# leejet/stable-diffusion.cpp

Measured on AMD Instinct MI355X. Metric: denoise it/s (image-iterations/s: cond+uncond UNet forwards per image per step), higher is better.
Workload: dtype f16; 1 GPU; sd15 UNet 512x512, cfg 7 (cond+uncond), f16 weights, batch 8/GPU, Euler-A step; global_batch=8, flash_attn=True, hip_graph=1, cfg_pair_in_one_graph=True, device_resident_sampler=True

## Files before the change

include/ggml-mi355x.h:

```cpp
#ifndef GGML_MI355X_H
#define GGML_MI355X_H

#include "ggml-abi.h"

#ifdef __cplusplus
extern "C" {
#endif

#define GGML_MI355X_API __attribute__((visibility("default")))

GGML_MI355X_API ggml_backend_reg_t ggml_backend_init(void);
GGML_MI355X_API int ggml_backend_score(void);
GGML_MI355X_API ggml_backend_reg_t ggml_backend_mi355x_reg(void);
GGML_MI355X_API int ggml_backend_mi355x_get_device_count(void);

struct ggml_backend_mi355x_stats {
    int64_t graphs_computed;
    int64_t plans_built;
    int64_t nodes_seen;
    int64_t kernels_planned;
    int64_t kernels_launched;
    int64_t fused_conv;
    int64_t fused_conv_bounced;
    int64_t fused_linear;
    int64_t fused_norm;
    int64_t fused_geglu;
    int64_t fused_attention;
    int64_t generic_matmul;
    int64_t swizzled_weight_bytes;
    int64_t graph_replays;
    int64_t fused_linear_geglu;
    int64_t split_k_gemms;
    int64_t head_major_gemms;
    int64_t fused_modulate;
    int64_t fused_gate;
    int64_t fused_gelu;
    int64_t fused_rope;
    int64_t fused_concat_heads;
    int64_t qgemv_linears;
    int64_t fused_chan_add;
    int64_t fused_proj_tokens;
    int64_t gemm_attention;
    int64_t fused_q16;
    int64_t split_k_inlaunch;
    int64_t qgemm16_linears;
    int64_t fgemv_linears;
    int64_t fused_presilu;
    int64_t fused_sibling_linears;
    int64_t hoisted_kv_linears;
    int64_t window_convs;
    int64_t hoisted_emb_linears;
    int64_t fused_rows16;
    int64_t fused_joint_qkv;
    int64_t jit_images;
    int64_t fused_cat_rows16;
    int64_t fused_gn_stats;
    int64_t fused_ln_reduce;
    int64_t redirect_fallbacks;
    int64_t fused_concat_gn;
    int64_t fused_conv_scale;
    int64_t view_graphs;
    int64_t plans_evicted;
    int64_t hoisted_mod_linears;
    int64_t view_external_nodes;
    int64_t qinloop_linears;
    int64_t flash_out_alias;
    int64_t flash_slice_images;
    int64_t flash_short_launches;
    int64_t flash_qb2_launches;
    int64_t flash_mslot_launches;
    int64_t flash_generic_launches;
};
GGML_MI355X_API void ggml_backend_mi355x_get_stats(struct ggml_backend_mi355x_stats* out);
GGML_MI355X_API int ggml_backend_mi355x_resolve_enums(const char* (*op_name)(int), const char* (*unary_op_name)(int), const char* (*type_name)(int));
GGML_MI355X_API const char* ggml_backend_mi355x_enum_status(void);
GGML_MI355X_API void ggml_backend_mi355x_get_enum_maps(uint8_t* ops256, uint8_t* unary256);
struct ggml_backend_mi355x_kernel_timing {
    char kernel[96];
    int64_t launches;
    double total_ms;
    double total_flops;
    double total_bytes;
    int32_t bound;
    int32_t family;
};
GGML_MI355X_API void ggml_backend_mi355x_kernel_timing_enable(int enable);
GGML_MI355X_API void ggml_backend_mi355x_kernel_timing_enable_mask(uint32_t family_mask);
GGML_MI355X_API void ggml_backend_mi355x_get_kernel_timing(struct ggml_backend_mi355x_kernel_timing* out);
GGML_MI355X_API int ggml_backend_mi355x_get_kernel_timings(struct ggml_backend_mi355x_kernel_timing* out, int capacity);
GGML_MI355X_API void ggml_backend_mi355x_set_option(const char* key, int value);
struct ggml_backend_mi355x_calibration {
    float mfma_f16_tflops;
    float mfma_clock_mhz;
    float copy_tbs;
    float read_tbs;
    int compute_units;
};
GGML_MI355X_API int ggml_backend_mi355x_calibrate(struct ggml_backend_mi355x_calibration* out);
GGML_MI355X_API void* ggml_backend_mi355x_get_stream(ggml_backend_t backend);
GGML_MI355X_API const char* ggml_backend_mi355x_hip_library(void);
GGML_MI355X_API int ggml_backend_mi355x_set_device(int hip_device);
GGML_MI355X_API int ggml_backend_mi355x_get_device(void);

#ifdef __cplusplus
}
#endif
#endif
```

stable-diffusion.cpp_amd/__init__.py:

```python
from __future__ import annotations

import ctypes as C
import os
from pathlib import Path

import numpy as np

PKG_DIR = Path(__file__).resolve().parent
ROOT = PKG_DIR.parent
LIB_DIR = PKG_DIR / "lib"
HOST_LIB = Path(os.environ.get("SDCPP_HOST_LIB", str(LIB_DIR / "libsdcpp-host.so")))
BACKEND_LIB = Path(os.environ.get("SDCPP_BACKEND_LIB", str(LIB_DIR / "libggml-mi355x.so")))

F32, F16, Q4_0, Q8_0, I32, BF16 = 0, 1, 2, 8, 26, 30
TYPE_SIZE = {F32: 4, F16: 2, BF16: 2, I32: 4}

SD15, SDXL, SD15_TINY, SDXL_TINY, SD35_LARGE, SD35_TINY, FLUX_DEV, FLUX_TINY, SD35_WIDE2, FLUX_WIDE1, SD3M_TINY, SD35_WIDE8, FLUX_WIDE8 = 0, 1, 2, 3, 4, 5, 6, 7, 8, 9, 10, 11, 12
PAIR_EXCHANGE_FN = C.CFUNCTYPE(C.c_bool, C.c_void_p, C.c_int64, C.c_void_p, C.c_void_p)
EVAL_CALLBACK_FN = C.CFUNCTYPE(C.c_bool, C.c_void_p, C.c_bool, C.c_void_p)
EULER, EULER_A, HEUN, DPM2, DPMPP2S_A, DPMPP2M, DPMPP2Mv2, IPNDM, IPNDM_V, LCM, DDIM_TRAILING = range(11)
TCD, RES_MULTISTEP, RES_2S, ER_SDE, EULER_CFG_PP, EULER_A_CFG_PP, EULER_GE, DPMPP2M_SDE, DPMPP2M_SDE_BT, LMS = range(11, 21)
SAMPLE_METHOD_DEFAULT = 21
SCHED_DISCRETE, SCHED_KARRAS, SCHED_EXPONENTIAL, SCHED_AYS, SCHED_GITS, SCHED_SGM_UNIFORM, SCHED_SIMPLE, SCHED_SMOOTHSTEP, SCHED_KL_OPTIMAL, SCHED_LCM = range(10)
SCHED_BONG_TANGENT, SCHED_FLUX, SCHED_BETA, SCHEDULER_DEFAULT = 10, 14, 15, 16
# ... 202 lines not shown
    L.sd_get_tensor_f32.restype = C.c_bool
    L.sd_set_tensor_f32.argtypes = [C.c_void_p, C.c_char_p, C.c_void_p, C.c_int64]
    L.sd_set_tensor_f32.restype = C.c_bool
    L.sd_unet_forward.argtypes = [C.c_void_p, C.c_void_p, C.c_int, C.c_int, C.c_int, C.c_int, C.c_void_p, C.c_void_p,
                                  C.c_int64, C.c_int64, C.c_int64, C.c_void_p, C.c_int64, C.c_int64, C.c_void_p]
    L.sd_unet_forward.restype = C.c_bool
    L.sd_vae_decode.argtypes = [C.c_void_p, C.c_void_p, C.c_int, C.c_int, C.c_int, C.c_int, C.c_void_p]
    L.sd_vae_decode.restype = C.c_bool
    L.sd_sample_latents.argtypes = [C.c_void_p, C.POINTER(SdImgGenParams), C.c_void_p]
    L.sd_sample_latents.restype = C.c_bool
    L.sdm_generate_image.argtypes = [C.c_void_p, C.POINTER(SdImgGenParams), C.POINTER(C.POINTER(SdImage)), C.POINTER(C.c_int)]
    L.sdm_generate_image.restype = C.c_bool
    L.sdm_free_images.argtypes = [C.POINTER(SdImage), C.c_int]
    L.sd_philox_randn.argtypes = [C.c_uint64, C.c_uint32, C.c_uint32, C.c_void_p]
    L.sd_philox_uint32.argtypes = [C.c_uint64, C.c_uint32, C.c_uint32, C.c_void_p]
    L.sd_get_sigmas.argtypes = [C.c_int, C.c_void_p]
    L.sd_get_flow_sigmas.argtypes = [C.c_int, C.c_float, C.c_void_p]
    L.sd_get_flux_sigmas.argtypes = [C.c_int, C.c_int, C.c_void_p]
    L.sd_set_guidance.argtypes = [C.c_void_p, C.c_float]
    L.sd_set_guidance.restype = None
    L.sd_set_vae_conv2d_scale.argtypes = [C.c_void_p, C.c_float]
    L.sd_set_vae_conv2d_scale.restype = C.c_bool
    L.sd_set_pair_exchange.argtypes = [C.c_void_p, PAIR_EXCHANGE_FN, C.c_void_p, C.c_int]
    L.sd_set_pair_exchange.restype = None
    L.sd_rccl_get_unique_id.argtypes = [C.c_void_p]
    L.sd_rccl_get_unique_id.restype = C.c_bool
    L.sd_rccl_comm_create.argtypes = [C.c_int, C.c_int, C.c_int, C.c_void_p]
    L.sd_rccl_comm_create.restype = C.c_void_p
    L.sd_rccl_comm_destroy.argtypes = [C.c_void_p]
    L.sd_rccl_comm_destroy.restype = None
    L.sd_set_pair_exchange_rccl.argtypes = [C.c_void_p, C.c_void_p, C.c_int]
    L.sd_set_pair_exchange_rccl.restype = C.c_bool
    L.sd_rccl_last_error.restype = C.c_char_p
    L.sd_gen_flux_pe.argtypes = [C.c_int, C.c_int, C.c_int, C.c_int, C.POINTER(C.c_int), C.c_int, C.c_float, C.c_void_p]
    L.sd_sigma_to_t.argtypes = [C.c_float]
    L.sd_sigma_to_t.restype = C.c_float
    L.sd_get_stats.argtypes = [C.c_void_p, C.POINTER(SdStats)]
    L.sd_load_weights_prefixed.argtypes = [C.c_void_p, C.c_char_p, C.c_char_p, C.POINTER(C.c_int64), C.POINTER(C.c_int64)]
    L.sd_load_weights_prefixed.restype = C.c_int64
    L.sd_convert_tensor_name.argtypes = [C.c_void_p, C.c_char_p, C.c_char_p, C.c_size_t]
    L.sd_convert_tensor_name.restype = C.c_bool
    L.sd_text_encoders_init.argtypes = [C.c_void_p]
    L.sd_text_encoders_init.restype = C.c_bool
    L.sd_clip_forward.argtypes = [C.c_void_p, C.c_int, C.c_void_p, C.c_int, C.c_int, C.c_bool, C.c_int, C.c_void_p, C.c_int64]
    L.sd_clip_forward.restype = C.c_int64
    L.sd_t5_forward.argtypes = [C.c_void_p, C.c_void_p, C.c_int, C.c_void_p, C.c_int64]
    L.sd_t5_forward.restype = C.c_int64
    L.sd_t5_relative_position_buckets.argtypes = [C.c_int, C.c_int, C.c_void_p]
    L.sd_get_learned_condition.argtypes = [C.c_void_p, C.POINTER(SdTokenList), C.POINTER(SdTokenList), C.POINTER(SdTokenList), C.c_int, C.c_int, C.c_int,
                                           C.c_bool, C.c_void_p, C.c_int64, C.POINTER(C.c_int64), C.c_void_p, C.c_int64, C.POINTER(C.c_int64)]
    L.sd_get_learned_condition.restype = C.c_bool
    L.sdm_set_backend_eval_callback.argtypes = [EVAL_CALLBACK_FN, C.c_void_p]
    L.sdm_set_backend_eval_callback.restype = None
    L.sdm_backend_graph_compute_with_eval_callback.argtypes = [C.c_void_p, C.c_void_p, EVAL_CALLBACK_FN, C.c_void_p]
    L.sdm_backend_graph_compute_with_eval_callback.restype = C.c_int
    _lib = L
    return L


_loaded_plugins: set[str] = set()


def load_backend(path: os.PathLike | str) -> None:
    p = str(Path(path).resolve())
    if p in _loaded_plugins:
        return
    if not lib().sd_load_backend(p.encode()):
        raise EngineError(f"failed to load backend plug-in {p}")
    _loaded_plugins.add(p)


def load_mi355x_backend() -> None:
    if not BACKEND_LIB.exists():
        raise EngineError(f"{BACKEND_LIB} missing — the HIP backend was not built")
    load_backend(BACKEND_LIB)
    names = devices()
    if not any(n.upper().startswith("MI355X") for n in names):
        raise EngineError(f"libggml-mi355x.so loaded but exposes no MI355X device (devices: {names}); is a gfx950 GPU visible?")


_BACKEND_STAT_FIELDS = ("graphs_computed plans_built nodes_seen kernels_planned kernels_launched fused_conv fused_conv_bounced fused_linear "
                        "fused_norm fused_geglu fused_attention generic_matmul swizzled_weight_bytes graph_replays fused_linear_geglu "
                        "split_k_gemms head_major_gemms fused_modulate fused_gate fused_gelu fused_rope fused_concat_heads qgemv_linears fused_chan_add fused_proj_tokens gemm_attention fused_q16 split_k_inlaunch qgemm16_linears fgemv_linears fused_presilu fused_sibling_linears hoisted_kv_linears window_convs hoisted_emb_linears fused_rows16 fused_joint_qkv jit_images fused_cat_rows16 fused_gn_stats fused_ln_reduce redirect_fallbacks fused_concat_gn fused_conv_scale view_graphs plans_evicted hoisted_mod_linears view_external_nodes qinloop_linears flash_out_alias flash_slice_images "
                        "flash_short_launches flash_qb2_launches flash_mslot_launches flash_generic_launches").split()


class BackendStats(C.Structure):
    _fields_ = [(n, C.c_int64) for n in _BACKEND_STAT_FIELDS]


_backend_cdll = None


def _backend() -> C.CDLL:
    global _backend_cdll
    if _backend_cdll is None:
        load_mi355x_backend()
        _backend_cdll = C.CDLL(str(BACKEND_LIB))
        _backend_cdll.ggml_backend_mi355x_get_stats.argtypes = [C.POINTER(BackendStats)]
        _backend_cdll.ggml_backend_mi355x_set_option.argtypes = [C.c_char_p, C.c_int]
    return _backend_cdll


def backend_stats() -> dict:
    st = BackendStats()
    _backend().ggml_backend_mi355x_get_stats(C.byref(st))
    return {n: int(getattr(st, n)) for n in _BACKEND_STAT_FIELDS}


class KernelTiming(C.Structure):
    _fields_ = [("kernel", C.c_char * 96), ("launches", C.c_int64), ("total_ms", C.c_double), ("total_flops", C.c_double),
                ("total_bytes", C.c_double), ("bound", C.c_int32), ("family", C.c_int32)]


KF_ALL = 0x3FFFF


def kernel_timing_enable(on) -> None:
    b = _backend()
    b.ggml_backend_mi355x_kernel_timing_enable_mask.argtypes = [C.c_uint32]
    mask = 1 if on is True else int(on or 0)
    b.ggml_backend_mi355x_kernel_timing_enable_mask(mask)


def _timing_dict(kt) -> dict:
    return {"kernel": kt.kernel.decode(), "family": int(kt.family), "bound": "hbm" if kt.bound else "mfma", "launches": int(kt.launches),
            "total_ms": float(kt.total_ms), "total_flops": float(kt.total_flops), "total_bytes": float(kt.total_bytes)}


def kernel_timings() -> list:
    arr = (KernelTiming * 32)()
    b = _backend()
    b.ggml_backend_mi355x_get_kernel_timings.argtypes = [C.POINTER(KernelTiming), C.c_int]
    b.ggml_backend_mi355x_get_kernel_timings.restype = C.c_int
    n = b.ggml_backend_mi355x_get_kernel_timings(arr, 32)
    return [_timing_dict(arr[i]) for i in range(n)]


def kernel_timing() -> dict:
    t = kernel_timings()
    return t[0] if t else {"kernel": "(no timed launches)", "family": -1, "bound": "mfma", "launches": 0, "total_ms": 0.0, "total_flops": 0.0, "total_bytes": 0.0}


class Calibration(C.Structure):
    _fields_ = [("mfma_f16_tflops", C.c_float), ("mfma_clock_mhz", C.c_float), ("copy_tbs", C.c_float), ("read_tbs", C.c_float), ("compute_units", C.c_int)]


def calibrate() -> dict | None:
    b = _backend()
    b.ggml_backend_mi355x_calibrate.argtypes = [C.POINTER(Calibration)]
    c = Calibration()
    if b.ggml_backend_mi355x_calibrate(C.byref(c)) != 0:
        return None
    return {"mfma_f16_tflops": round(c.mfma_f16_tflops, 1), "mfma_clock_mhz": round(c.mfma_clock_mhz, 1), "copy_tbs": round(c.copy_tbs, 3), "read_tbs": round(c.read_tbs, 3),
            "compute_units": c.compute_units}


def backend_set_option(key: str, value: int) -> None:
    _backend().ggml_backend_mi355x_set_option(key.encode(), int(value))


def devices() -> list[str]:
    L = lib()
    return [L.sd_device_name(i).decode() for i in range(L.sd_device_count())]


def _fptr(a: np.ndarray | None):
# ... 542 lines not shown
```

stable-diffusion.cpp_amd/csrc/backend/planner.cpp:

```cpp
#include "planner.h"

#include <atomic>
#include <cstddef>
#include <cstdio>
#include <cstdlib>
#include <cstring>
#include <functional>
#include <memory>
#include <mutex>
#include <string>
#include <algorithm>
#include <map>
#include <unordered_map>
#include <unordered_set>
#include <vector>

#include "kernels.h"
#include "ktime.h"

namespace mi355x {

static uint8_t g_opmap[256];
static uint8_t g_unmap[256];
static bool g_opmap_init = [] {
// ... 26 lines not shown
const NameNum kNeededTypes[] = {
    {"f32", GGML_TYPE_F32}, {"f16", GGML_TYPE_F16}, {"q4_0", GGML_TYPE_Q4_0}, {"q8_0", GGML_TYPE_Q8_0}, {"i32", GGML_TYPE_I32}, {"bf16", GGML_TYPE_BF16},
};

bool plausible_op_name(const char* nm) {
    if (!nm) return false;
    int n = 0;
    for (; nm[n] && n <= 32; ++n)
        if (!((nm[n] >= 'A' && nm[n] <= 'Z') || (nm[n] >= '0' && nm[n] <= '9') || nm[n] == '_')) return false;
    return n > 0 && n <= 32;
}
bool build_map(const char* (*name_of)(int), const NameNum* need, int n_need, int cap, int unknown, uint8_t* table, char* err, size_t err_len, const char* what,
               const char* const* optional = nullptr, int n_optional = 0) {
    uint8_t out[256];
    for (int i = 0; i < 256; ++i) out[i] = (uint8_t)unknown;
    std::vector<int> found(n_need, -1);
    int left = n_need;
    for (int h = 0; h < cap && left > 0; ++h) {
        const char* nm = name_of(h);
        if (!plausible_op_name(nm)) break;
        for (int k = 0; k < n_need; ++k)
            if (!strcmp(nm, need[k].name)) {
                if (found[k] >= 0) {
                    snprintf(err, err_len, "host %s numbers %d and %d are both named '%s'", what, found[k], h, nm);
                    return false;
                }
                found[k] = h;
                out[h]   = (uint8_t)need[k].num;
                --left;
            }
    }
    for (int k = 0; k < n_need; ++k)
        if (found[k] < 0) {
            bool opt = false;
            for (int o = 0; o < n_optional; ++o) opt = opt || !strcmp(optional[o], need[k].name);
            if (opt) continue;
            snprintf(err, err_len, "host has no %s named '%s'", what, need[k].name);
            return false;
        }
    memcpy(table, out, 256);
    return true;
}
}

bool planner_build_op_maps(const char* (*op_name)(int), const char* (*unary_name)(int), const char* (*type_name)(int), char* err, size_t err_len) {
    uint8_t ops[256], un[256];
    if (err && err_len) err[0] = 0;
    char local[256];
    if (!err) {
        err     = local;
        err_len = sizeof(local);
    }
    static const char* const kOptionalOps[]   = {"CONV_2D"};
    static const char* const kOptionalUnary[] = {"EXP"};
    if (op_name && !build_map(op_name, kNeededOps, (int)(sizeof(kNeededOps) / sizeof(kNeededOps[0])), 200, GGML_OP_COUNT, ops, err, err_len, "op", kOptionalOps, 1)) return false;
    if (unary_name && !build_map(unary_name, kNeededUnary, (int)(sizeof(kNeededUnary) / sizeof(kNeededUnary[0])), 64, GGML_UNARY_OP_COUNT, un, err, err_len, "unary op", kOptionalUnary, 1))
        return false;
    if (type_name) {
        for (const NameNum& t : kNeededTypes) {
            const char* nm = type_name(t.num);
            if (!nm || strcmp(nm, t.name)) {
                snprintf(err, err_len, "host ggml_type %d is named '%s', this backend was written against '%s'", t.num, nm ? nm : "(null)", t.name);
                return false;
            }
        }
    }
    if (op_name) memcpy(g_opmap, ops, 256);
    if (unary_name) memcpy(g_unmap, un, 256);
    return true;
}
void planner_get_op_maps(uint8_t* ops256, uint8_t* unary256) {
    if (ops256) memcpy(ops256, g_opmap, 256);
    if (unary256) memcpy(unary256, g_unmap, 256);
}

namespace {

constexpr size_t N_STATS = sizeof(ggml_backend_mi355x_stats) / sizeof(int64_t);
static_assert(N_STATS * sizeof(int64_t) == sizeof(ggml_backend_mi355x_stats), "ggml_backend_mi355x_stats: int64_t fields only");
std::atomic<int64_t> g_stat_counters[N_STATS];
#define STAT(field) g_stat_counters[offsetof(ggml_backend_mi355x_stats, field) / sizeof(int64_t)]

struct Options {
    std::atomic<int> fusion{1}, mfma_gemm{1}, hip_graph{1}, flash_pattern{1}, fuse_modulate{1}, fuse_gate{1}, fuse_gelu{1}, fuse_rope{1}, fuse_concat_heads{1}, qgemv{1}, fuse_chan_add{1}, fuse_proj_tokens{1}, fuse_q16{1}, qgemm16{1}, fgemv{1}, fuse_siblings{1}, hoist_kv{1}, hoist_emb{1}, fuse_rows16{0}, fuse_cat_rows16{1}, fuse_joint_qkv{1}, jit_qimages{4096}, fuse_gn_stats{1}, fuse_ln_reduce{1}, relax_res_overlap{1}, fuse_split_gelu{1}, fuse_concat_gn{1}, fuse_gn_tokens{1}, fuse_linear_nchw{1}, fuse_conv_scale{1}, ignore_use_counts{0}, plan_cache_cap{512}, hoist_mod{1}, fuse_flash_slices{1}, fuse_act_pack{1};
} g_opt;

using Step = std::function<void(hipStream_t)>;

struct Plan {
    int n_nodes = 0;
    uint64_t check = 0;
    size_t arena_needed = 0;
    std::vector<Step> steps;
    hipGraphExec_t graph_exec = nullptr;
    bool graph_failed         = false;
    int64_t runs              = 0;
    uint64_t last_use         = 0;
};

struct SwzEntry {
    void* swz;
    size_t bytes;
    const void* src;
    size_t src_bytes;
};

std::mutex g_mu;
std::vector<Planner*> g_planners;

}

struct Planner {
    int device;
    std::mutex mu;
    uint64_t tick = 0;
    std::unordered_map<uint64_t, std::unique_ptr<Plan>> plans;
    std::unordered_map<uint64_t, SwzEntry> swz;
    char* arena       = nullptr;
    size_t arena_cap  = 0;
    std::map<size_t, void*> jit_buf;
    void* jit_buffer(size_t bytes, int parity = 0) {
        const size_t key = bytes * 2 + (size_t)(parity & 1);
        auto it = jit_buf.find(key);
        if (it != jit_buf.end()) return it->second;
        void* d = nullptr;
        if (hipMalloc(&d, bytes) != hipSuccess) return nullptr;
        jit_buf[key] = d;
        return d;
    }
};

namespace {

inline bool overlaps(const void* a, size_t an, const void* b, size_t bn) {
    const char* pa = (const char*)a;
    const char* pb = (const char*)b;
    return pa < pb + bn && pb < pa + an;
}

bool flash_out_aliases_operand(const ggml_tensor* ct, const ggml_tensor* fa, bool q_in_arena, bool k_in_arena, bool v_in_arena) {
    const size_t on = ggml_abi_nbytes(ct);
    const bool skip[3] = {q_in_arena, k_in_arena, v_in_arena};
    for (int j = 0; j < 3; ++j) {
        const ggml_tensor* o = fa->src[j];
        if (!o || skip[j]) continue;
        const ggml_tensor* root = o->view_src ? o->view_src : o;
        if (overlaps(ct->data, on, root->data, ggml_abi_nbytes(root)) || overlaps(ct->data, on, o->data, ggml_abi_nbytes(o))) return true;
    }
    return false;
}

View4 view_of(const ggml_tensor* t) {
    View4 v;
    v.data = t->data;
    for (int i = 0; i < 4; ++i) {
        v.ne[i] = t->ne[i];
        v.nb[i] = (int64_t)t->nb[i];
    }
    v.type = (int)t->type;
    return v;
}
inline bool is_f32(const ggml_tensor* t) { return t->type == GGML_TYPE_F32; }
inline bool contig(const ggml_tensor* t) { return ggml_abi_is_contiguous(t); }
inline const ggml_tensor* root_of(const ggml_tensor* t) { return t->view_src ? t->view_src : t; }
inline bool is_static_weight(const ggml_tensor* t) {
    const ggml_backend_buffer* b = t->view_src ? t->view_src->buffer : t->buffer;
    return b != nullptr && b->usage == GGML_BACKEND_BUFFER_USAGE_WEIGHTS;
// ... 109 lines not shown
        mix2(h, k, &n->data, sizeof(n->data));
        for (int j = 0; j < GGML_MAX_SRC; ++j) {
            const ggml_tensor* s = n->src[j];
            if (!s) break;
            const uint64_t sh[4] = {(uint64_t)(uintptr_t)s->data, ((uint64_t)(uint32_t)s->type << 32) | (uint32_t)j,
                                    ((uint64_t)(uint32_t)s->op << 32) | (is_static_weight(s) ? 1u : 0u), (uint64_t)s->view_offs};
            mix2(h, k, sh, sizeof(sh));
            mix2(h, k, s->ne, sizeof(s->ne));
            mix2(h, k, s->nb, sizeof(s->nb));
        }
    }
    return {h, k};
}

struct GInfo {
    const ggml_cgraph* g;
    std::unordered_map<const ggml_tensor*, int> index;
    std::vector<std::vector<int>> consumers;
    std::vector<char> done;

    ggml_tensor phantom;
    bool is_view = false;
    int n_external = 0;

    explicit GInfo(const ggml_cgraph* gr) : g(gr), consumers(gr->n_nodes + 1), done(gr->n_nodes + 1, 0) {
        memset(&phantom, 0, sizeof(phantom));
        phantom.op = (enum ggml_op)255;
        for (int h = 255; h >= 0; --h)
            if (g_opmap[h] == GGML_OP_COUNT) {
                phantom.op = (enum ggml_op)h;
                break;
            }
        snprintf(phantom.name, sizeof(phantom.name), "(reader outside the view)");
        done[g->n_nodes] = 1;
        for (int i = 0; i < g->n_nodes; ++i) index[g->nodes[i]] = i;
        for (int i = 0; i < g->n_nodes; ++i) {
            const ggml_tensor* n = g->nodes[i];
            for (int j = 0; j < GGML_MAX_SRC; ++j) {
                if (!n->src[j]) continue;
                auto it = index.find(n->src[j]);
                if (it != index.end()) consumers[it->second].push_back(i);
            }
        }
        is_view = graph_is_view(g);
        if (is_view) {
            std::vector<char> ext;
            view_external_nodes(g, ext);
            for (int i = 0; i < g->n_nodes; ++i)
                if (ext[i]) {
                    consumers[i].push_back(g->n_nodes);
                    ++n_external;
                }
        }
    }
    const ggml_tensor* node(int i) const { return i == g->n_nodes ? &phantom : g->nodes[i]; }
    int idx(const ggml_tensor* t) const {
        auto it = index.find(t);
        return it == index.end() ? -1 : it->second;
    }
    int sole(int i) const {
        if (i < 0 || consumers[i].size() != 1) return -1;
        if (node(i)->flags & GGML_TENSOR_FLAG_OUTPUT) return -1;
        if (i == g->n_nodes - 1) return -1;
        return consumers[i][0];
    }
    bool only_noops_between(int a, int b, const std::vector<int>& chain) const {
        for (int k = a + 1; k < b; ++k) {
            if (ggml_abi_op_is_noop(xop(node(k)))) continue;
            bool in_chain = false;
            for (int c : chain) in_chain = in_chain || (c == k);
            if (!in_chain) return false;
        }
        return true;
    }
};

struct Packed {
    size_t off;
    int64_t ld;
    bool nhwc;
    float mul = 1.f;
    int64_t runL = 0, runS = 0;
};

struct Builder {
    Planner* P;
    Plan* plan;
    GInfo gi;
    size_t arena_off = 0;
    std::unordered_map<const ggml_tensor*, Packed> packed;
    std::unordered_map<const ggml_tensor*, size_t> q16;
    std::unordered_map<const ggml_tensor*, const ggml_tensor*> ups;
    std::unordered_map<const ggml_tensor*, const ggml_tensor*> presilu;
    std::map<int, std::vector<Step>> deferred;
    std::map<size_t, int> jit_seq;
    Builder(Planner* p, Plan* pl, const ggml_cgraph* g) : P(p), plan(pl), gi(g) {}
    int emit_redirect = -1;
    bool hm_grouping  = false;
    bool hm_hoisting  = false;
    struct HmLaunch {
        int node, out_node;
        float* dst;
        void* dst16;
        size_t dst16_off;
        bool dst16_arena;
        size_t a_off;
        int64_t lda;
        const void* swz;
        int64_t tokens, K, M;
        Epilogue ep;
        int hd, hH, hL;
    };
    std::vector<HmLaunch> hm_group;
    std::unordered_map<const ggml_tensor*, size_t> moved;
    struct MovedEmb {
        size_t off;
        int64_t ld, M, N;
    };
    std::unordered_map<const ggml_tensor*, MovedEmb> moved_emb;
    struct GnPre {
        size_t off;
        const float *w, *b;
        int groups;
        float eps;
    };
    std::unordered_map<const ggml_tensor*, GnPre> gn_pre;
    struct LnPre {
        size_t off;
        const float *w, *b;
        float eps;
    };
    std::unordered_map<const ggml_tensor*, LnPre> ln_pre;
    struct Cat16 {
        size_t off;
        int64_t ld;
        bool written[2];
    };
    struct Cat16Part {
        size_t off;
        int64_t ld, col;
        int cat, part;
    };
    std::unordered_map<int, Cat16> cat16;
    std::unordered_map<const ggml_tensor*, Cat16Part> cat16_part;
    struct PreScale {
        const ggml_tensor* src;
        float mul;
    };
    std::unordered_map<const ggml_tensor*, PreScale> prescale;
    std::unordered_set<const ggml_tensor*> cat16_by_linear;
    struct JPart {
        size_t off = 0;
        int64_t xs = 0;
        const float* w = nullptr;
        float eps = 0.f;
    };
    struct JCat {
        JPart part[2];
        int d = 0, H = 0, last = -1;
        bool f16 = false;
        std::vector<int> chain;
    };
    std::unordered_map<int, JCat> jqkv;
    std::unordered_map<const ggml_tensor*, size_t> lin_redirect;
    std::unordered_set<const ggml_tensor*> redirect_taken;
    bool no_redirect = false;
    struct RopeSrc {
        JPart part[2];
        int64_t La = 0, Lb = 0;
    };
    std::unordered_map<int, RopeSrc> rope_src, v_src;
    std::unordered_map<int, std::pair<size_t, size_t>> scratch_slots;
    size_t scratch(int key, size_t bytes) {
        auto it = scratch_slots.find(key);
        if (it != scratch_slots.end() && it->second.second >= bytes) return it->second.first;
        const size_t off   = alloc(bytes);
        scratch_slots[key] = {off, bytes};
        return off;
    }
    void emit(Step s) {
        if (emit_redirect >= 0)
            deferred[emit_redirect].push_back(std::move(s));
        else
            plan->steps.push_back(std::move(s));
    }
    void emit_at(int node, int cur, Step s) {
        if (node <= cur)
            emit(std::move(s));
        else
            deferred[node].push_back(std::move(s));
    }
    bool clobbered_between(int a, int b, const void* p, size_t n, const std::vector<int>& chain) const {
        for (int k = a + 1; k <= b; ++k) {
            const ggml_tensor* t = gi.node(k);
            if (ggml_abi_op_is_noop(xop(t))) continue;
            bool in_chain = false;
            for (int c : chain) in_chain = in_chain || (c == k);
            if (in_chain) continue;
            const char *a0 = (const char*)t->data, *b0 = (const char*)p;
            if (a0 < b0 + n && b0 < a0 + ggml_abi_nbytes(t)) return true;
        }
        return false;
    }
    size_t alloc(size_t bytes) {
        const size_t off = (arena_off + 255) & ~(size_t)255;
        arena_off        = off + bytes;
        return off;
    }
    static constexpr size_t CNT_CAP = 1u << 18;
// ... 445 lines not shown
        STAT(qgemv_linears)++;
        STAT(fused_linear)++;
        if (silu) STAT(fused_presilu)++;
        return;
    }
    if (g_opt.fgemv && plain_epi && simple_rows && src_safe && emit_node == i && fgemv_supported((int)w->type, tokens, K) && aligned16(w->data)) {
        float* fdst       = (float*)gi.node(last)->data;
        const float* fx   = (const float*)xsrc->data;
        const int64_t fxs = (int64_t)x->nb[1] / 4;
        const void* wp    = w->data;
        const int wt      = (int)w->type;
        const bool silu   = xsrc != x;
        B.emit([=](hipStream_t st) { launch_fgemv(st, fdst, M, fx, fxs, tokens, wp, wt, K, M, ep, silu); });
        STAT(fgemv_linears)++;
        STAT(fused_linear)++;
        if (silu) STAT(fused_presilu)++;
        return;
    }
    if (xsrc != x) {
        float* ud       = (float*)x->data;
        const float* us = (const float*)xsrc->data;
        const int64_t un = ggml_abi_nelements(x);
        B.emit([=](hipStream_t st) { launch_unary(st, UN_SILU, ud, us, un); });
    }
    const bool useq  = g_opt.qgemm16 && hm_d == 0 && geglu_out < 0 && qgemm16_supported((int)w->type, tokens, K, M);
    const void* wraw = w->data;
    const int wt     = (int)w->type;
    const bool qin = !useq && geglu_out < 0 && hm_d == 0 && !B.hm_hoisting && nchw_add < 0 && (wt == 8 || wt == 2) &&
                     (int64_t)w->nb[1] == (int64_t)ggml_abi_row_size(w->type, K) && aligned16(w->data) && gemm16_qinloop_supported(wt, tokens, M, K, 1, 1);
    if (qin) {
        ep.qtype      = wt;
        ep.qrow_bytes = (int64_t)w->nb[1];
        STAT(qinloop_linears)++;
    }
    const bool jit = !useq && !qin && g_opt.jit_qimages > 0 && tokens >= g_opt.jit_qimages && geglu_out < 0 && hm_d == 0 && !B.hm_hoisting && wswz_q_supported((int)w->type, K) &&
                     (int64_t)w->nb[1] == (int64_t)ggml_abi_row_size(w->type, K) && aligned16(w->data);
    const int geglu_mode = geglu_out >= 0 ? gemm16_geglu_mode(tokens, M, K) : 0;
    const void* swz = useq ? nullptr : qin ? w->data : (jit ? B.P->jit_buffer(wswz_bytes(M, K), B.jit_seq[wswz_bytes(M, K)]++) : get_swz_linear(B.P, w, s, geglu_mode));
    if (jit && swz) {
        void* jb          = const_cast<void*>(swz);
        const void* wsrc  = w->data;
        const int wty     = (int)w->type;
        B.emit_at(emit_node, i, [=](hipStream_t st) { launch_wswz_q(st, jb, wsrc, wty, K, M); });
        STAT(jit_images)++;
    }
    float* dst      = (float*)gi.node(last)->data;
    const float* xp = (const float*)x->data;
    const int64_t xs = (int64_t)x->nb[1] / 4;
    const ggml_tensor* key = strip_reshape(x);
    auto it = B.packed.find(key);
    if (it == B.packed.end() || it->second.nhwc) {
        Packed pk{B.alloc((size_t)tokens * rup64(K) * 2), rup64(K), false};
        Planner* P = B.P;
        const size_t off = pk.off;
        const bool runs  = x->ne[2] > 1 && x->nb[2] != x->nb[1] * (size_t)x->ne[1];
        const int64_t pL = runs ? x->ne[1] : 0, pbs = runs ? (int64_t)x->nb[2] / 4 : 0;
        B.emit([=](hipStream_t st) { launch_pack_rows_f16(st, P->arena + off, xp, tokens, K, xs, pL, pbs); });
        it = B.packed.emplace(key, pk).first;
        if (it->second.nhwc) it->second = pk;
    }
    Planner* P       = B.P;
    size_t off       = it->second.off;
    const int64_t ld = it->second.ld;
    if (it->second.runL > 0) {
        const int64_t rL = it->second.runL, rS = it->second.runS;
        if (geglu_out >= 0 || hm_d > 0 || nchw_add >= 0) {
            const size_t goff = B.alloc((size_t)tokens * ld * 2), soff = off;
            const int64_t nrun = tokens / rL;
            B.emit([=](hipStream_t st) {
                for (int64_t r = 0; r < nrun; ++r)
                    (void)hipMemcpyAsync(P->arena + goff + (size_t)(r * rL * ld * 2), P->arena + soff + (size_t)(r * rS * ld * 2), (size_t)(rL * ld * 2), hipMemcpyDeviceToDevice, st);
            });
            off = goff;
        } else {
            ep.a_run_L = rL;
            ep.a_run_S = rS;
        }
    }
    if (nchw_add >= 0 && !useq && swz && ld == rup64(K) && geglu_out < 0 && gelu_out < 0 && !ep.gate && !redir) {
        float* ndst             = (float*)gi.node(nchw_add)->data;
        const int64_t HWt = nchw_HW, Nimg = nchw_N;
        const float* resp       = nchw_res;
        const Builder::Split sk = B.plan_split(tokens, M, rup64(K), true, true);
        B.emit_at(emit_node, i, [=](hipStream_t st) {
            Epilogue e2 = ep;
            e2.residual = resp;
            launch_gemm16_conv(st, ndst, P->arena + off, swz, HWt, 1, K, Nimg, M, 1, 1, 0, false, e2, sk.ws(P), sk.cnt(P), sk.S);
        });
        STAT(fused_linear)++;
        STAT(fused_proj_tokens)++;
        return;
    }
    if (nchw_add >= 0) {
        while (!chain.empty() && chain.back() != last) chain.pop_back();
    }
    if (geglu_out >= 0) {
        const size_t ooff  = B.alloc((size_t)tokens * (M / 2) * 2);
        const float* biasp = ep.bias;
        const Builder::Split sk = B.plan_split(tokens, M, K, false, false, true);
        B.emit([=](hipStream_t st) { launch_gemm16_linear_geglu(st, P->arena + ooff, P->arena + off, ld, swz, tokens, K, M, biasp, sk.ws(P), sk.cnt(P), sk.S, geglu_mode); });
        B.packed[gi.node(geglu_out)] = Packed{ooff, M / 2, false};
        STAT(fused_geglu)++;
        STAT(fused_linear_geglu)++;
    } else if (gelu_out >= 0) {
        const size_t ooff = B.alloc((size_t)tokens * M * 2);
        if (useq) {
            B.emit([=](hipStream_t st) { launch_qgemm16(st, nullptr, P->arena + ooff, M, P->arena + off, ld, tokens, wraw, wt, K, M, ep); });
            STAT(qgemm16_linears)++;
        } else {
            const Builder::Split sk = B.plan_split(tokens, M, K, false, false);
            B.emit([=](hipStream_t st) { launch_gemm16_linear(st, nullptr, P->arena + ooff, M, P->arena + off, ld, swz, tokens, K, M, M, ep, 0, 0, 0, sk.ws(P), sk.cnt(P), sk.S); });
        }
        B.packed[gi.node(gelu_out)] = Packed{ooff, M, false};
        STAT(fused_gelu)++;
    } else if (hm_d > 0) {
        void* hdst = gi.node(last)->data;
        STAT(head_major_gemms)++;
        const bool f16o = hm_f16;
        const int hd = hm_d, hH = hm_H, hL = hm_L;
        int qflash = -1, qview = -1;
        if (!f16o && g_opt.fuse_q16 && hd % 8 == 0) {
            const int c1 = gi.sole(last);
            const int c2 = (c1 >= 0 && xop(gi.node(c1)) == GGML_OP_RESHAPE) ? gi.sole(c1) : -1;
            if (c2 >= 0 && xop(gi.node(c2)) == GGML_OP_FLASH_ATTN_EXT && gi.node(c2)->src[0] == gi.node(c1) && !gi.node(c2)->src[3] && contig(gi.node(c1)) &&
                gi.node(c1)->ne[0] == hd && flash_attn_supported(hd, gi.node(c2)->src[2]->ne[0])) {
                qflash = c2;
                qview  = c1;
            }
        }
        const bool groupable = B.hm_grouping && !ep.residual && !ep.gate && !ep.gelu && !ep.chan_add;
        if (qflash >= 0) {
            const size_t qoff        = B.alloc((size_t)tokens * M * 2);
            B.q16[gi.node(qview)]    = qoff;
            STAT(fused_q16)++;
            const Builder::Split sk = B.plan_split(tokens, M, K, false, false);
            if (groupable && sk.S <= 1)
                B.hm_group.push_back(Builder::HmLaunch{i, last, nullptr, nullptr, qoff, true, off, ld, swz, tokens, K, M, ep, hd, hH, hL});
            else
                B.emit([=](hipStream_t st) { launch_gemm16_linear(st, nullptr, P->arena + qoff, 0, P->arena + off, ld, swz, tokens, K, M, M, ep, hd, hH, hL, sk.ws(P), sk.cnt(P), sk.S); });
        } else {
            const Builder::Split sk = (hL >= 32 && !B.hm_hoisting) ? B.plan_split(tokens, M, K, false, false) : Builder::Split();
            if (groupable && sk.S <= 1)
                B.hm_group.push_back(Builder::HmLaunch{i, last, f16o ? nullptr : (float*)hdst, f16o ? hdst : nullptr, 0, false, off, ld, swz, tokens, K, M, ep, hd, hH, hL});
            else
                B.emit([=](hipStream_t st) {
                    launch_gemm16_linear(st, f16o ? nullptr : (float*)hdst, f16o ? hdst : nullptr, 0, P->arena + off, ld, swz, tokens, K, M, M, ep, hd, hH, hL, sk.ws(P), sk.cnt(P), sk.S);
                });
        }
    } else if (useq) {
        const int S        = ep.gate ? 1 : qgemm16_split_k(tokens, K, M);
        const size_t wsoff = S > 1 ? B.alloc((size_t)S * tokens * M * 4) : 0;
        B.emit_at(emit_node, i, [=](hipStream_t st) {
            launch_qgemm16(st, redir ? (float*)(P->arena + redir_off) : dst, nullptr, 0, P->arena + off, ld, tokens, wraw, wt, K, M, ep, S > 1 ? (float*)(P->arena + wsoff) : nullptr, S);
        });
        if (redir) B.redirect_taken.insert(gi.node(last));
        STAT(qgemm16_linears)++;
    } else if (g_opt.fuse_rows16 && !ep.gate && emit_node == i && M % 64 == 0 && x->ne[3] == 1 && only_consumer_is_tokens_to_conv(gi, last)) {
        const size_t ooff       = B.alloc((size_t)tokens * M * 2);
        const Builder::Split sk = B.plan_split(tokens, M, K, false, false);
        B.emit([=](hipStream_t st) { launch_gemm16_linear(st, nullptr, P->arena + ooff, M, P->arena + off, ld, swz, tokens, K, M, M, ep, 0, 0, 0, sk.ws(P), sk.cnt(P), sk.S); });
        B.packed[gi.node(last)] = Packed{ooff, M, false};
        STAT(fused_rows16)++;
    } else {
        const Builder::Split sk = B.plan_split(tokens, M, K, false, !ep.gate);
        bool ln_on       = false;
        size_t ln_off    = 0;
        const float *lnw = nullptr, *lnb = nullptr;
        float lneps      = 0.f;
        if (g_opt.fuse_ln_reduce && g_opt.fusion && sk.S > 1 && sk.S <= 4 && !sk.inkernel && !redir && !ep.gate && emit_node == i && hm_d == 0 && splitk_reduce_ln_supported(tokens, M) &&
// ... 539 lines not shown
        const int jp = gi.sole(last);
        const int jc = (jp >= 0 && xop(gi.node(jp)) == GGML_OP_PERMUTE && gi.node(jp)->src[0] == gi.node(last)) ? gi.sole(jp) : -1;
        if (jc >= 0 && xop(gi.node(jc)) == GGML_OP_CONT && gi.node(jc)->src[0] == gi.node(jp) && is_f32(gi.node(jc)) && contig(gi.node(jc))) {
            const int32_t* pa = gi.node(jp)->op_params;
            std::vector<int> c2 = chain;
            c2.push_back(jp);
            c2.push_back(jc);
            if (pa[0] == 1 && pa[1] == 2 && pa[2] == 0 && pa[3] == 3 && gi.node(jc)->ne[0] == OC && gi.only_noops_between(last, jc, c2) &&
                !(gi.node(last)->flags & GGML_TENSOR_FLAG_OUTPUT)) {
                chain           = c2;
                last            = jc;
                token_major_out = jc;
            }
        }
    }
    const size_t ob = ggml_abi_nbytes(out);
    int emit_node = i;
    bool emb_arena = false;
    size_t emb_off = 0;
    if (g_opt.fuse_chan_add && token_major_out < 0) {
        const int r = gi.sole(last);
        if (r >= 0 && xop(gi.node(r)) == GGML_OP_ADD && gi.node(r)->src[0] == gi.node(last)) {
            const ggml_tensor* a = gi.node(r);
            const ggml_tensor* e = a->src[1];
            const ggml_tensor* eroot = strip_reshape(e);
            const bool from_linear   = xop(eroot) == GGML_OP_MUL_MAT || (xop(eroot) == GGML_OP_ADD && eroot->src[0] && xop(strip_reshape(eroot->src[0])) == GGML_OP_MUL_MAT);
            if (!gi.done[r] && from_linear && is_f32(e) && contig(e) && contig(a) && e->ne[0] == 1 && e->ne[1] == 1 && e->ne[2] == OC && e->ne[3] == N && N > 0 &&
                ggml_abi_same_shape(out, a) && gi.idx(eroot) < r && !(gi.node(last)->flags & GGML_TENSOR_FLAG_OUTPUT)) {
                bool ok = true;
                for (int k = last + 1; k < r && ok; ++k) {
                    const ggml_tensor* t = gi.node(k);
                    if (ggml_abi_op_is_noop(xop(t))) continue;
                    for (int q = 0; q < GGML_MAX_SRC && t->src[q]; ++q)
                        for (int c : chain) ok = ok && t->src[q] != gi.node(c);
                }
                if (ok) {
                    ep.chan_add = (const float*)e->data;
                    chain.push_back(r);
                    last      = r;
                    emit_node = r;
                    STAT(fused_chan_add)++;
                    const auto me = B.moved_emb.find(eroot);
                    if (me != B.moved_emb.end()) {
                        emb_arena  = true;
                        emb_off    = me->second.off;
                        ep.chan_ld = me->second.ld;
                        ep.chan_add = nullptr;
                    }
                }
            }
        }
    }
    if (!ep.chan_add && !emb_arena && token_major_out < 0) {
        int r = gi.sole(last);
        if (r >= 0 && !gi.done[r] && xop(gi.node(r)) == GGML_OP_ADD && gi.only_noops_between(last, r, chain)) {
            const ggml_tensor* a     = gi.node(r);
            const ggml_tensor* other = a->src[0] == gi.node(last) ? a->src[1] : (a->src[1] == gi.node(last) ? a->src[0] : nullptr);
            if (other && is_f32(other) && contig(other) && contig(a) && ggml_abi_same_shape(other, a) && ggml_abi_same_shape(out, a) && gi.idx(other) < i &&
                (other->data == a->data || !overlaps(a->data, ob, other->data, ob))) {
                ep.residual = (const float*)other->data;
                chain.push_back(r);
                last = r;
            }
        }
    }
    float* final_dst = (float*)gi.node(last)->data;
    const int ks = KW, st_ = s0, pd = p0;
    Builder::GnPre gnp{0, nullptr, nullptr, 0, 0.f};
    if (g_opt.fuse_gn_stats && token_major_out < 0) {
        const ggml_tensor* res = gi.node(last);
        for (int k : gi.consumers[last]) {
            if (gnp.groups) break;
            const ggml_tensor* g = gi.node(k);
            if (xop(g) != GGML_OP_GROUP_NORM || g->src[0] != res || gi.done[k]) continue;
            const int j1 = gi.sole(k);
            if (j1 < 0 || xop(gi.node(j1)) != GGML_OP_MUL || gi.node(j1)->src[0] != g || !bias_like_chan(gi.node(j1)->src[1], OC)) break;
            const int j2 = gi.sole(j1);
            if (j2 < 0 || xop(gi.node(j2)) != GGML_OP_ADD || gi.node(j2)->src[0] != gi.node(j1) || !bias_like_chan(gi.node(j2)->src[1], OC)) break;
            const int64_t ohw = res->ne[0] * res->ne[1];
            if (!splitk_reduce_gn_supported(ohw, OC, N, g->op_params[0])) break;
            gnp = Builder::GnPre{0, (const float*)gi.node(j1)->src[1]->data, (const float*)gi.node(j2)->src[1]->data, g->op_params[0], ggml_abi_op_param_f32(g, 1)};
        }
    }
    auto gn_register = [&](int S) -> bool {
        if (S <= 1 || !gnp.groups) return false;
        if ((((uintptr_t)final_dst | (uintptr_t)ep.residual) & 15) != 0) return false;
        gnp.off                    = B.alloc((size_t)N * OC * 4 * 2);
        B.gn_pre[gi.node(last)]    = gnp;
        STAT(fused_gn_stats)++;
        return true;
    };
    auto gn_fill = [](Epilogue& e, const Builder::GnPre& g, char* arena, int64_t nc) {
        e.gn_scale  = (float*)(arena + g.off);
        e.gn_shift  = e.gn_scale + nc;
        e.gn_w      = g.w;
        e.gn_b      = g.b;
        e.gn_groups = g.groups;
        e.gn_eps    = g.eps;
    };
    const bool ups_in = B.ups.find(xs) != B.ups.end();
    const int w3S     = (token_major_out < 0) ? conv3w_plan(x->ne[0], x->ne[1], IC, N, OC, ks, st_, ups_in) : 0;
    const void* swz   = get_swz_conv(B.P, ker, s, w3S > 0);
    if (!swz) return false;
    const ggml_tensor* src = xs;
    bool upscale           = false;
    auto ui                = B.ups.find(xs);
    if (ui != B.ups.end()) {
        src     = ui->second;
        upscale = true;
    }
    const int64_t SW = src->ne[0], SH = src->ne[1];
    auto it = B.packed.find(src);
    if (it != B.packed.end() && it->second.nhwc && it->second.mul != pre_mul) {
        fprintf(stderr, "[ggml-mi355x] plan_conv_chain: operand image of node %d was written with factor %g, the conv wants %g\n", i, it->second.mul, pre_mul);
        return false;
    }
    if (it == B.packed.end() || !it->second.nhwc) {
        Packed pk{B.alloc((size_t)N * SW * SH * rup64(IC) * 2), rup64(IC), true, pre_mul};
        Planner* P       = B.P;
        const size_t off = pk.off;
        const float* sp  = (const float*)src->data;
        B.emit([=](hipStream_t st) { launch_nchw_to_nhwc_f16(st, P->arena + off, sp, SW * SH, IC, N, nullptr, nullptr, false, nullptr, 0, nullptr, pre_mul); });
        B.packed[src] = pk;
        it            = B.packed.find(src);
    }
    Planner* P       = B.P;
    const size_t off = it->second.off;
    const int64_t CW_ = upscale ? SW * 2 : SW, CH_ = upscale ? SH * 2 : SH;
    const int64_t opos = ((CW_ + 2 * pd - ks) / st_ + 1) * ((CH_ + 2 * pd - ks) / st_ + 1) * N;
    if (token_major_out >= 0) {
        float* tdst          = (float*)gi.node(token_major_out)->data;
        const int64_t tokens = SW * SH * N;
        const int64_t lda    = it->second.ld;
        B.emit([=](hipStream_t st) { launch_gemm16_linear(st, tdst, nullptr, 0, P->arena + off, lda, swz, tokens, IC, OC, OC, ep); });
        STAT(fused_conv)++;
        STAT(fused_proj_tokens)++;
        return true;
    }
    if (w3S > 0) {
        const size_t wsoff = w3S > 1 ? B.alloc((size_t)w3S * opos * OC * 4) : 0;
        if (w3S > 1) STAT(split_k_gemms)++;
        const bool gn_on = gn_register(w3S);
        B.emit_at(emit_node, i, [=](hipStream_t st) {
            Epilogue e2 = ep;
            if (emb_arena) e2.chan_add = (const float*)(P->arena + emb_off);
            if (gn_on) gn_fill(e2, gnp, P->arena, N * OC);
            launch_conv3w(st, final_dst, P->arena + off, swz, SW, SH, IC, N, OC, e2, w3S > 1 ? (float*)(P->arena + wsoff) : nullptr, w3S);
        });
        STAT(fused_conv)++;
        STAT(window_convs)++;
        return true;
    }
    const Builder::Split sk = B.plan_split(opos, OC, rup64(IC) * ks * ks, true, true);
    const bool gn_on        = sk.inkernel ? false : gn_register(sk.S);
    B.emit_at(emit_node, i, [=](hipStream_t st) {
        Epilogue e2 = ep;
        if (emb_arena) e2.chan_add = (const float*)(P->arena + emb_off);
        if (gn_on) gn_fill(e2, gnp, P->arena, N * OC);
        launch_gemm16_conv(st, final_dst, P->arena + off, swz, SW, SH, IC, N, OC, ks, st_, pd, upscale, e2, sk.ws(P), sk.cnt(P), sk.S);
    });
    STAT(fused_conv)++;
    return true;
}

bool plan_tokens_to_conv(Builder& B, int i, hipStream_t, std::vector<int>& chain) {
    GInfo& gi = B.gi;
    int rs    = -1;
    if (!tokens_to_conv_match(gi, i, &rs)) return false;
    const ggml_tensor* t  = gi.node(i)->src[0]->src[0];
    const ggml_tensor* xr = gi.node(rs);
    const int64_t C = t->ne[0], HW = t->ne[1], N = t->ne[2];
    chain = {i};
    STAT(fused_proj_tokens)++;
    const auto pr = B.packed.find(t);
    if (pr != B.packed.end() && !pr->second.nhwc && pr->second.ld == rup64(C)) {
        B.packed[xr] = Packed{pr->second.off, pr->second.ld, true};
        return true;
    }
    Packed pk{B.alloc((size_t)N * HW * rup64(C) * 2), rup64(C), true};
    Planner* P       = B.P;
    const size_t off = pk.off;
    const float* tp  = (const float*)t->data;
    B.emit([=](hipStream_t st) { launch_pack_rows_f16(st, P->arena + off, tp, N * HW, C, C); });
    B.packed[xr] = pk;
    return true;
}

bool plan_group_norm(Builder& B, int i, hipStream_t, std::vector<int>& chain) {
    GInfo& gi            = B.gi;
    const ggml_tensor* n = gi.node(i);
    const ggml_tensor* x = n->src[0];
    if (!is_f32(x) || !contig(x) || !contig(n)) return false;
    const int groups = n->op_params[0];
    const float eps  = ggml_abi_op_param_f32(n, 1);
    const int64_t hw = x->ne[0] * x->ne[1], C = x->ne[2], N = x->ne[3];
    const float *w = nullptr, *b = nullptr;
    bool silu = false;
    chain.push_back(i);
    int last = i;
    if (g_opt.fusion) {
        int j1 = gi.sole(i);
        if (j1 >= 0 && xop(gi.node(j1)) == GGML_OP_MUL && gi.node(j1)->src[0] == n && bias_like_chan(gi.node(j1)->src[1], C) && gi.node(j1)->data == n->data &&
            gi.only_noops_between(i, j1, chain)) {
            int j2 = gi.sole(j1);
            if (j2 >= 0 && xop(gi.node(j2)) == GGML_OP_ADD && gi.node(j2)->src[0] == gi.node(j1) && bias_like_chan(gi.node(j2)->src[1], C) &&
                gi.node(j2)->data == n->data && gi.only_noops_between(j1, j2, chain)) {
                w = (const float*)gi.node(j1)->src[1]->data;
                b = (const float*)gi.node(j2)->src[1]->data;
                chain.push_back(j1);
                chain.push_back(j2);
                last   = j2;
                int j3 = gi.sole(j2);
                if (j3 >= 0 && xop(gi.node(j3)) == GGML_OP_UNARY && xunary(gi.node(j3)) == GGML_UNARY_OP_SILU && gi.node(j3)->data == n->data &&
                    gi.only_noops_between(j2, j3, chain)) {
                    silu = true;
                    chain.push_back(j3);
                    last = j3;
                }
            }
        }
    }
    float* dst      = (float*)n->data;
    const float* xp = (const float*)x->data;
    int tok_cont = -1;
    if (g_opt.fusion && g_opt.fuse_gn_tokens && w && !silu) {
        const int jp = gi.sole(last);
        const ggml_tensor* pt = jp >= 0 ? gi.node(jp) : nullptr;
        if (pt && xop(pt) == GGML_OP_PERMUTE && pt->src[0] == gi.node(last) && pt->op_params[0] == 1 && pt->op_params[1] == 2 && pt->op_params[2] == 0 && pt->op_params[3] == 3) {
            const int jc = gi.sole(jp);
            const ggml_tensor* ct = jc >= 0 ? gi.node(jc) : nullptr;
            if (ct && xop(ct) == GGML_OP_CONT && ct->src[0] == pt && is_f32(ct) && contig(ct) && ct->ne[0] == C && !(ct->flags & GGML_TENSOR_FLAG_OUTPUT) && all_consumers_gemm16(gi, jc, false)) {
                std::vector<int> c2 = chain;
                c2.push_back(jp);
                c2.push_back(jc);
                if (gi.only_noops_between(last, jc, c2)) tok_cont = jc;
            }
        }
    }
    if (tok_cont >= 0) {
        Planner* P       = B.P;
        const auto pre   = B.gn_pre.find(x);
        const bool have  = pre != B.gn_pre.end() && pre->second.w == w && pre->second.b == b && pre->second.groups == groups && pre->second.eps == eps;
        const size_t so  = have ? pre->second.off : B.alloc((size_t)N * C * 4 * 2);
        const size_t off = B.alloc((size_t)N * hw * rup64(C) * 2);
        const int gsp    = have ? 0 : gn_stats_split(hw, C, N, groups);
        const size_t po  = gsp ? B.alloc((size_t)N * groups * gsp * 2 * 4) : 0;
        B.emit([=](hipStream_t st) {
            float* sc = (float*)(P->arena + so);
            float* sh = sc + N * C;
            if (!have) launch_gn_stats(st, sc, sh, xp, hw, C, N, groups, eps, w, b, nullptr, 0, gsp ? (float*)(P->arena + po) : nullptr);
            launch_nchw_to_nhwc_f16(st, P->arena + off, xp, hw, C, N, sc, sh, false);
        });
        chain.push_back(gi.sole(last));
        chain.push_back(tok_cont);
        B.packed[gi.node(tok_cont)] = Packed{off, rup64(C), false};
        STAT(fused_norm)++;
        STAT(fused_proj_tokens)++;
        return true;
    }
    float conv_mul = 1.f;
    if (w && all_consumers_gemm16(gi, last, true, &conv_mul)) {
        Planner* P          = B.P;
        const auto pre      = B.gn_pre.find(x);
        const bool have     = pre != B.gn_pre.end() && pre->second.w == w && pre->second.b == b && pre->second.groups == groups && pre->second.eps == eps;
        const size_t so     = have ? pre->second.off : B.alloc((size_t)N * C * 4 * 2);
        const size_t off    = B.alloc((size_t)N * hw * rup64(C) * 2);
        const int gsp       = have ? 0 : gn_stats_split(hw, C, N, groups);
        const size_t po     = gsp ? B.alloc((size_t)N * groups * gsp * 2 * 4) : 0;
        B.emit([=](hipStream_t st) {
            float* sc = (float*)(P->arena + so);
            float* sh = sc + N * C;
            if (!have) launch_gn_stats(st, sc, sh, xp, hw, C, N, groups, eps, w, b, nullptr, 0, gsp ? (float*)(P->arena + po) : nullptr);
            launch_nchw_to_nhwc_f16(st, P->arena + off, xp, hw, C, N, sc, sh, silu, nullptr, 0, nullptr, conv_mul);
        });
        STAT(kernels_planned)++;
        B.packed[gi.node(last)] = Packed{off, rup64(C), true, conv_mul};
        STAT(fused_norm)++;
        return true;
    }
    B.emit([=](hipStream_t st) { launch_group_norm(st, dst, xp, hw, C, N, groups, eps, w, b, silu); });
    if (last != i) STAT(fused_norm)++;
    return true;
}

bool plan_concat_gn(Builder& B, int i, hipStream_t, std::vector<int>& chain) {
    GInfo& gi            = B.gi;
    const ggml_tensor* n = gi.node(i);
    if (!g_opt.fusion || !g_opt.fuse_concat_gn || xop(n) != GGML_OP_CONCAT || n->op_params[0] != 2 || !is_f32(n) || !contig(n) || (n->flags & GGML_TENSOR_FLAG_OUTPUT)) return false;
    const ggml_tensor *a = n->src[0], *b = n->src[1];
    if (!is_f32(a) || !is_f32(b) || !contig(a) || !contig(b) || a->ne[0] != n->ne[0] || a->ne[1] != n->ne[1] || a->ne[3] != n->ne[3] || b->ne[0] != n->ne[0] || b->ne[1] != n->ne[1] ||
        b->ne[3] != n->ne[3] || a->ne[2] + b->ne[2] != n->ne[2])
        return false;
    const int64_t hw = n->ne[0] * n->ne[1], C = n->ne[2], C1 = a->ne[2], N = n->ne[3];
    int jg = -1, jc = -1;
    for (int c : gi.consumers[i]) {
        const ggml_tensor* t = gi.node(c);
        if (xop(t) == GGML_OP_GROUP_NORM && t->src[0] == n && jg < 0)
            jg = c;
        else if (xop(t) == GGML_OP_IM2COL && t->src[1] == n && jc < 0 && conv_im2col_fast_ok(gi, c))
            jc = c;
        else
            return false;
    }
    if (jg < 0) return false;
    const ggml_tensor* gn = gi.node(jg);
    const int groups      = gn->op_params[0];
    const float eps       = ggml_abi_op_param_f32(gn, 1);
    if (!contig(gn) || !gn_two_source_supported((const float*)a->data, (const float*)b->data, hw, C, C1, groups)) return false;
    const int j1 = gi.sole(jg);
    if (j1 < 0 || xop(gi.node(j1)) != GGML_OP_MUL || gi.node(j1)->src[0] != gn || !bias_like_chan(gi.node(j1)->src[1], C) || gi.node(j1)->data != gn->data) return false;
    const int j2 = gi.sole(j1);
    if (j2 < 0 || xop(gi.node(j2)) != GGML_OP_ADD || gi.node(j2)->src[0] != gi.node(j1) || !bias_like_chan(gi.node(j2)->src[1], C) || gi.node(j2)->data != gn->data) return false;
    int last  = j2;
    bool silu = false;
    const int j3 = gi.sole(j2);
    if (j3 >= 0 && xop(gi.node(j3)) == GGML_OP_UNARY && xunary(gi.node(j3)) == GGML_UNARY_OP_SILU && gi.node(j3)->data == gn->data) {
        silu = true;
        last = j3;
    }
    if (!all_consumers_gemm16(gi, last, true)) return false;
    for (int k : {jg, j1, j2, j3})
        if (k >= 0 && k <= last && gi.done[k]) return false;
    const float* w  = (const float*)gi.node(j1)->src[1]->data;
    const float* bb = (const float*)gi.node(j2)->src[1]->data;
    Planner* P       = B.P;
    const size_t so  = B.alloc((size_t)N * C * 4 * 2);
    const size_t off = B.alloc((size_t)N * hw * rup64(C) * 2);
    const size_t roff = jc >= 0 ? B.alloc((size_t)N * hw * rup64(C) * 2) : 0;
    const float *ap = (const float*)a->data, *bp = (const float*)b->data;
    const bool raw  = jc >= 0;
    B.emit([=](hipStream_t st) {
        float* sc = (float*)(P->arena + so);
        float* sh = sc + N * C;
        launch_gn_stats(st, sc, sh, ap, hw, C, N, groups, eps, w, bb, bp, C1);
        launch_nchw_to_nhwc_f16(st, P->arena + off, ap, hw, C, N, sc, sh, silu, bp, C1, raw ? (void*)(P->arena + roff) : nullptr);
    });
    B.packed[gi.node(last)] = Packed{off, rup64(C), true};
    if (raw) B.packed[n] = Packed{roff, rup64(C), true};
    chain = {i, jg, j1, j2};
    if (silu) chain.push_back(j3);
    STAT(fused_norm)++;
    STAT(fused_concat_gn)++;
    return true;
}

bool plan_layer_norm(Builder& B, int i, hipStream_t, std::vector<int>& chain) {
    GInfo& gi            = B.gi;
    const ggml_tensor* n = gi.node(i);
    const ggml_tensor* x = n->src[0];
    if (!is_f32(x) || x->nb[0] != 4 || n->nb[0] != 4) return false;
    if ((x->ne[2] > 1 && x->nb[2] != x->nb[1] * (size_t)x->ne[1]) || (x->ne[3] > 1 && x->nb[3] != x->nb[2] * (size_t)x->ne[2]) ||
        (n->ne[2] > 1 && n->nb[2] != n->nb[1] * (size_t)n->ne[1]) || (n->ne[3] > 1 && n->nb[3] != n->nb[2] * (size_t)n->ne[2])) {
        for (int d = 1; d < 4; ++d)
            if (x->nb[d] % 4 != 0 || n->nb[d] % 4 != 0) return false;
        View4 xv = view_of(x), dv = view_of(n);
        const float eps4 = ggml_abi_op_param_f32(n, 0);
        const bool rms4  = xop(n) == GGML_OP_RMS_NORM;
        B.emit([=](hipStream_t st) { launch_layer_norm_4d(st, (float*)dv.data, (const float*)xv.data, xv.ne, xv.nb, dv.nb, eps4, nullptr, nullptr, rms4); });
        chain.push_back(i);
        return true;
    }
    const bool rms   = xop(n) == GGML_OP_RMS_NORM;
    const float eps  = ggml_abi_op_param_f32(n, 0);
    const int64_t C = x->ne[0], rows = x->ne[1] * x->ne[2] * x->ne[3];
    const float *w = nullptr, *b = nullptr;
    chain.push_back(i);
    int last = i;
    if (g_opt.fusion) {
        int j1 = gi.sole(i);
        if (j1 >= 0 && xop(gi.node(j1)) == GGML_OP_MUL && gi.node(j1)->src[0] == n && bias_like_row(gi.node(j1)->src[1], C) && gi.node(j1)->data == n->data &&
            gi.only_noops_between(i, j1, chain)) {
            w = (const float*)gi.node(j1)->src[1]->data;
            chain.push_back(j1);
            last   = j1;
            int j2 = gi.sole(j1);
            if (j2 >= 0 && xop(gi.node(j2)) == GGML_OP_ADD && gi.node(j2)->src[0] == gi.node(j1) && bias_like_row(gi.node(j2)->src[1], C) &&
                gi.node(j2)->data == n->data && gi.only_noops_between(j1, j2, chain)) {
                b = (const float*)gi.node(j2)->src[1]->data;
                chain.push_back(j2);
                last = j2;
            }
        }
    }
    float* dst      = (float*)n->data;
    const float* xp = (const float*)x->data;
    const int64_t xs = (int64_t)x->nb[1] / 4, ds = (int64_t)n->nb[1] / 4;
    if (g_opt.fusion && g_opt.fuse_modulate && !w && !rms && gi.consumers[i].size() == 2 && n->ne[3] == 1 && contig(n) && C % 4 == 0 && xs % 4 == 0 && aligned16(xp)) {
        int jm = -1, ja = -1;
        for (int c : gi.consumers[i]) {
            const ggml_tensor* t = gi.node(c);
            if (xop(t) == GGML_OP_MUL && t->src[0] == n) jm = c;
            if (xop(t) == GGML_OP_ADD && t->src[0] == n) ja = c;
        }
        auto mod_vec = [&](const ggml_tensor* v) {
            return v && is_f32(v) && contig(v) && v->ne[0] == C && v->ne[1] == 1 && v->ne[2] == n->ne[2] && v->ne[3] == 1 && aligned16(v->data);
        };
        const int js = (jm >= 0 && ja >= 0 && gi.node(ja)->src[1] == gi.node(jm) && gi.sole(jm) == ja) ? gi.sole(ja) : -1;
        if (js >= 0 && xop(gi.node(js)) == GGML_OP_ADD && gi.node(js)->src[0] == gi.node(ja) && mod_vec(gi.node(jm)->src[1]) && mod_vec(gi.node(js)->src[1]) &&
            all_consumers_gemm16(gi, js, false)) {
            std::vector<int> c2{i, jm, ja, js};
            const ggml_tensor* sc_t = gi.node(jm)->src[1];
            if (!B.clobbered_between(i, js, x->data, ggml_abi_nbytes(x), c2)) {
                chain               = c2;
                Planner* P          = B.P;
                const size_t off    = B.alloc((size_t)rows * rup64(C) * 2);
                const float* scalep = (const float*)sc_t->data;
                const float* shiftp = (const float*)gi.node(js)->src[1]->data;
                const int64_t L     = n->ne[1];
                const bool sc_clob  = B.clobbered_between(jm, js, sc_t->data, ggml_abi_nbytes(sc_t), c2);
                const size_t sc_n   = ggml_abi_nbytes(sc_t);
                const size_t sc_off = sc_clob ? B.alloc(sc_n) : 0;
                if (sc_clob) B.emit_at(jm, i, [=](hipStream_t st) { (void)hipMemcpyAsync(P->arena + sc_off, scalep, sc_n, hipMemcpyDeviceToDevice, st); });
                B.emit_at(js, i, [=](hipStream_t st) {
                    launch_layer_norm_f16(st, P->arena + off, xp, C, rows, xs, eps, sc_clob ? (const float*)(P->arena + sc_off) : scalep, shiftp, false, L);
                });
                B.packed[gi.node(js)] = Packed{off, rup64(C), false};
                STAT(fused_norm)++;
// ... 1535 lines not shown
            if (!a || !b || n->type != GGML_TYPE_F32) return false;
            const bool at = a->type == GGML_TYPE_F32 || a->type == GGML_TYPE_F16 || a->type == GGML_TYPE_BF16 || a->type == GGML_TYPE_Q8_0 || a->type == GGML_TYPE_Q4_0;
            const bool bt = b->type == GGML_TYPE_F32 || b->type == GGML_TYPE_F16;
            return at && bt && a->nb[0] == ggml_abi_type_size(a->type) && b->nb[0] == ggml_abi_type_size(b->type);
        }
        case GGML_OP_IM2COL:
            return f32c(n->src[1]) && (n->type == GGML_TYPE_F16 || n->type == GGML_TYPE_F32);
        case GGML_OP_CONV_2D: {
            const ggml_tensor *k = n->src[0], *x = n->src[1];
            if (!k || !x || k->type != GGML_TYPE_F16 || !f32c(x) || !ggml_abi_is_contiguous(x) || !ggml_abi_is_contiguous(k)) return false;
            const int32_t* p = n->op_params;
            const int ks     = (int)k->ne[0];
            if (k->ne[1] != ks || p[0] != p[1] || p[2] != p[3] || p[4] != 1 || p[5] != 1) return false;
            return (ks == 3 && p[2] == 1 && (p[0] == 1 || p[0] == 2)) || (ks == 1 && p[2] == 0 && p[0] == 1);
        }
        case GGML_OP_CONCAT:
        case GGML_OP_REPEAT:
        case GGML_OP_UPSCALE:
        case GGML_OP_PAD:
            if (xop(n) == GGML_OP_UPSCALE && n->op_params[0] != GGML_SCALE_MODE_NEAREST) return false;
            return f32c(n) && f32c(n->src[0]);
        case GGML_OP_GET_ROWS: {
            const ggml_tensor *a = n->src[0], *b = n->src[1];
            if (!a || !b || !f32c(n) || b->type != GGML_TYPE_I32 || n->nb[0] != 4) return false;
            const bool at = a->type == GGML_TYPE_F32 || a->type == GGML_TYPE_F16 || a->type == GGML_TYPE_BF16 || a->type == GGML_TYPE_Q8_0 || a->type == GGML_TYPE_Q4_0;
            return at && a->nb[0] == ggml_abi_type_size(a->type);
        }
        case GGML_OP_TIMESTEP_EMBEDDING:
            return f32c(n) && f32c(n->src[0]);
        case GGML_OP_FLASH_ATTN_EXT: {
            const ggml_tensor *q = n->src[0], *k = n->src[1], *v = n->src[2];
            if (!q || !k || !v || n->src[3] != nullptr) return false;
            if (!f32c(q) || !(k->type == GGML_TYPE_F16 || k->type == GGML_TYPE_F32) || v->type != k->type) return false;
            if (ggml_abi_op_param_f32(n, 1) != 0.0f || ggml_abi_op_param_f32(n, 2) != 0.0f) return false;
            if (q->nb[0] != 4 || k->nb[0] != ggml_abi_type_size(k->type) || v->nb[0] != ggml_abi_type_size(v->type)) return false;
            if (q->ne[3] != 1 || k->ne[2] != q->ne[2]) return false;
            return flash_attn_supported(q->ne[0], v->ne[0]);
        }
        default:
            return false;
    }
}

void planner_get_stats(ggml_backend_mi355x_stats* o) {
    int64_t* out = reinterpret_cast<int64_t*>(o);
    for (size_t i = 0; i < N_STATS; ++i) out[i] = g_stat_counters[i].load();
    o->flash_short_launches   = flash_attn_variant_launches(FLASH_VAR_SHORT);
    o->flash_qb2_launches     = flash_attn_variant_launches(FLASH_VAR_QB2);
    o->flash_mslot_launches   = flash_attn_variant_launches(FLASH_VAR_MSLOT);
    o->flash_generic_launches = flash_attn_variant_launches(FLASH_VAR_GENERIC);
}

namespace {
struct OptionRow {
    const char* key;
    std::atomic<int> Options::*member;
    void (*setter)(int);
};
#define OPT(name) {#name, &Options::name, nullptr}
const OptionRow g_option_table[] = {
    OPT(fusion),
    OPT(mfma_gemm),
    OPT(hip_graph),
    OPT(flash_pattern),
    {"gemm16_t320", nullptr, gemm16_set_t320},
    {"t256p_pad", nullptr, gemm16_set_t256p_pad},
    {"tail_split", nullptr, gemm16_set_tail_split},
    {"conv_wmajor", nullptr, gemm16_set_conv_wmajor},
    {"ln16_rows", nullptr, gemm16_set_ln16_rows},
    {"t320_linear_max_split", nullptr, gemm16_set_t320_linear_max_split},
    OPT(qgemv),
    OPT(fuse_q16),
    {"streamk", nullptr, gemm16_set_streamk},
    {"geglu16", nullptr, gemm16_set_geglu16},
    {"bn64_max_tiles", nullptr, gemm16_set_bn64_max},
    {"conv3w_prio", nullptr, conv3w_set_prio},
    {"t256p_min_nt_sk", nullptr, gemm16_set_t256p_min_nt_sk},
    {"t256p_min_tiles_sk", nullptr, gemm16_set_t256p_min_tiles_sk},
    {"conv3w", nullptr, conv3w_set},
    OPT(hoist_emb),
    OPT(fuse_rows16),
    OPT(fuse_cat_rows16),
    OPT(fuse_gn_stats),
    OPT(fuse_joint_qkv),
    OPT(fuse_ln_reduce),
    OPT(jit_qimages),
    {"qinloop_min_rows", nullptr, gemm16_set_qinloop_min_rows},
    OPT(fuse_flash_slices),
    {"gemm16_t192p", nullptr, gemm16_set_t192p},
    {"conv3w_min_blocks", nullptr, conv3w_set_min_blocks},
    {"conv3w_min_blocks_deep", nullptr, conv3w_set_min_blocks_deep},
    {"gemm16_bn64", nullptr, gemm16_set_bn64},
    OPT(qgemm16),
    {"qgemv_max_rows", nullptr, qgemv_set_max_rows},
    OPT(fgemv),
    OPT(fuse_siblings),
    OPT(hoist_kv),
    {"fgemv_max_rows", nullptr, fgemv_set_max_rows},
    {"qgemm16_max_rows", nullptr, qgemm16_set_max_rows},
    {"qgemm16_rb", nullptr, qgemm16_set_rb},
    {"splitk_inkernel", nullptr, gemm16_set_splitk_inkernel},
    {"splitk_in_target", nullptr, gemm16_set_splitk_in_target},
    OPT(fuse_chan_add),
    OPT(fuse_proj_tokens),
    OPT(fuse_modulate),
    OPT(fuse_gate),
    OPT(relax_res_overlap),
    OPT(fuse_split_gelu),
    OPT(fuse_concat_gn),
    OPT(fuse_gn_tokens),
    OPT(fuse_linear_nchw),
    OPT(fuse_conv_scale),
    OPT(fuse_act_pack),
    OPT(hoist_mod),
    OPT(plan_cache_cap),
    OPT(ignore_use_counts),
    OPT(fuse_gelu),
    OPT(fuse_rope),
    OPT(fuse_concat_heads),
    {"gemm16_variant", nullptr, gemm16_set_variant},
    {"conv_tap_major", nullptr, gemm16_set_tap_major},
    {"gemm16_tile", nullptr, gemm16_set_tile},
    {"splitk_mid", nullptr, gemm16_set_splitk_mid},
    {"splitk_target", nullptr, gemm16_set_splitk_target},
    {"gn_split_min", nullptr, gemm16_set_gn_split_min},
#ifdef MI355X_EXPERIMENTS
    {"gemm16_abl", nullptr, gemm16_set_abl},
#endif
};
#undef OPT
}

void planner_set_option(const char* key, int value) {
    const OptionRow* row = nullptr;
    for (const OptionRow& r : g_option_table)
        if (!strcmp(key, r.key)) row = &r;
    if (!row) {
        fprintf(stderr, "ggml-mi355x: unknown backend option \"%s\" (ignored)\n", key);
        return;
    }
    if (row->member)
        (g_opt.*row->member) = value;
    else
        row->setter(value);
    std::lock_guard<std::mutex> lk(g_mu);
    for (Planner* p : g_planners) {
        std::lock_guard<std::mutex> lp(p->mu);
        (void)hipDeviceSynchronize();
        planner_clear_locked(p);
    }
}

}
```

stable-diffusion.cpp_amd/csrc/kernels/conv3w.hip:

```cpp
#include <cstdio>
#include <cstdlib>

#include "device_utils.h"
#include "g16_common.h"
#include "kernels.h"
#include "ktime.h"

namespace mi355x {

template <int TW, int BN>
struct C3Geom {
    static constexpr int TR     = 256 / TW;
    static constexpr int PITCH  = TW + 16;
    static constexpr int WROWS  = TR + 2;
    static constexpr int WBYTES = WROWS * PITCH * 64;
    static constexpr int NWP    = WBYTES / 1024;
    static constexpr int NWPW   = (NWP + 7) / 8;
    static constexpr int WBUF   = NWPW * 8 * 1024;
    static constexpr int CB     = BN / 64;
    static constexpr int NF     = (BN / 32) * 2;
    static constexpr int BSTAGE = NF * 1024;
    static constexpr int NST    = 4;
    static constexpr int LDS    = 2 * WBUF + NST * BSTAGE;
    static constexpr int RB1    = TW >= 64 ? 32 * 64 : (32 / TW) * PITCH * 64;
// ... 150 lines not shown
        C3_TIE(AS_[0]);                                                                                              \
        C3_TIE(AS_[1]);                                                                                              \
        _Pragma("unroll") for (int cb_ = 0; cb_ < CL; ++cb_) C3_TIE(BL[cb_]);                                        \
        C3_TIE(HS_[0]);                                                                                              \
        C3_TIE(HS_[1]);                                                                                              \
        __builtin_amdgcn_sched_barrier(0);                                                                           \
    } while (0)
#define C3_NOHOOK(I_, ...) ((void)0)
#define C3_DMAHOOK(I_, T_, NP_, LAST_, FSLOT_)                                                        \
    do {                                                                                              \
        if constexpr ((!(LAST_) || (T_) <= 4) && (I_) < (NP_)) C3_DMA_B(I_, FSLOT_);                  \
        if constexpr (!(LAST_) && (T_) < NWPW && (I_) == 3) C3_DMA_W(T_, wb ^ 1);                     \
    } while (0)

#define C3_W(T_) ((T_) >= 0 && (T_) < NWPW ? 1 : 0)
#define C3_STAGE(T_, NP_, LAST_)                                                                                                         \
    do {                                                                                                                                 \
        constexpr int kh_ = (T_) / 3, kw_ = (T_) % 3, tn_ = ((T_) + 1) % 9, khn_ = tn_ / 3, kwn_ = tn_ % 3;                             \
        if constexpr ((T_) == 0 && !(LAST_)) abase += 64;         \
        constexpr int vm_ = (LAST_) ? (NP_) * (((T_) <= 6 ? 1 : 0) + ((T_) <= 5 ? 1 : 0))                                                \
                                    : 2 * (NP_) + C3_W((T_) - 3) + C3_W((T_) - 2) + C3_W((T_) - 1);                                      \
        asm volatile("s_waitcnt lgkmcnt(0)" ::: "memory");                                                                               \
        C3_TIE_FRAGS(A0, BH0);                                                                                                           \
        const uint32_t a1_ = aw[kw_] ^ 32u;                                                                                              \
        C3_KSTEP(A0, A1, BH0, BH1, a1_, kh_ * PITCH * 64, bcur, 1, C3_NOHOOK, 0);                                                        \
        asm volatile("s_waitcnt vmcnt(%0) lgkmcnt(0)" ::"n"(vm_) : "memory");                                                            \
        C3_TIE_FRAGS(A1, BH1);                                                                                                           \
        asm volatile("s_barrier" ::: "memory");                                                                                          \
        const int fslot_ = slot;                                                                                                         \
        slot             = (slot + 1) & 3;                                                                                               \
        bcur             = bad0 + (uint32_t)slot * BSTAGE;                                                                               \
        if constexpr ((T_) == 8 && !(LAST_)) {                     \
            wb ^= 1;                                                                                                                     \
            const uint32_t d_ = wb ? (uint32_t)WBUF : (uint32_t)(0 - WBUF);                                                              \
            _Pragma("unroll") for (int a_ = 0; a_ < 3; ++a_) aw[a_] += d_;                                                               \
        }                                                                                                                                \
        __builtin_amdgcn_sched_barrier(0);                                                                                               \
        C3_KSTEP(A1, A0, BH1, BH0, aw[kwn_], khn_ * PITCH * 64, bcur, 0, C3_DMAHOOK, T_, NP_, LAST_, fslot_);                            \
    } while (0)
#define C3_BLOCK(NP_, LAST_)          \
    do {                              \
        C3_STAGE(0, NP_, LAST_);      \
        C3_STAGE(1, NP_, LAST_);      \
        C3_STAGE(2, NP_, LAST_);      \
        C3_STAGE(3, NP_, LAST_);      \
        C3_STAGE(4, NP_, LAST_);      \
        C3_STAGE(5, NP_, LAST_);      \
        C3_STAGE(6, NP_, LAST_);      \
        C3_STAGE(7, NP_, LAST_);      \
        C3_STAGE(8, NP_, LAST_);      \
    } while (0)
#define C3_MAIN(NP_)                                                                                                         \
    do {                                                                                                                     \
         \
        _Pragma("unroll") for (int j_ = 0; j_ < NWPW; ++j_) C3_DMA_W(j_, 0);                                                 \
        _Pragma("unroll") for (int s_ = 0; s_ < 4; ++s_) {                                                                   \
            if constexpr ((NP_) > 0) C3_DMA_B(0, s_);                                                                        \
            if constexpr ((NP_) > 1) C3_DMA_B(1, s_);                                                                        \
            if constexpr ((NP_) > 2) C3_DMA_B(2, s_);                                                                        \
        }                                                                                                                    \
        asm volatile("s_waitcnt vmcnt(%0)" ::"n"(3 * (NP_)) : "memory");                                                     \
        asm volatile("s_barrier" ::: "memory");                                                                              \
        C3_RD(A0[0], aw[0], 0);                                                                                              \
        C3_RD(A0[1], aw[0], RB1);                                                                                            \
        C3_RD(BL[0], bcur, (0 * 2) * 1024);                                                                                  \
        C3_RD(BL[1], bcur, (1 * 2) * 1024);                                                                                  \
        if constexpr (CL > 2) C3_RD(BL[CL - 1], bcur, (2 * 2) * 1024);                                                       \
        C3_RD(BH0[0], bcur, ((CB - 2) * 2) * 1024);                                                                          \
        C3_RD(BH0[1], bcur, ((CB - 1) * 2) * 1024);                                                                          \
        for (int ib_ = 0; ib_ + 1 < nicb; ++ib_) C3_BLOCK(NP_, false);                                                       \
        C3_BLOCK(NP_, true);                                                                                                 \
        asm volatile("s_waitcnt lgkmcnt(0)" ::: "memory");                                                                   \
    } while (0)

    if constexpr (NF % 8 != 0) {
        if (w_short)
            C3_MAIN(NPBMAX - 1);
        else
            C3_MAIN(NPBMAX);
    } else {
        C3_MAIN(NPBMAX);
    }

    if (g.ep.residual)
        epi_conv<1>(acc, g, row0, col0, wr, wc, lane);
    else
        epi_conv<0>(acc, g, row0, col0, wr, wc, lane);
}

static int g_conv3w_prio = 3;
void conv3w_set_prio(int v) { g_conv3w_prio = v; }
static int g_conv3w = 1;
void conv3w_set(int v) { g_conv3w = v; }
static int g_conv3w_min_blocks = 8, g_conv3w_min_blocks_deep = 5;
void conv3w_set_min_blocks(int v) { g_conv3w_min_blocks = v > 0 ? v : 1; }
void conv3w_set_min_blocks_deep(int v) { g_conv3w_min_blocks_deep = v > 0 ? v : 1; }

int conv3w_plan(int64_t W, int64_t H, int64_t IC, int64_t N, int64_t OC, int ksize, int stride, bool upscale2x, int* bn_out) {
    if (!g_conv3w || ksize != 3 || stride != 1 || upscale2x) return 0;
    if (!(W == 16 || W == 32 || W == 64 || W == 128) || (H * W) % 256 != 0 || IC < 64) return 0;
    if (N * H * W * ((IC + 63) / 64 * 64) * 2 >= (1ll << 32)) return 0;
    const int bn = OC % 320 == 0 ? 320 : (OC % 256 == 0 ? 256 : 0);
    if (!bn) return 0;
    const int64_t tiles = (H * W * N / 256) * (OC / bn);
    const int64_t nicb  = (IC + 63) / 64 * 2;
    int S = 1;
    if (tiles < 192) {
        S = (int)(256 / tiles);
        if (S > 8) S = 8;
        const int64_t minb = tiles <= 64 ? g_conv3w_min_blocks_deep : g_conv3w_min_blocks;
        if (tiles <= 64 && S > 4) S = 4;
        while (S > 1 && (nicb / S < minb || (S - 1) * ((nicb + S - 1) / S) >= nicb)) --S;
        if (tiles * S < 128) return 0;
    } else {
        const int64_t rounds = (tiles + 255) / 256;
        if (tiles * 4 < rounds * 256 * 3) return 0;
    }
    if (bn_out) *bn_out = bn;
    return S;
}

template <int TW, int BN>
static void c3_launch(hipStream_t s, const G16Args& g, unsigned tiles, unsigned ny) {
    if constexpr (BN == 320 && TW <= 64) {
        if (g_conv3w_prio == 0) return (void)k_conv3w<TW, BN, 0><<<dim3(tiles, ny), 512, 0, s>>>(g);
    }
    k_conv3w<TW, BN><<<dim3(tiles, ny), 512, 0, s>>>(g);
}

const _Float16* gemm16_zero_page();
void launch_splitk_reduce_conv_gn(hipStream_t s, float* dst, const float* ws, int S, int64_t hw, int64_t C, int64_t N, const Epilogue& e);
void launch_splitk_reduce_conv(hipStream_t s, float* dst, const float* ws, int S, int64_t n, const float* bias, int64_t inner, int64_t C, const float* residual,
                               const float* chan_add, int64_t chan_ld);

void launch_conv3w(hipStream_t s, float* dst, const void* x16_nhwc, const void* wswz32, int64_t W, int64_t H, int64_t IC, int64_t N, int64_t OC, const Epilogue& e,
                   float* splitk_ws, int S) {
    int bn = 0;
    if (conv3w_plan(W, H, IC, N, OC, 3, 1, false, &bn) == 0) {
        fprintf(stderr, "ggml-mi355x: launch_conv3w called for a shape it does not take\n");
        abort();
    }
    if (e.act >= 0) {
        fprintf(stderr, "ggml-mi355x: conv3w has no fused activation\n");
        abort();
    }
    G16Args g{};
    g.A    = (const _Float16*)x16_nhwc;
    g.W    = (const half8_t*)wswz32;
    g.ICp  = (int)((IC + 63) / 64 * 64);
    g.kfr  = (int64_t)g.ICp * 9 / 16;
    g.dst  = dst;
    g.H    = (int)H;
    g.Wd   = (int)W;
    g.OW   = (int)W;
    g.OH   = (int)H;
    g.OHOW = W * H;
    g.S    = 1;
    g.pad  = 1;
    g.KS   = 3;
    g.nt   = g.ICp / 32;
    g.R    = g.OHOW * N;
    g.C    = OC;
    g.zero = gemm16_zero_page();
    g.ep   = G16Epi{e.bias, e.residual, e.scale};
    g.ep.chan_add = e.chan_add;
    g.ep.chan_ld  = (int)e.chan_ld;
    g.ncol_tiles  = (int)(OC / bn);
    if (S > 1 && splitk_ws) {
        g.split_k  = S;
        g.nt_slice = (g.nt + S - 1) / S;
        g.slab     = g.R * OC;
        g.dst      = splitk_ws;
        g.ep       = G16Epi{nullptr, nullptr, e.scale};
    } else {
        S = 1;
    }
    const unsigned tiles = (unsigned)((g.R / 256) * g.ncol_tiles);
    g.worder             = gemm16_worder_rows(g, tiles, (unsigned)S);
    const double bytes   = (double)N * H * W * g.ICp * 2.0 + (double)g.ICp * 9 * ((OC + 127) / 128 * 128) * 2.0 + (double)g.R * OC * 4.0 * (e.residual ? 2.0 : 1.0);
    {
        KScope ks_(s, KF_CONV_T256, 2.0 * g.R * IC * 9 * OC, bytes);
        if (bn == 320) {
            if (W == 16) c3_launch<16, 320>(s, g, tiles, (unsigned)S);
            else if (W == 32) c3_launch<32, 320>(s, g, tiles, (unsigned)S);
            else if (W == 64) c3_launch<64, 320>(s, g, tiles, (unsigned)S);
            else c3_launch<128, 320>(s, g, tiles, (unsigned)S);
        } else {
            if (W == 16) c3_launch<16, 256>(s, g, tiles, (unsigned)S);
            else if (W == 32) c3_launch<32, 256>(s, g, tiles, (unsigned)S);
            else if (W == 64) c3_launch<64, 256>(s, g, tiles, (unsigned)S);
            else c3_launch<128, 256>(s, g, tiles, (unsigned)S);
        }
    }
    if (S > 1) launch_splitk_reduce_conv_gn(s, dst, splitk_ws, S, g.OHOW, OC, N, e);
}

}
```

stable-diffusion.cpp_amd/csrc/kernels/g16_common.h:

```cpp
#pragma once
#include "device_utils.h"
#include "kernels.h"

namespace mi355x {

struct G16Epi {
    const float* bias;
    const float* residual;
    float scale;
    const float* gate = nullptr;
    int gate_L        = 0;
    int gelu          = 0;
    const float* chan_add = nullptr;
    int chan_ld           = 0;
};

struct G16Args {
    const _Float16* A;
    int64_t lda;
    const half8_t* W;
    int64_t kfr;
    float* dst;
    _Float16* dst16;
    int64_t ldd, ldd16;
    int geglu_inner;
    int geglu16;
    int hm_d, hm_H, hm_L;
    int64_t R, C;
    int64_t row_base;
    int worder;
    int a_runL, a_runS;
    int qt;
    int64_t qrow_bytes;
    int wblk_lim;
    int nt;
    int ncol_tiles;
    int split_k;
    int nt_slice;
    int64_t slab;
    float* sk_slab;
    int* sk_cnt;
    int sk_grid, sk_tiles, sk_dp;
    int split_col;
    _Float16* split_dst16;
    int64_t split_ldd16;
    int multi;
    const half8_t* Wm[16];
    float* dstm[16];
    _Float16* dst16m[16];
    const float* biasm[16];
    int H, Wd, ICp, OH, OW, S, pad, UPS, KS, icb_per_tap, tap_major;
    int64_t OHOW;
    const _Float16* zero;
    G16Epi ep;
#ifdef MI355X_EXPERIMENTS
    int abl;
#endif
};

int gemm16_worder_rows(const G16Args& g, unsigned gx, unsigned ny);
void gemm16_set_conv_wmajor(int v);
__device__ __forceinline__ void g16_wg_order(const G16Args& g, int ncol_all, int& bid, int& kslice) {
    if (g.worder > 0) {
        const int L  = (int)blockIdx.y * (int)gridDim.x + (int)blockIdx.x;
        const int k  = L & 7, j = L >> 3;
        const int pl = j / g.worder, r = j - pl * g.worder;
        const int p  = pl * 8 + k;
        kslice       = p / ncol_all;
        bid          = r * ncol_all + (p - kslice * ncol_all);
        return;
    }
    const int nb = gridDim.x;
    bid          = blockIdx.x;
    if ((nb & 7) == 0) bid = (bid & 7) * (nb >> 3) + (bid >> 3);
    kslice = blockIdx.y;
}

#define GLDS16(gptr, ldsptr) \
    __builtin_amdgcn_global_load_lds((const __attribute__((address_space(1))) void*)(gptr), (__attribute__((address_space(3))) void*)(ldsptr), 16, 0, 0)


template <typename T>
__device__ __forceinline__ void st_u(T* ubase, uint32_t lane_bytes, T v) { *(T*)((char*)ubase + lane_bytes) = v; }
template <typename T>
__device__ __forceinline__ T ld_u(const T* ubase, uint32_t lane_bytes) { return *(const T*)((const char*)ubase + lane_bytes); }

enum { EPI_F32 = 0, EPI_F32_RES = 1, EPI_F16 = 2, EPI_HM_F32 = 3, EPI_HM_F16 = 4, EPI_GENERIC = 5, EPI_F16_GELU = 6, EPI_F32_GATE = 7, EPI_F16_RES = 8 };

template <int RB, int CB>
__device__ __forceinline__ void epi_geglu(const float16_t (&acc)[RB][CB], const G16Args& g, int64_t row0, int col0, int wr, int wc, int lane) {
    static_assert(CB % 2 == 0, "GEGLU pairing needs an even number of column blocks per wave");
    const int hi = lane >> 5, lc = lane & 31;
#pragma unroll
    for (int p = 0; p < CB / 2; ++p) {
        const int gb  = col0 / 32 + wc * CB + 2 * p;
        const int oc0 = ((gb >> 2) * 2 + ((gb & 3) >> 1)) * 32;
        if (oc0 >= g.geglu_inner) continue;
        const float bx = g.ep.bias ? g.ep.bias[oc0 + lc] : 0.f, bg = g.ep.bias ? g.ep.bias[g.geglu_inner + oc0 + lc] : 0.f;
// ... 173 lines not shown
            }
        }
    }
}

template <int BM, int RB, int CB>
__device__ __forceinline__ void epi_dispatch_linear(const float16_t (&acc)[RB][CB], const G16Args& g, int64_t row0, int col0, int wr, int wc, int lane) {
    const bool full = row0 + BM <= g.R;
    if (g.geglu_inner > 0 && g.geglu16) {
        epi_geglu16(acc, g, row0, col0, wr, wc, lane);
    } else if (CB % 2 == 0 && g.geglu_inner > 0) {
        if constexpr (CB % 2 == 0) epi_geglu(acc, g, row0, col0, wr, wc, lane);
    } else if (g.hm_d > 0 && g.hm_L >= 32 && !g.ep.residual && (g.dst != nullptr) != (g.dst16 != nullptr)) {
        if (g.dst16)
            epi_linear<EPI_HM_F16>(acc, g, row0, col0, wr, wc, lane);
        else
            epi_linear<EPI_HM_F32>(acc, g, row0, col0, wr, wc, lane);
    } else if (g.ep.gate) {
        epi_linear<EPI_F32_GATE>(acc, g, row0, col0, wr, wc, lane);
    } else if (full && g.hm_d == 0 && g.dst && !g.dst16) {
        if (g.ep.residual)
            epi_linear<EPI_F32_RES>(acc, g, row0, col0, wr, wc, lane);
        else
            epi_linear<EPI_F32>(acc, g, row0, col0, wr, wc, lane);
    } else if (g.hm_d == 0 && g.dst16 && !g.dst && g.ep.residual && !g.ep.gelu) {
        epi_linear<EPI_F16_RES>(acc, g, row0, col0, wr, wc, lane);
    } else if (g.hm_d == 0 && g.dst16 && !g.dst && !g.ep.residual) {
        if (g.ep.gelu)
            epi_linear<EPI_F16_GELU>(acc, g, row0, col0, wr, wc, lane);
        else
            epi_linear<EPI_F16>(acc, g, row0, col0, wr, wc, lane);
    } else {
        epi_linear<EPI_GENERIC>(acc, g, row0, col0, wr, wc, lane);
    }
}


template <int MODE, int RB, int CB>
__device__ __forceinline__ void epi_conv(const float16_t (&acc)[RB][CB], const G16Args& g, int64_t row0, int col0, int wr, int wc, int lane) {
    const int hi = lane >> 5, lc = lane & 31;
    const uint32_t ohow = (uint32_t)g.OHOW;
#pragma unroll
    for (int rb = 0; rb < RB; ++rb) {
        const int64_t pos_base = row0 + wr * (RB * 32) + rb * 32;
        if (pos_base >= g.R) continue;
        const uint32_t img0 = (uint32_t)pos_base / ohow, p0 = (uint32_t)pos_base - img0 * ohow;
        uint32_t pl = p0 + lc, dimg = 0;
        while (pl >= ohow) {
            pl -= ohow;
            ++dimg;
        }
        if (pos_base + lc >= g.R) continue;
        const uint32_t le = dimg * (uint32_t)g.C * ohow + pl + 4u * hi * ohow;
#pragma unroll
        for (int cb = 0; cb < CB; ++cb) {
            const int cblk = col0 + (wc * CB + cb) * 32;
            if (cblk >= g.C) continue;
            const int64_t ub = ((int64_t)img0 * g.C + cblk) * g.OHOW;
            const float* pb  = g.ep.bias ? g.ep.bias + cblk : nullptr;
            const uint32_t cld = g.ep.chan_ld ? (uint32_t)g.ep.chan_ld : (uint32_t)g.C;
            const float* pc  = g.ep.chan_add ? g.ep.chan_add + (int64_t)img0 * cld + cblk : nullptr;
#pragma unroll
            for (int r0 = 0; r0 < 16; r0 += 8) {
                float bv[8], rv[8];
#pragma unroll
                for (int r = r0; r < r0 + 8; ++r) {
                    const int ro  = (r & 3) + 8 * (r >> 2);
                    const bool ok = MODE != 2 || cblk + ro + 4 * hi < g.C;
                    bv[r - r0]    = (pb && ok) ? ld_u(pb + ro, 16u * hi) : 0.f;
                    if (pc && ok) bv[r - r0] += ld_u(pc + ro, (4u * hi + dimg * cld) * 4u);
                    rv[r - r0]    = ((MODE == 1 || (MODE == 2 && g.ep.residual)) && ok) ? ld_u(g.ep.residual + ub + (int64_t)ro * g.OHOW, le * 4u) : 0.f;
                }
#pragma unroll
                for (int r = r0; r < r0 + 8; ++r) {
                    const int ro = (r & 3) + 8 * (r >> 2);
                    if (MODE == 2 && cblk + ro + 4 * hi >= g.C) continue;
                    st_u(g.dst + ub + (int64_t)ro * g.OHOW, le * 4u, acc[rb][cb][r] * g.ep.scale + bv[r - r0] + rv[r - r0]);
                }
            }
        }
    }
}

}
```

stable-diffusion.cpp_amd/csrc/kernels/gemm16.hip:

```cpp
#include <atomic>
#include <cstdio>
#include <cstdlib>
#include <mutex>
#include <type_traits>
#include <utility>
#include <vector>
#include "device_utils.h"
#include "kernels.h"
#include "ktime.h"
#include "g16_common.h"

namespace mi355x {

template <int BM, int BN, bool CONV, int BK, int NST, int WR, int WC, int PIPE = 0, bool SK = false, int QT = 0>
__global__ __launch_bounds__(WR * WC * 64, PIPE ? 2 : 2) void k_gemm16(G16Args g) {
    static_assert(!SK || (PIPE == 1 && !CONV), "stream-K is written for the pipelined Linear tiles");
    static_assert(QT == 0 || ((QT == 8 || QT == 4) && PIPE == 1 && !CONV && !SK && BM == 256 && (BN == 256 || BN == 192) && WR * WC == 8), "in-loop dequantisation: pipelined 256 x 256 / 256 x 192 Linear tiles");
    constexpr int NW  = WR * WC;
    constexpr int RB  = BM / WR / 32;
    constexpr int CB  = BN / WC / 32;
    static_assert(RB * WR * 32 == BM && CB * WC * 32 == BN, "tile must split into 32x32 blocks per wave");
    constexpr int ROWB   = BK * 2;
    constexpr int SLOTS  = ROWB / 16;
    constexpr int RPP    = 1024 / ROWB;
    constexpr int ABYTES = BM * ROWB;
    constexpr int KSTEPS = BK / 16;
    constexpr int NF     = (BN / 32) * KSTEPS;
    constexpr int APW    = (ABYTES / 1024) / NW;
    constexpr int WPW    = (NF + NW - 1) / NW;
    constexpr int WEXTRA = NF % NW;
    constexpr int BBYTES = NF * 1024;
    constexpr int NPT    = APW + WPW;
    static_assert(APW * NW * 1024 == ABYTES && APW >= 1, "A stage must split evenly over the waves");
    constexpr int QBLK  = QT == 8 ? 34 : 18;
    constexpr int QPB   = QT == 8 ? 64 : 32;
    constexpr int QNP   = QPB / 16;
    constexpr int QTOFF = 2 * QBLK - 16;
    constexpr int QVC   = 256;
    constexpr int QRAWB = QVC * (QPB + 16);
    constexpr int QNRAW = 3;
    constexpr int QPI   = QT ? QVC * QNP / (NW * 64) : 0;
    constexpr int QRQ   = QPI + 1;
    constexpr int QB0   = NST * ABYTES;
    constexpr int QR0   = QB0 + 2 * BBYTES;
    constexpr int SMEMB = QT ? QR0 + QNRAW * QRAWB : NST * (ABYTES + BBYTES);
    static_assert(SMEMB <= 160 * 1024, "LDS budget");
    __shared__ __attribute__((aligned(1024))) char smem[SMEMB];

    const int lane0 = threadIdx.x & 63;
    const int wave = __builtin_amdgcn_readfirstlane(threadIdx.x >> 6);
    const int wr = wave % WR, wc = wave / WR;

    int64_t sk_u = 0, sk_end = 0;
    int sk_w = 0;
    int dp_t = 0, dp_end = 0;
    if constexpr (SK) {
        const int64_t U = (int64_t)(g.sk_tiles - g.sk_dp) * g.nt;
        sk_w            = (g.sk_grid & 7) == 0 ? (int)(blockIdx.x & 7) * (g.sk_grid >> 3) + (int)(blockIdx.x >> 3) : (int)blockIdx.x;
        sk_u            = (int64_t)sk_w * U / g.sk_grid;
        sk_end          = (int64_t)(sk_w + 1) * U / g.sk_grid;
        const int per   = g.sk_dp / g.sk_grid;
        dp_t            = sk_w * per;
        dp_end          = dp_t + per;
    }
  for (bool sk_more = true; sk_more;) {
    int lane = lane0;
    if constexpr (SK) asm volatile("" : "+v"(lane));
    int bid = blockIdx.x, kslice = blockIdx.y;
    int kt0 = 0, nt = g.nt;
    if constexpr (SK) {
        if (sk_u < sk_end) {
            const int rt = (int)(sk_u / g.nt);
            bid          = g.sk_dp + rt;
            kt0          = (int)(sk_u - (int64_t)rt * g.nt);
            nt           = (int)min((int64_t)(g.nt - kt0), sk_end - sk_u);
            sk_u += nt;
        } else if (dp_t < dp_end) {
            bid = dp_t++;
        } else {
            break;
        }
        sk_more = sk_u < sk_end || dp_t < dp_end;
    } else {
        sk_more = false;
        g16_wg_order(g, g.multi > 1 ? g.ncol_tiles * g.multi : g.ncol_tiles, bid, kslice);
#ifdef MI355X_EXPERIMENTS
        if (g.abl == 7) nt = PIPE ? 4 : 1;
#endif
        if (g.split_k > 1) {
            kt0 = kslice * g.nt_slice;
            nt  = min(g.nt_slice, g.nt - kt0);
            if (!g.sk_cnt) g.dst += (int64_t)kslice * g.slab;
        }
    }
    const int nct_all  = g.multi > 1 ? g.ncol_tiles * g.multi : g.ncol_tiles;
    const int row_tile = bid / nct_all;
    int col_tile       = bid - row_tile * nct_all;
    if (!CONV && g.multi > 1) {
        const int wi = col_tile / g.ncol_tiles;
        col_tile -= wi * g.ncol_tiles;
#define G16_PICK(F, A)                                                                                                                                    \
    g.F = wi < 8 ? (wi < 4 ? (wi < 2 ? (wi == 0 ? g.A[0] : g.A[1]) : (wi == 2 ? g.A[2] : g.A[3])) : (wi < 6 ? (wi == 4 ? g.A[4] : g.A[5]) : (wi == 6 ? g.A[6] : g.A[7]))) \
                 : (wi < 12 ? (wi < 10 ? (wi == 8 ? g.A[8] : g.A[9]) : (wi == 10 ? g.A[10] : g.A[11]))                                                       \
                            : (wi < 14 ? (wi == 12 ? g.A[12] : g.A[13]) : (wi == 14 ? g.A[14] : g.A[15])))
        G16_PICK(W, Wm);
        G16_PICK(dst, dstm);
        G16_PICK(dst16, dst16m);
        G16_PICK(ep.bias, biasm);
#undef G16_PICK
    }
    const int64_t row0 = (CONV ? 0 : g.row_base) + (int64_t)row_tile * BM;
    const int col0     = col_tile * BN;

    auto rowswz = [](int r) { return SLOTS == 8 ? ((r >> 1) & 7) : ((r >> 2) & 3); };

    const _Float16* asrc[APW];
    unsigned a_mask[APW];
    int a_slot[APW];
#pragma unroll
    for (int q = 0; q < APW; ++q) {
        const int r  = (wave * APW + q) * RPP + lane / SLOTS;
        const int ls = (lane % SLOTS) ^ rowswz(r);
        a_slot[q]    = ls * 8;
        int64_t row  = row0 + r;
        if (!CONV) {
            if (row >= g.R) row = g.R - 1;
            if (g.a_runL > 0) row = (int64_t)((uint32_t)row / (uint32_t)g.a_runL) * g.a_runS + (uint32_t)row % (uint32_t)g.a_runL;
            asrc[q] = g.A + row * g.lda + ls * 8;
        } else {
            const bool ok = row < g.R;
// ... 656 lines not shown
#pragma unroll
            for (int rb = 0; rb < RB; ++rb)
#pragma unroll
                for (int cb = 0; cb < CB; ++cb)
#pragma unroll
                    for (int i4 = 0; i4 < 4; ++i4) {
                        const u32x4_t v = __builtin_amdgcn_raw_buffer_load_b128(rs, sl * TILE_B + ((((wave * RB + rb) * CB + cb) * 4 + i4) * 64 + lane) * 16, 0, 16);
                        acc[rb][cb][4 * i4] += __uint_as_float(v[0]);
                        acc[rb][cb][4 * i4 + 1] += __uint_as_float(v[1]);
                        acc[rb][cb][4 * i4 + 2] += __uint_as_float(v[2]);
                        acc[rb][cb][4 * i4 + 3] += __uint_as_float(v[3]);
                    }
        }
    }

    if constexpr (SK) {
        __syncthreads();
        if (!(kt0 == 0 && nt == g.nt)) {
            typedef unsigned int u32x4_t __attribute__((ext_vector_type(4)));
            constexpr int TILE_B = BM * BN * 4;
            const int64_t U  = (int64_t)(g.sk_tiles - g.sk_dp) * g.nt, G = g.sk_grid;
            const int64_t uf = (int64_t)(bid - g.sk_dp) * g.nt;
            const int wf     = (int)(((uf + 1) * G - 1) / U), wl = (int)(((uf + g.nt) * G - 1) / U);
            const int nparts = wl - wf + 1;
            char* mine       = (char*)g.sk_slab + (int64_t)(2 * sk_w + (kt0 == 0 ? 1 : 0)) * TILE_B;
            {
                const auto rs = __builtin_amdgcn_make_buffer_rsrc((void*)mine, 0, TILE_B, 0x00020000);
#pragma unroll
                for (int rb = 0; rb < RB; ++rb)
#pragma unroll
                    for (int cb = 0; cb < CB; ++cb)
#pragma unroll
                        for (int i4 = 0; i4 < 4; ++i4) {
                            u32x4_t v;
                            v[0] = __float_as_uint(acc[rb][cb][4 * i4]);
                            v[1] = __float_as_uint(acc[rb][cb][4 * i4 + 1]);
                            v[2] = __float_as_uint(acc[rb][cb][4 * i4 + 2]);
                            v[3] = __float_as_uint(acc[rb][cb][4 * i4 + 3]);
                            __builtin_amdgcn_raw_buffer_store_b128(v, rs, ((((wave * RB + rb) * CB + cb) * 4 + i4) * 64 + lane) * 16, 0, 16);
                        }
            }
            asm volatile("s_waitcnt vmcnt(0)" ::: "memory");
            __syncthreads();
            int* flag = (int*)smem;
            if (threadIdx.x == 0) *flag = __hip_atomic_fetch_add(&g.sk_cnt[bid - g.sk_dp], 1, __ATOMIC_RELAXED, __HIP_MEMORY_SCOPE_AGENT) == nparts - 1;
            __syncthreads();
            const int last = *flag;
            __syncthreads();
            if (!last) continue;
#pragma unroll
            for (int rb = 0; rb < RB; ++rb)
#pragma unroll
                for (int cb = 0; cb < CB; ++cb) acc[rb][cb] = (float16_t){0};
            for (int p = 0; p < nparts; ++p) {
                const char* part = (const char*)g.sk_slab + (int64_t)(p == 0 ? 2 * wf + 1 : 2 * (wf + p)) * TILE_B;
                const auto rp    = __builtin_amdgcn_make_buffer_rsrc((void*)part, 0, TILE_B, 0x00020000);
#pragma unroll
                for (int rb = 0; rb < RB; ++rb)
#pragma unroll
                    for (int cb = 0; cb < CB; ++cb)
#pragma unroll
                        for (int i4 = 0; i4 < 4; ++i4) {
                            const u32x4_t v = __builtin_amdgcn_raw_buffer_load_b128(rp, ((((wave * RB + rb) * CB + cb) * 4 + i4) * 64 + lane) * 16, 0, 16);
                            acc[rb][cb][4 * i4] += __uint_as_float(v[0]);
                            acc[rb][cb][4 * i4 + 1] += __uint_as_float(v[1]);
                            acc[rb][cb][4 * i4 + 2] += __uint_as_float(v[2]);
                            acc[rb][cb][4 * i4 + 3] += __uint_as_float(v[3]);
                        }
            }
        }
    }

    if (!CONV) {
        if (PIPE == 1 && BN == 256 && g.split_col > 0) {
            const bool hi_part = col0 >= g.split_col;
            G16Args gs   = g;
            gs.dst       = hi_part ? nullptr : g.dst;
            gs.dst16     = hi_part ? g.split_dst16 : nullptr;
            gs.ldd16     = hi_part ? g.split_ldd16 : 0;
            gs.ep.gelu   = hi_part ? 1 : 0;
            epi_dispatch_linear<BM>(acc, gs, row0, col0, wr, wc, lane);
        } else
        epi_dispatch_linear<BM>(acc, g, row0, col0, wr, wc, lane);
    } else {
        const bool fullc = col0 + BN <= g.C;
        if (fullc) {
            if (g.ep.residual)
                epi_conv<1>(acc, g, row0, col0, wr, wc, lane);
            else
                epi_conv<0>(acc, g, row0, col0, wr, wc, lane);
        } else {
            epi_conv<2>(acc, g, row0, col0, wr, wc, lane);
        }
    }
  }
}

static inline int64_t rup64(int64_t a, int64_t b) { return (a + b - 1) / b * b; }

static int g_g16_variant = 3;
static int g_g16_tap_major = 0;
void gemm16_set_tap_major(int v) { g_g16_tap_major = v; }
int gemm16_tap_major() { return g_g16_tap_major; }
void gemm16_set_variant(int v) { g_g16_variant = v; }
static inline bool g16_bk32() { return g_g16_variant == 1 || g_g16_variant == 3; }

enum { G16_T128 = 0, G16_T256 = 1, G16_T256W = 2, G16_T160 = 3, G16_T160N = 4, G16_T320 = 5, G16_T256P = 6, G16_T128N64 = 7, G16_T192P = 8 };
static int g_g16_force_tile = -1;
void gemm16_set_tile(int t) { g_g16_force_tile = t; }
#ifdef MI355X_EXPERIMENTS
static int g_g16_abl = 0;
void gemm16_set_abl(int v) { g_g16_abl = v; }
#endif
static int g_g16_bn64 = 1;
void gemm16_set_bn64(int v) { g_g16_bn64 = v; }
static int g_g16_streamk = 0;
static int g_g16_t256p_min_nt_sk = 64, g_g16_t256p_min_tiles_sk = 192;
void gemm16_set_t256p_min_nt_sk(int v) { g_g16_t256p_min_nt_sk = v; }
void gemm16_set_t256p_min_tiles_sk(int v) { g_g16_t256p_min_tiles_sk = v; }
static int g_g16_t320 = 1;
void gemm16_set_t320(int v) { g_g16_t320 = v; }
int gemm16_split_k(int64_t rows, int64_t M, int64_t K, bool conv);
static int g16_t320_split(int64_t rows, int64_t M, int64_t nt, bool conv);
static int g_g16_t192p = 1;
void gemm16_set_t192p(int v) { g_g16_t192p = v; }
static int g_g16_t256p_pad = 1;
void gemm16_set_t256p_pad(int v) { g_g16_t256p_pad = v; }
static int g_g16_tail_split = 0;
void gemm16_set_tail_split(int v) { g_g16_tail_split = v; }
static bool g16_pad256_ok(int64_t M, int geglu, bool conv, int mul) {
    return g_g16_t256p_pad && !conv && mul == 1 && geglu == 0 && M % 128 == 0 && M % 256 != 0 && M >= 2048;
}
static int g16_num_cus();
static int g16_tail_rows(int64_t rows, int64_t M) {
    if (!g_g16_tail_split) return 0;
    const int64_t ncol = (M + 255) / 256, rt = (rows + 255) / 256, T = rt * ncol, full = T / g16_num_cus(), rem = T % g16_num_cus();
    if (full < 1 || rem == 0) return 0;
    const int64_t rtm = full * g16_num_cus() / ncol;
    if (rtm <= 0 || rtm >= rt) return 0;
    const int64_t tail_rows = rows - rtm * 256, tail_wgs = ((tail_rows + 127) / 128) * ((M + 127) / 128);
    const double tail_cost = tail_wgs <= 256 ? 0.5 : (tail_wgs <= 512 ? 0.75 : 1.25 * (double)((tail_wgs + 767) / 768));
    const double main_cost = (double)((rtm * ncol + g16_num_cus() - 1) / g16_num_cus());
    return (main_cost + tail_cost < (double)(full + 1) * 0.95) ? (int)rtm : 0;
}
static int g16_pick_tile(int64_t rows, int64_t M, int geglu, bool conv, int split, int64_t nt, int mul = 1) {
    if (g_g16_variant != 3) return G16_T128;
    const bool can160 = M % 160 == 0 && geglu != 1;
    const bool can320 = M % 320 == 0 && geglu != 1;
    if (g_g16_force_tile >= 0) {
        if (g_g16_force_tile == G16_T320) return can320 ? G16_T320 : G16_T256;
        if (g_g16_force_tile == G16_T256P) return M % 256 == 0 ? G16_T256P : G16_T256;
        if (g_g16_force_tile == G16_T192P) return ((M % 192 == 0 || (M % 64 == 0 && M >= 2048)) && !conv && geglu == 0 && !split) ? G16_T192P : G16_T256;
        if ((g_g16_force_tile == G16_T160 || g_g16_force_tile == G16_T160N) && !can160) return G16_T256;
        return g_g16_force_tile > G16_T256P ? G16_T128 : g_g16_force_tile;
    }
    const int64_t rt256 = (rows + 255) / 256, c128 = ((rows + 127) / 128) * ((M + 127) / 128) * mul, c256 = rt256 * ((M + 127) / 128) * mul;
    if (g_g16_force_tile < 0 && !split && g_g16_t320 && !can320 && (M % 256 == 0 || g16_pad256_ok(M, geglu, conv, mul))) {
        const int64_t c256p = rt256 * ((M + 255) / 256) * mul;
        int64_t rounds      = (c256p + 255) / 256;
        if (!conv && mul == 1 && geglu == 0 && g16_tail_rows(rows, M) > 0) rounds = c256p / 256;
        const bool sk_ok = g_g16_streamk == 2 && !conv && mul == 1 && c256p * nt >= 256 * 16;
        const bool ok256 = nt >= (sk_ok ? g_g16_t256p_min_nt_sk : 64) && c256p >= (sk_ok ? g_g16_t256p_min_tiles_sk : 192) && (sk_ok || c256p * 4 >= rounds * 256 * 3);
        if (g_g16_t192p && !conv && mul == 1 && geglu == 0 && (M % 192 == 0 || (g_g16_t256p_pad && M % 64 == 0 && M >= 2048)) && !sk_ok && nt >= 64) {
            const int64_t c192 = rt256 * ((M + 191) / 192), r192 = (c192 + 255) / 256;
            const bool ok192   = c192 >= 192 && c192 * 4 >= r192 * 256 * 3;
            if (ok192 && (!ok256 || (double)r192 * 0.80 < (double)rounds * 0.97)) return G16_T192P;
// ... 13 lines not shown
    if (c256 >= 256 && cost256 < best) {
        best = cost256;
        tile = G16_T256;
    }
    if (c160 >= 512 && (double)((c160 + 511) / 512) * 1.52 < best) tile = conv ? G16_T160 : G16_T160N;
    else if (tile == G16_T128 && c160 >= 256 && c160 < 512 && c128 <= 768) tile = G16_T160N;
    return tile;
}

bool gemm16_split_col_supported(int64_t rows, int64_t M, int64_t K);
int gemm16_geglu_mode(int64_t rows, int64_t M, int64_t K);
static bool g16_use_bn64(int64_t rows, int64_t M, int mul);
void gemm16_set_streamk(int v) { g_g16_streamk = v; }
static int g16_num_cus() {
    static const int n = [] {
        int dev = 0, cus = 0;
        if (hipGetDevice(&dev) != hipSuccess || hipDeviceGetAttribute(&cus, hipDeviceAttributeMultiprocessorCount, dev) != hipSuccess || cus <= 0) cus = 256;
        return cus;
    }();
    return n;
}
static int g16_streamk_grid(int64_t rows, int64_t M, int64_t K, bool geglu, int* tiles_out = nullptr, int* bn_out = nullptr, int* dp_out = nullptr) {
    if (!g_g16_streamk || g_g16_variant != 3 || !g16_bk32() || g_g16_force_tile >= 0) return 0;
    const int64_t nt = rup64(K, 64) / 32;
    if (!geglu && gemm16_split_k(rows, M, K, false) > 1) return 0;
    const int tile = g16_pick_tile(rows, M, geglu ? gemm16_geglu_mode(rows, M, K) : 0, false, 0, nt, 1);
    if (tile != G16_T256P) return 0;
    const int bn        = 256;
    const int64_t tiles = ((rows + 255) / 256) * ((M + bn - 1) / bn);
    const int cus       = g16_num_cus();
    const int64_t rounds = (tiles + cus - 1) / cus;
    if (tiles * nt < (int64_t)cus * 16 || tiles >= (1 << 20)) return 0;
    if (g_g16_streamk == 1 && (rounds < 2 || tiles * 100 >= rounds * cus * 85)) return 0;
    if (g_g16_streamk == 2 && tiles * 100 >= rounds * cus * 92) return 0;
    int64_t dp = 0;
    if (g_g16_streamk == 3) {
        dp = (tiles / cus) * cus;
        const int64_t rem = tiles - dp;
        if (dp == 0 || rem == 0 || rem * 4 > (int64_t)cus * 3 || rem * nt < (int64_t)cus * 12) return 0;
    }
    if (dp_out) *dp_out = (int)dp;
    if (tiles_out) *tiles_out = (int)tiles;
    if (bn_out) *bn_out = bn;
    return cus;
}

static int g_g16_geglu16 = 1;
void gemm16_set_geglu16(int v) { g_g16_geglu16 = v; }
int gemm16_geglu_mode(int64_t rows, int64_t M, int64_t K) {
    if (!g_g16_geglu16 || g_g16_variant != 3 || !g16_bk32() || g_g16_force_tile >= 0 || (M / 2) % 16 != 0) return 1;
    const int tile = g16_pick_tile(rows, M, 2, false, 0, rup64(K, 64) / 32, 1);
    return (tile == G16_T160 || tile == G16_T160N || tile == G16_T320) ? 2 : 1;
}
static int g_g16_qinloop_min_rows = 513;
void gemm16_set_qinloop_min_rows(int v) { g_g16_qinloop_min_rows = v; }
bool gemm16_qinloop_supported(int wtype, int64_t rows, int64_t M, int64_t K, int mul, int split) {
    if (g_g16_qinloop_min_rows <= 0 || rows < g_g16_qinloop_min_rows || (wtype != 8 && wtype != 2)) return false;
    if (g_g16_variant != 3 || !g16_bk32() || g_g16_force_tile >= 0 || g_g16_streamk) return false;
    if (K % 64 != 0 || K < 192 || g16_use_bn64(rows, M, mul)) return false;
    const int64_t nt = K / 32;
    if (split > 1 || gemm16_split_k(rows, M, K, false) > 1) return false;
    const int tile = g16_pick_tile(rows, M, 0, false, 0, nt, mul);
    return (tile == G16_T256P || tile == G16_T192P) && M % 64 == 0;
}
bool gemm16_split_col_supported(int64_t rows, int64_t M, int64_t K) {
    if (g_g16_variant != 3 || !g16_bk32() || M % 256 != 0 || M % 160 == 0 || g16_use_bn64(rows, M, 1)) return false;
    const int64_t nt = rup64(K, 64) / 32;
    return gemm16_split_k(rows, M, K, false) == 1 && g16_pick_tile(rows, M, false, false, 0, nt, 1) == G16_T256P;
}

static int g_g16_conv_wmajor = 1;
void gemm16_set_conv_wmajor(int v) { g_g16_conv_wmajor = v; }
int gemm16_worder_rows(const G16Args& g, unsigned gx, unsigned ny) {
    if (!g_g16_conv_wmajor || g.KS == 0 || g.ncol_tiles <= 0 || g.multi > 1 || g.sk_grid > 0) return 0;
    if (gx % 8 != 0 || gx % (unsigned)g.ncol_tiles != 0 || ((unsigned)g.ncol_tiles * ny) % 8 != 0) return 0;
    const int nrow = (int)(gx / (unsigned)g.ncol_tiles);
    if (nrow < 2) return 0;
    const int64_t imgs = g.OHOW > 0 ? g.R / g.OHOW : 1;
    const double act   = (double)imgs * g.H * g.Wd * g.ICp * 2.0;
    const double wts   = (double)g.ICp * g.KS * g.KS * (double)rup64(g.C, 128) * 2.0;
    return wts >= 2.0 * act ? nrow : 0;
}
static bool g16_trace();
template <int BN_, bool CONV_>
static void g16_launch(hipStream_t s, G16Args& g, int64_t rows, double flops, double bytes) {
    const unsigned ny = g.split_k > 1 ? (unsigned)g.split_k : 1u;
    const int mul     = (!CONV_ && g.multi > 1) ? g.multi : 1;
    if (BN_ == 128 && g_g16_variant == 3 && (!g.sk_cnt || g.sk_grid > 0)) {
        const int tile = g16_pick_tile(rows, g.C, g.geglu_inner > 0 ? (g.geglu16 ? 2 : 1) : 0, CONV_, g.split_k > 1 ? g.split_k : 0, g.nt, mul);
        if (g16_trace()) fprintf(stderr, "G16 tile %d rows=%lld C=%lld nt=%d split=%d mul=%d qt=%d\n", tile, (long long)rows, (long long)g.C, g.nt, g.split_k, mul, g.qt);
        if (g.qt && ((tile != G16_T256P && tile != G16_T192P) || g.sk_grid > 0 || g.C % 64 != 0 || g.nt < 6 || (g.nt & 1) || (g.split_k > 1 && ((g.nt_slice & 1) || g.nt_slice < 6 || g.nt - (g.split_k - 1) * g.nt_slice < 6)))) {
            fprintf(stderr, "ggml-mi355x: in-loop dequantisation planned for a launch that does not take the pipelined 256 x 256 tile (tile %d, rows %lld, M %lld, K stages %d)\n", tile, (long long)rows, (long long)g.C, g.nt);
            abort();
        }
        if (g.geglu_inner > 0 && g.geglu16 && tile != G16_T160 && tile != G16_T160N && tile != G16_T320) {
            fprintf(stderr, "ggml-mi355x: GEGLU launch planned on the 16-column interleave, but its tile takes the paired image\n");
            abort();
        }
        if constexpr (!CONV_) {
            if (g.sk_grid > 0) {
                KScope ks_(s, KF_LINEAR, flops, bytes);
                if (tile == G16_T256P) {
                    g.ncol_tiles = (int)((g.C + 255) / 256);
                    k_gemm16<256, 256, false, 32, 4, 4, 2, 1, true><<<dim3((unsigned)g.sk_grid, 1), 512, 0, s>>>(g);
                } else {
                    fprintf(stderr, "ggml-mi355x: stream-K launch planned for a shape that does not take a pipelined tile\n");
                    abort();
                }
                return;
            }
        }
        if constexpr (!CONV_) {
            const int rtm = (tile == G16_T256P && ny == 1 && mul == 1 && g.geglu_inner == 0 && !g.sk_cnt && g.split_col == 0 && !g.qt) ? g16_tail_rows(rows, g.C) : 0;
            if (rtm > 0) {
                const double fm = (double)((int64_t)rtm * 256) / (double)rows;
                G16Args t       = g;
                t.row_base      = g.row_base + (int64_t)rtm * 256;
                {
                    KScope ks_(s, KF_LINEAR, flops * fm, bytes * fm);
                    g.ncol_tiles = (int)((g.C + 255) / 256);
                    if (g.C % 256 != 0) g.wblk_lim = (int)(rup64(g.C, 128) / 32);
                    k_gemm16<256, 256, false, 32, 4, 4, 2, 1><<<dim3((unsigned)(rtm * g.ncol_tiles), 1), 512, 0, s>>>(g);
                }
                g16_launch<BN_, CONV_>(s, t, rows - (int64_t)rtm * 256, flops * (1.0 - fm), bytes * (1.0 - fm));
                return;
            }
        }
        if (tile != G16_T128) {
            const int64_t rt256 = (rows + 255) / 256;
            KScope ks_(s, CONV_ ? KF_CONV_T256 : KF_LINEAR, flops, bytes);
            if constexpr (CONV_) {
                G16Args t    = g;
                t.ncol_tiles = tile == G16_T320 ? (int)((g.C + 319) / 320) : (tile == G16_T256P ? (int)((g.C + 255) / 256) : ((tile == G16_T160 || tile == G16_T160N) ? (int)(g.C / 160) : g.ncol_tiles));
                g.worder     = gemm16_worder_rows(t, (unsigned)(rt256 * t.ncol_tiles * mul), ny);
            }
            if (tile == G16_T320) {
                g.ncol_tiles = (int)((g.C + 319) / 320);
#ifdef MI355X_EXPERIMENTS
                if (g_g16_abl == 1) {
                    k_gemm16<256, 320, CONV_, 32, 4, 4, 2, 2><<<dim3((unsigned)(rt256 * g.ncol_tiles * mul), ny), 512, 0, s>>>(g);
                    return;
                }
                if (g_g16_abl == 2) {
                    k_gemm16<256, 320, CONV_, 32, 4, 4, 2, 3><<<dim3((unsigned)(rt256 * g.ncol_tiles * mul), ny), 512, 0, s>>>(g);
                    return;
                }
                if (g_g16_abl == 3) {
                    k_gemm16<256, 320, CONV_, 32, 4, 4, 2, 4><<<dim3((unsigned)(rt256 * g.ncol_tiles * mul), ny), 512, 0, s>>>(g);
                    return;
                }
#endif
                k_gemm16<256, 320, CONV_, 32, 4, 4, 2, 1><<<dim3((unsigned)(rt256 * g.ncol_tiles * mul), ny), 512, 0, s>>>(g);
            } else if (tile == G16_T256P) {
                g.ncol_tiles = (int)((g.C + 255) / 256);
                if constexpr (!CONV_) {
                    if (g.qt) {
                        const dim3 grid((unsigned)(rt256 * g.ncol_tiles * mul), ny);
                        if (g.qt == 8)
                            k_gemm16<256, 256, false, 32, 4, 4, 2, 1, false, 8><<<grid, 512, 0, s>>>(g);
                        else
                            k_gemm16<256, 256, false, 32, 4, 4, 2, 1, false, 4><<<grid, 512, 0, s>>>(g);
                        return;
                    }
                    if (g.C % 256 != 0) g.wblk_lim = (int)(rup64(g.C, 128) / 32);
#ifdef MI355X_EXPERIMENTS
                    if (g_g16_abl == 1) {
                        k_gemm16<256, 256, false, 32, 4, 4, 2, 2><<<dim3((unsigned)(rt256 * g.ncol_tiles * mul), ny), 512, 0, s>>>(g);
                        return;
                    }
                    if (g_g16_abl == 2) {
                        k_gemm16<256, 256, false, 32, 4, 4, 2, 3><<<dim3((unsigned)(rt256 * g.ncol_tiles * mul), ny), 512, 0, s>>>(g);
                        return;
                    }
                    if (g_g16_abl == 5) {
                        k_gemm16<256, 256, false, 32, 4, 4, 2, 5><<<dim3((unsigned)(rt256 * g.ncol_tiles * mul), ny), 512, 0, s>>>(g);
                        return;
                    }
                    if (g_g16_abl == 6) {
                        k_gemm16<256, 256, false, 32, 4, 4, 2, 6><<<dim3((unsigned)(rt256 * g.ncol_tiles * mul), ny), 512, 0, s>>>(g);
                        return;
                    }
#endif
                }
                k_gemm16<256, 256, CONV_, 32, 4, 4, 2, 1><<<dim3((unsigned)(rt256 * g.ncol_tiles * mul), ny), 512, 0, s>>>(g);
            } else if (tile == G16_T192P) {
                g.ncol_tiles = (int)((g.C + 191) / 192);
                if (g.C % 192 != 0) g.wblk_lim = (int)(rup64(g.C, 128) / 32);
                if constexpr (!CONV_) {
                    const dim3 grid((unsigned)(rt256 * g.ncol_tiles * mul), ny);
                    if (g.qt == 8)
                        k_gemm16<256, 192, false, 32, 4, 4, 2, 1, false, 8><<<grid, 512, 0, s>>>(g);
                    else if (g.qt)
                        k_gemm16<256, 192, false, 32, 4, 4, 2, 1, false, 4><<<grid, 512, 0, s>>>(g);
                    else
                        k_gemm16<256, 192, false, 32, 4, 4, 2, 1><<<grid, 512, 0, s>>>(g);
                }
            } else if (tile == G16_T160) {
                g.ncol_tiles = (int)(g.C / 160);
                k_gemm16<256, 160, CONV_, 32, 3, 4, 1><<<dim3((unsigned)(rt256 * g.ncol_tiles * mul), ny), 256, 0, s>>>(g);
            } else if (tile == G16_T160N) {
                g.ncol_tiles = (int)(g.C / 160);
                k_gemm16<256, 160, CONV_, 32, 3, 8, 1><<<dim3((unsigned)(rt256 * g.ncol_tiles * mul), ny), 512, 0, s>>>(g);
            } else if (tile == G16_T256W) {
                k_gemm16<256, 128, CONV_, 32, 3, 2, 2><<<dim3((unsigned)(rt256 * g.ncol_tiles * mul), ny), 256, 0, s>>>(g);
            } else {
                k_gemm16<256, 128, CONV_, 32, 3, 4, 2><<<dim3((unsigned)(rt256 * g.ncol_tiles * mul), ny), 512, 0, s>>>(g);
            }
            return;
        }
    }
    const dim3 grid((unsigned)(((rows + 127) / 128) * g.ncol_tiles * mul), ny);
    KScope ks_(s, CONV_ ? KF_CONV_T128 : KF_LINEAR, flops, bytes);
    if (g_g16_variant == 0)
        k_gemm16<128, BN_, CONV_, 64, 2, 2, 2><<<grid, 256, 0, s>>>(g);
    else if (g_g16_variant == 2)
        k_gemm16<128, BN_, CONV_, 64, 3, 2, 2><<<grid, 256, 0, s>>>(g);
    else
        k_gemm16<128, BN_, CONV_, 32, 3, 2, 2><<<grid, 256, 0, s>>>(g);
}

static int g_g16_splitk_target = 384;
void gemm16_set_splitk_target(int v) { g_g16_splitk_target = v; }
static int g_g16_splitk_mid = 0;
void gemm16_set_splitk_mid(int v) { g_g16_splitk_mid = v; }
static int g_g16_t320_linear_max_split = 4;
void gemm16_set_t320_linear_max_split(int v) { g_g16_t320_linear_max_split = v; }
static int g16_t320_split(int64_t rows, int64_t M, int64_t nt, bool conv) {
    if (!g_g16_t320 || g_g16_variant != 3 || M % 320 != 0 || (g_g16_force_tile >= 0 && g_g16_force_tile != G16_T320)) return 0;
    const int64_t c320 = ((rows + 255) / 256) * (M / 320);
    if (c320 >= 192 || c320 < 8) return 0;
    int64_t S = 256 / c320;
    if (S > 16) S = 16;
    if (!conv && S > g_g16_t320_linear_max_split) return 0;
    const int64_t min_stages = rows <= 2048 ? 20 : 48;
    while (S > 1 && nt / S < min_stages) --S;
    return (S >= 2 && c320 * S >= 128) ? (int)S : 0;
}
int gemm16_split_k(int64_t rows, int64_t M, int64_t K, bool conv) {
    if (!g16_bk32()) return 1;
    const int64_t wgs = ((rows + 127) / 128) * ((M + 127) / 128);
    const int64_t nt  = rup64(K, 64) / 32;
    if (const int s320 = g16_t320_split(rows, M, nt, conv)) return s320;
    if (wgs > g_g16_splitk_target / 2) {
        if (g_g16_splitk_mid && wgs <= g_g16_splitk_target && nt >= 128) return 2;
        return 1;
    }
    int64_t S = g_g16_splitk_target / wgs;
    if (S > 8) S = 8;
    if (S > nt / 8) S = nt / 8;
    return S < 2 ? 1 : (int)S;
}

static int g_g16_sk_inkernel = 0;
void gemm16_set_splitk_inkernel(int v) { g_g16_sk_inkernel = v; }
static int g_g16_sk_in_target = 320;
void gemm16_set_splitk_in_target(int v) { g_g16_sk_in_target = v; }
static int g_g16_bn64_max = 128;
void gemm16_set_bn64_max(int v) { g_g16_bn64_max = v; }
static bool g16_use_bn64(int64_t rows, int64_t M, int mul) {
    const int64_t c128 = ((rows + 127) / 128) * ((M + 127) / 128) * mul;
    return M <= 64 || (M % 64 == 0 && g16_bk32() && (g_g16_force_tile == G16_T128N64 || (g_g16_force_tile < 0 && g_g16_bn64 && c128 <= g_g16_bn64_max)));
}
G16SplitPlan gemm16_split_plan(int64_t rows, int64_t M, int64_t K, bool conv, bool plain_out, bool geglu) {
    G16SplitPlan r{1, false, 0, 0};
    const int64_t nt = rup64(K, 64) / (g16_bk32() ? 32 : 64);
    if (!g16_bk32()) return r;
    if (!conv) {
        int tiles = 0, bn = 0;
        if (const int grid = g16_streamk_grid(rows, M, K, geglu, &tiles, &bn)) {
            r.S        = -grid;
            r.inkernel = true;
            r.tiles    = tiles;
            r.ws_bytes = (size_t)grid * 2 * 256 * bn * 4;
            return r;
        }
    }
    if (geglu) return r;
    if (g16_t320_split(rows, M, nt, conv) == 0 && (g_g16_sk_inkernel == 1 || (g_g16_sk_inkernel == 2 && !plain_out)) && g_g16_variant == 3 && g_g16_force_tile < 0) {
        const int bn        = (conv ? M <= 64 : g16_use_bn64(rows, M, 1)) ? 64 : 128;
        const int64_t tiles = ((rows + 127) / 128) * ((M + bn - 1) / bn);
        const int64_t c256 = ((rows + 255) / 256) * ((M + 127) / 128);
        if (tiles <= 384 && c256 < 256 && nt >= 16 && tiles < (1 << 20)) {
            int64_t S = (g_g16_sk_in_target + tiles / 2) / tiles;
            if (S > 4) S = 4;
            while (S > 1 && nt / S < 8) --S;
            if (S >= 2) {
                r.S        = (int)S;
                r.inkernel = true;
                r.tiles    = (int)tiles;
                r.ws_bytes = (size_t)tiles * S * 128 * bn * 4;
                return r;
            }
        }
// ... 395 lines not shown
            launch_splitk_reduce(s, dst, splitk_ws, S, rows * M, e.bias, 1, M, e.residual);
    }
}

void launch_gemm16_linear_multi(hipStream_t s, int n, float* const* dst, void* const* dst16, const void* a16, int64_t lda, const void* const* wswz, int64_t rows,
                               int64_t K, int64_t M, const float* const* bias, float scale, int hm_d, int hm_H, int hm_L) {
    if (n < 2 || n > 16) {
        fprintf(stderr, "ggml-mi355x: launch_gemm16_linear_multi takes 2..16 weights\n");
        abort();
    }
    G16Args g{};
    g.A     = (const _Float16*)a16;
    g.lda   = lda;
    const int64_t Kp = rup64(K, 64);
    g.kfr   = Kp / 16;
    g.ldd   = M;
    g.ldd16 = 0;
    g.hm_d  = hm_d;
    g.hm_H  = hm_H;
    g.hm_L  = hm_L;
    g.R     = rows;
    g.C     = M;
    g.nt    = (int)(Kp / (g16_bk32() ? 32 : 64));
    g.ep    = G16Epi{bias[0], nullptr, scale};
    g.multi = n;
    for (int i = 0; i < n; ++i) {
        g.Wm[i]     = (const half8_t*)wswz[i];
        g.dstm[i]   = dst[i];
        g.dst16m[i] = (_Float16*)dst16[i];
        g.biasm[i]  = bias[i];
    }
    g.W     = g.Wm[0];
    g.dst   = g.dstm[0];
    g.dst16 = g.dst16m[0];
    double out_b = 0.0;
    for (int i = 0; i < n; ++i) out_b += (double)rows * M * (dst16[i] ? 2.0 : 4.0);
    const double bytes = (double)rows * Kp * 2.0 + (double)n * Kp * rup64(M, 128) * 2.0 + out_b;
    if (g16_trace()) fprintf(stderr, "G16 linear x%d rows=%lld K=%lld M=%lld hm=%d\n", n, (long long)rows, (long long)K, (long long)M, hm_d);
    if (g16_use_bn64(rows, M, n)) {
        g.ncol_tiles = (int)((M + 63) / 64);
        g16_launch<64, false>(s, g, rows, 2.0 * n * rows * K * M, bytes);
    } else {
        g.ncol_tiles = (int)((M + 127) / 128);
        g16_launch<128, false>(s, g, rows, 2.0 * n * rows * K * M, bytes);
    }
}

void launch_gemm16_linear_geglu(hipStream_t s, void* dst16, const void* a16, int64_t lda, const void* wswz_geglu, int64_t rows, int64_t K, int64_t M,
                                const float* bias, float* splitk_ws, int* splitk_cnt, int splitk_S, int geglu_mode) {
    G16Args g{};
    g.A           = (const _Float16*)a16;
    g.lda         = lda;
    g.W           = (const half8_t*)wswz_geglu;
    const int64_t Kp = rup64(K, 64);
    g.kfr         = Kp / 16;
    g.dst16       = (_Float16*)dst16;
    g.geglu_inner = (int)(M / 2);
    g.geglu16     = geglu_mode == 2 ? 1 : 0;
    g.ldd16       = M / 2;
    g.R           = rows;
    g.C           = M;
    g.nt          = (int)(Kp / (g16_bk32() ? 32 : 64));
    g.ep          = G16Epi{bias, nullptr, 1.f};
    g.ncol_tiles  = (int)((M + 127) / 128);
#ifdef MI355X_EXPERIMENTS
    g.abl = g_g16_abl;
#endif
    if (splitk_ws && splitk_cnt && splitk_S < 0) {
        int tiles = 0, dp = 0;
        if (g16_streamk_grid(rows, M, K, true, &tiles, nullptr, &dp) != -splitk_S) {
            fprintf(stderr, "ggml-mi355x: stream-K plan and launch disagree (options changed between plan and launch?)\n");
            abort();
        }
        g.sk_grid  = -splitk_S;
        g.sk_tiles = tiles;
        g.sk_dp    = dp;
        g.sk_slab  = splitk_ws;
        g.sk_cnt   = splitk_cnt;
    }
    if (g16_trace()) fprintf(stderr, "G16 linear rows=%lld K=%lld M=%lld res=0 hm=0 f16out=1 geglu=1\n", (long long)rows, (long long)K, (long long)M);
    g16_launch<128, false>(s, g, rows, 2.0 * rows * K * M, (double)rows * rup64(K, 64) * 2.0 + (double)rup64(K, 64) * rup64(M, 128) * 2.0 + (double)rows * (M / 2) * 2.0);
}

void launch_gemm16_conv(hipStream_t s, float* dst, const void* x16_nhwc, const void* wswz, int64_t W, int64_t H, int64_t IC, int64_t N, int64_t OC, int ksize,
                        int stride, int pad, bool upscale2x, const Epilogue& e, float* splitk_ws, int* splitk_cnt, int splitk_S) {
    G16Args g{};
    g.A   = (const _Float16*)x16_nhwc;
    g.W   = (const half8_t*)wswz;
    g.ICp = (int)rup64(IC, 64);
    g.kfr = (int64_t)g.ICp * ksize * ksize / 16;
    g.dst = dst;
    g.H   = (int)H;
    g.Wd  = (int)W;
    const int CW = upscale2x ? (int)W * 2 : (int)W, CH = upscale2x ? (int)H * 2 : (int)H;
    g.OW   = (CW + 2 * pad - ksize) / stride + 1;
    g.OH   = (CH + 2 * pad - ksize) / stride + 1;
    g.OHOW = (int64_t)g.OW * g.OH;
    g.S    = stride;
    g.pad  = pad;
    g.UPS  = upscale2x ? 1 : 0;
    g.KS   = ksize;
    g.icb_per_tap = g.ICp / 64;
    g.tap_major   = g_g16_tap_major;
    g.nt   = ksize * ksize * g.icb_per_tap * (g16_bk32() ? 2 : 1);
    g.R    = g.OHOW * N;
    g.C    = OC;
    g.zero = zero_page();
    g16_check_epi(e);
    g.ep   = G16Epi{e.bias, e.residual, e.scale};
    g.ep.chan_add = e.chan_add;
    g.ep.chan_ld  = (int)e.chan_ld;
    const bool inker = splitk_ws && splitk_cnt != nullptr && splitk_S > 1;
    const int S      = inker ? splitk_S : (splitk_ws ? gemm16_split_k(g.R, OC, (int64_t)g.ICp * ksize * ksize, true) : 1);
    if (S > 1) {
        g.split_k  = S;
        g.nt_slice = (g.nt + S - 1) / S;
        if (inker) {
            g.sk_slab = splitk_ws;
            g.sk_cnt  = splitk_cnt;
        } else {
            g.slab = g.R * OC;
            g.dst  = splitk_ws;
            g.ep   = G16Epi{nullptr, nullptr, e.scale};
        }
    }
    const bool bn64 = OC <= 64;
    const double conv_bytes = (double)N * H * W * g.ICp * 2.0 + (double)g.ICp * ksize * ksize * rup64(OC, 128) * 2.0 + (double)g.R * OC * 4.0 * (e.residual ? 2.0 : 1.0);
    if (g16_trace())
        fprintf(stderr, "G16 conv rows=%lld K=%lld M=%lld res=%d ks=%d s=%d ups=%d hw=%lldx%lld ic=%lld\n", (long long)g.R, (long long)g.ICp * ksize * ksize, (long long)OC,
                e.residual ? 1 : 0, ksize, stride, g.UPS, (long long)W, (long long)H, (long long)IC);
    if (bn64) {
        g.ncol_tiles = (int)((OC + 63) / 64);
        g16_launch<64, true>(s, g, g.R, 2.0 * g.R * IC * ksize * ksize * OC, conv_bytes);
    } else {
        g.ncol_tiles = (int)((OC + 127) / 128);
        g16_launch<128, true>(s, g, g.R, 2.0 * g.R * IC * ksize * ksize * OC, conv_bytes);
    }
    if (S > 1 && !inker) {
        const bool gn_ok = (((uintptr_t)dst | (uintptr_t)splitk_ws | (uintptr_t)e.residual) & 15) == 0 && splitk_reduce_gn_supported(g.OHOW, OC, N, e.gn_groups);
        if (e.gn_scale && !gn_ok) g16_gn_contract_violation();
        if (e.gn_scale)
            launch_splitk_reduce_gn(s, dst, splitk_ws, S, g.OHOW, OC, N, e);
        else
            launch_splitk_reduce(s, dst, splitk_ws, S, g.R * OC, e.bias, g.OHOW, OC, e.residual, e.chan_add, e.chan_ld);
    }
}

__global__ void k_pack_rows_f16(_Float16* __restrict__ dst, const float* __restrict__ xin, int64_t R, int K, int Kp, int64_t xs, int64_t L, int64_t bs) {
    const int64_t n8 = R * (Kp / 8);
    for (int64_t i = blockIdx.x * (int64_t)blockDim.x + threadIdx.x; i < n8; i += (int64_t)gridDim.x * blockDim.x) {
        const int64_t r = i / (Kp / 8);
        const int k0    = (int)(i - r * (Kp / 8)) * 8;
        const float* x  = xin + (r / L) * bs + (r % L) * xs - r * xs;
        half8_t h;
        if (k0 + 8 <= K) {
            const float4 a = *(const float4*)(x + r * xs + k0), b = *(const float4*)(x + r * xs + k0 + 4);
            h[0] = (_Float16)a.x; h[1] = (_Float16)a.y; h[2] = (_Float16)a.z; h[3] = (_Float16)a.w;
            h[4] = (_Float16)b.x; h[5] = (_Float16)b.y; h[6] = (_Float16)b.z; h[7] = (_Float16)b.w;
        } else {
#pragma unroll
            for (int j = 0; j < 8; ++j) h[j] = (_Float16)(k0 + j < K ? x[r * xs + k0 + j] : 0.f);
        }
        *(half8_t*)(dst + r * Kp + k0) = h;
    }
}
void launch_pack_rows_f16(hipStream_t s, void* dst, const float* x, int64_t R, int64_t K, int64_t xs, int64_t L, int64_t bs) {
    KScope ks_(s, KF_PACK_F16, 0.0, (double)R * K * 4.0 + (double)R * rup64(K, 64) * 2.0);
    const int Kp = (int)rup64(K, 64);
    const int64_t n8 = R * (Kp / 8);
    int64_t blocks   = (n8 + 255) / 256;
    if (blocks > 8192) blocks = 8192;
    if (L <= 0) {
        L  = R;
        bs = 0;
    }
    k_pack_rows_f16<<<(unsigned)blocks, 256, 0, s>>>((_Float16*)dst, x, R, (int)K, Kp, xs, L, bs);
}

template <int GELU>
__global__ void k_pack_cols_f16(_Float16* __restrict__ dst, int64_t ld, const float* __restrict__ x, int64_t R, int K, int64_t xs) {
    const int K8     = K / 8;
    const int64_t n8 = R * K8;
    for (int64_t i = blockIdx.x * (int64_t)blockDim.x + threadIdx.x; i < n8; i += (int64_t)gridDim.x * blockDim.x) {
        const int64_t r = i / K8;
        const int k0    = (int)(i - r * K8) * 8;
        float4 a = *(const float4*)(x + r * xs + k0), b = *(const float4*)(x + r * xs + k0 + 4);
        if (GELU) {
            a.x = act_apply<UN_GELU>(a.x); a.y = act_apply<UN_GELU>(a.y); a.z = act_apply<UN_GELU>(a.z); a.w = act_apply<UN_GELU>(a.w);
            b.x = act_apply<UN_GELU>(b.x); b.y = act_apply<UN_GELU>(b.y); b.z = act_apply<UN_GELU>(b.z); b.w = act_apply<UN_GELU>(b.w);
        }
        half8_t h;
        h[0] = (_Float16)a.x; h[1] = (_Float16)a.y; h[2] = (_Float16)a.z; h[3] = (_Float16)a.w;
        h[4] = (_Float16)b.x; h[5] = (_Float16)b.y; h[6] = (_Float16)b.z; h[7] = (_Float16)b.w;
        *(half8_t*)(dst + r * ld + k0) = h;
    }
}
// ... 298 lines not shown
    }
    dummy = 0.f;
    block_sum2<NT / 64>(q, dummy, scratch);
    const float rstd = rsqrtf(q / (float)cnt + eps);
    for (int c = c0 + threadIdx.x; c < c1; c += NT) {
        const float sc            = (w ? w[c] : 1.f) * rstd;
        scale[(int64_t)n * C + c] = sc;
        shift[(int64_t)n * C + c] = (b ? b[c] : 0.f) - mean * sc;
    }
}
template <int NT>
__global__ __launch_bounds__(NT) void k_gn_stats_1pass(float* __restrict__ scale, float* __restrict__ shift, const float* __restrict__ x, int64_t hw, int C, int groups,
                                                       int cpg, float eps, const float* __restrict__ w, const float* __restrict__ b, const float* __restrict__ x2 = nullptr, int C1 = 0) {
    __shared__ float scratch[2 * (NT / 64)];
    const int gidx = blockIdx.x % groups, n = blockIdx.x / groups;
    const int c0 = gidx * cpg, c1 = min(c0 + cpg, C);
    if (c0 >= c1) return;
    const int64_t cnt = (int64_t)(c1 - c0) * hw;
    const float K     = gn_ld4(x, x2, C1, C, n, c0, hw, 0).x;
    float s1 = 0.f, s2 = 0.f;
    for (int64_t i = threadIdx.x; i < cnt / 4; i += NT) {
        const float4 v = gn_ld4(x, x2, C1, C, n, c0, hw, i);
        const float a = v.x - K, bb = v.y - K, c = v.z - K, d = v.w - K;
        s1 += (a + bb) + (c + d);
        s2 += (a * a + bb * bb) + (c * c + d * d);
    }
    block_sum2<NT / 64>(s1, s2, scratch);
    const float m1   = s1 / (float)cnt;
    const float mean = K + m1;
    const float var  = fmaxf(s2 / (float)cnt - m1 * m1, 0.f);
    const float rstd = rsqrtf(var + eps);
    for (int c = c0 + threadIdx.x; c < c1; c += NT) {
        const float sc            = (w ? w[c] : 1.f) * rstd;
        scale[(int64_t)n * C + c] = sc;
        shift[(int64_t)n * C + c] = (b ? b[c] : 0.f) - mean * sc;
    }
}
template <int NT>
__global__ __launch_bounds__(NT) void k_gn_stats_part(float* __restrict__ part, const float* __restrict__ x, int64_t hw, int C, int groups, int cpg, int P) {
    __shared__ float scratch[2 * (NT / 64)];
    const int p = blockIdx.x % P, slab = blockIdx.x / P;
    const int gidx = slab % groups, n = slab / groups;
    const int c0 = gidx * cpg, c1 = min(c0 + cpg, C);
    if (c0 >= c1) return;
    const int64_t n4 = (int64_t)(c1 - c0) * hw / 4;
    const float4* xs = (const float4*)(x + ((int64_t)n * C + c0) * hw);
    const float K    = ((const float*)xs)[0];
    const int64_t i0 = n4 * p / P, i1 = n4 * (p + 1) / P;
    float s1 = 0.f, s2 = 0.f;
    for (int64_t i = i0 + threadIdx.x; i < i1; i += NT) {
        const float4 v = xs[i];
        const float a = v.x - K, bb = v.y - K, c = v.z - K, d = v.w - K;
        s1 += (a + bb) + (c + d);
        s2 += (a * a + bb * bb) + (c * c + d * d);
    }
    block_sum2<NT / 64>(s1, s2, scratch);
    if (threadIdx.x == 0) {
        part[(int64_t)blockIdx.x * 2]     = s1;
        part[(int64_t)blockIdx.x * 2 + 1] = s2;
    }
}
__global__ __launch_bounds__(64) void k_gn_stats_final(float* __restrict__ scale, float* __restrict__ shift, const float* __restrict__ part, const float* __restrict__ x,
                                                       int64_t hw, int C, int groups, int cpg, int P, float eps, const float* __restrict__ w, const float* __restrict__ b) {
    const int slab = blockIdx.x, gidx = slab % groups, n = slab / groups;
    const int c0 = gidx * cpg, c1 = min(c0 + cpg, C);
    if (c0 >= c1) return;
    const int64_t cnt = (int64_t)(c1 - c0) * hw;
    float s1 = 0.f, s2 = 0.f;
    for (int p = 0; p < P; ++p) {
        s1 += part[((int64_t)slab * P + p) * 2];
        s2 += part[((int64_t)slab * P + p) * 2 + 1];
    }
    const float K    = x[((int64_t)n * C + c0) * hw];
    const float m1   = s1 / (float)cnt;
    const float mean = K + m1;
    const float var  = fmaxf(s2 / (float)cnt - m1 * m1, 0.f);
    const float rstd = rsqrtf(var + eps);
    for (int c = c0 + threadIdx.x; c < c1; c += 64) {
        const float sc            = (w ? w[c] : 1.f) * rstd;
        scale[(int64_t)n * C + c] = sc;
        shift[(int64_t)n * C + c] = (b ? b[c] : 0.f) - mean * sc;
    }
}
static int64_t g_gn_split_min = 1 << 16;
void gemm16_set_gn_split_min(int v) { g_gn_split_min = v <= 0 ? (1ll << 62) : (int64_t)v; }
int gn_stats_split(int64_t hw, int64_t C, int64_t N, int groups) {
    const int64_t cpg = (C + groups - 1) / groups, cnt = cpg * hw, slabs = N * groups;
    if (hw % 4 != 0 || C % groups != 0 || cnt < g_gn_split_min || slabs >= 128) return 0;
    int64_t P = 512 / slabs;
    if (P > 32) P = 32;
    while (P > 1 && cnt / 4 / P < 2048) P /= 2;
    return P >= 2 ? (int)P : 0;
}

bool gn_two_source_supported(const float* x, const float* x2, int64_t hw, int64_t C, int64_t C1, int groups) {
    const int64_t cnt = ((C + groups - 1) / groups) * hw;
    return hw % 4 == 0 && ((((uintptr_t)x) | ((uintptr_t)x2)) & 15) == 0 && C1 > 0 && C1 < C && (cnt <= 4 * 1024 * 16 || cnt >= 16384) && C * hw < (1ll << 31);
}
void launch_gn_stats(hipStream_t s, float* scale, float* shift, const float* x, int64_t hw, int64_t C, int64_t N, int groups, float eps, const float* w,
                     const float* b, const float* x2, int64_t C1, float* part) {
    KScope ks_(s, KF_GN_STATS, 0.0, (double)hw * C * N * 4.0);
    const int cpg       = (int)((C + groups - 1) / groups);
    const int64_t cnt   = (int64_t)cpg * hw;
    const bool v4       = hw % 4 == 0 && ((((uintptr_t)x) | ((uintptr_t)x2)) & 15) == 0;
    const unsigned grid = (unsigned)(N * groups);
    if (part && !x2 && v4) {
        if (const int P = gn_stats_split(hw, C, N, groups)) {
            k_gn_stats_part<1024><<<grid * (unsigned)P, 1024, 0, s>>>(part, x, hw, (int)C, groups, cpg, P);
            k_gn_stats_final<<<grid, 64, 0, s>>>(scale, shift, part, x, hw, (int)C, groups, cpg, P, eps, w, b);
            return;
        }
    }
    if (x2 && !gn_two_source_supported(x, x2, hw, C, C1, groups)) {
        fprintf(stderr, "ggml-mi355x: two-source GroupNorm statistics asked for a shape they do not take\n");
        abort();
    }
    if (v4 && cnt <= 4 * 256 * 4)
        k_gn_stats_reg<256, 4><<<grid, 256, 0, s>>>(scale, shift, x, hw, (int)C, groups, cpg, eps, w, b, x2, (int)C1);
    else if (v4 && cnt <= 4 * 1024 * 4)
        k_gn_stats_reg<1024, 4><<<grid, 1024, 0, s>>>(scale, shift, x, hw, (int)C, groups, cpg, eps, w, b, x2, (int)C1);
    else if (v4 && cnt <= 4 * 1024 * 16)
        k_gn_stats_reg<1024, 16><<<grid, 1024, 0, s>>>(scale, shift, x, hw, (int)C, groups, cpg, eps, w, b, x2, (int)C1);
    else if (v4 && cnt >= 16384)
        k_gn_stats_1pass<1024><<<grid, 1024, 0, s>>>(scale, shift, x, hw, (int)C, groups, cpg, eps, w, b, x2, (int)C1);
    else if (cnt >= 16384)
        k_gn_stats<1024><<<grid, 1024, 0, s>>>(scale, shift, x, hw, (int)C, groups, cpg, eps, w, b);
    else
        k_gn_stats<256><<<grid, 256, 0, s>>>(scale, shift, x, hw, (int)C, groups, cpg, eps, w, b);
}

__global__ __launch_bounds__(256) void k_nchw_to_nhwc_f16(_Float16* __restrict__ dst, const float* __restrict__ x, int64_t hw, int C, int Cp,
                                                          const float* __restrict__ scale, const float* __restrict__ shift, int silu, float post_mul, float* dst_f32) {
    __shared__ float tile[64][65];
    const int n  = blockIdx.z;
    const int p0 = blockIdx.x * 64, c0 = blockIdx.y * 64;
    const int tx = threadIdx.x & 63, ty = threadIdx.x >> 6;
    const float* xn = x + (int64_t)n * C * hw;
    for (int j = ty; j < 64; j += 4) {
        const int c = c0 + j, p = p0 + tx;
        float v = 0.f;
        if (c < C && p < hw) {
            v = xn[(int64_t)c * hw + p];
            if (scale) v = v * scale[(int64_t)n * C + c] + shift[(int64_t)n * C + c];
            if (silu == 1) v = act_apply<UN_SILU>(v);
            else if (silu == 2) v = act_apply<UN_RELU>(v);
            if (dst_f32) dst_f32[((int64_t)n * C + c) * hw + p] = v;
            v *= post_mul;
        }
        tile[j][tx] = v;
    }
    __syncthreads();
    _Float16* dn = dst + (int64_t)n * hw * Cp;
    for (int j = ty; j < 64; j += 4) {
        const int p = p0 + j, c = c0 + tx;
        if (p < hw && c < Cp) dn[(int64_t)p * Cp + c] = (_Float16)tile[tx][j];
    }
}
__global__ __launch_bounds__(256) void k_nchw_to_nhwc_f16_v4(_Float16* __restrict__ dst, const float* __restrict__ x, int64_t hw, int C, int Cp,
                                                             const float* __restrict__ scale, const float* __restrict__ shift, int silu,
                                                             const float* __restrict__ x2 = nullptr, int C1 = 0, _Float16* __restrict__ dst_raw = nullptr,
                                                             float post_mul = 1.f, float* dst_f32 = nullptr) {
    __shared__ uint32_t tile[64][33];
    __shared__ uint32_t tile_raw[64][33];
    const int n  = blockIdx.z;
    const int p0 = blockIdx.x * 64, c0 = blockIdx.y * 64;
    auto rowp = [&](int c) -> const float* {
        if (!x2) return x + ((int64_t)n * C + c) * hw;
        return c < C1 ? x + ((int64_t)n * C1 + c) * hw : x2 + ((int64_t)n * (C - C1) + (c - C1)) * hw;
    };
#pragma unroll
    for (int k = 0; k < 2; ++k) {
        const int item = threadIdx.x + 256 * k;
        const int cp = item >> 4, pq = (item & 15) * 4;
        const int c = c0 + 2 * cp, p = p0 + pq;
        float4 va = make_float4(0.f, 0.f, 0.f, 0.f), vb = va;
        if (p < hw) {
            if (c < C) va = *(const float4*)(rowp(c) + p);
            if (c + 1 < C) vb = *(const float4*)(rowp(c + 1) + p);
        }
        float a[4] = {va.x, va.y, va.z, va.w}, bq[4] = {vb.x, vb.y, vb.z, vb.w};
        if (dst_raw) {
#pragma unroll
            for (int i = 0; i < 4; ++i) {
                const _Float16 hu = (_Float16)(c < C ? a[i] : 0.f), hv = (_Float16)(c + 1 < C ? bq[i] : 0.f);
// ... 82 lines not shown
```

stable-diffusion.cpp_amd/csrc/kernels/kernels.h:

```cpp
#pragma once
#include <hip/hip_runtime.h>
#include <stddef.h>
#include <stdint.h>

namespace mi355x {

struct View4 {
    const void* data;
    int64_t ne[4];
    int64_t nb[4];
    int type;
};

enum BinOp { BIN_ADD = 0, BIN_SUB = 1, BIN_MUL = 2, BIN_DIV = 3 };
enum UnOp { UN_SILU = 0, UN_GELU = 1, UN_GELU_QUICK = 2, UN_SIGMOID = 3, UN_TANH = 4, UN_RELU = 5, UN_NEG = 6, UN_EXP = 7 };

void launch_binary(hipStream_t s, BinOp op, void* dst, const int64_t dnb[4], const View4& a, const View4& b);
void launch_unary(hipStream_t s, UnOp op, float* dst, const float* src, int64_t n);
void launch_scale(hipStream_t s, float* dst, const float* src, int64_t n, float scale, float bias);
void launch_copy(hipStream_t s, const View4& dst, const View4& src);
void launch_concat(hipStream_t s, const View4& dst, const View4& a, const View4& b, int dim);
void launch_repeat(hipStream_t s, const View4& dst, const View4& src);
void launch_concat_heads(hipStream_t s, void* out, bool out_f16, const float* a, const float* b, int64_t d, int64_t H, int64_t La, int64_t Lb, int64_t N);
bool joint_heads_supported(int64_t d);
void launch_joint_heads(hipStream_t s, void* out, bool out_f16, const float* a, int64_t xsa, const float* wa, const float* b, int64_t xsb, const float* wb, float eps,
                        int64_t d, int64_t H, int64_t La, int64_t Lb, int64_t N, const float* pe = nullptr);
void launch_rope_pairs(hipStream_t s, float* out, const View4& x, const float* pe);
void launch_upscale_nearest(hipStream_t s, const View4& dst, const View4& src);
void launch_pad(hipStream_t s, const View4& dst, const View4& src, const int32_t pads[8]);
void launch_get_rows(hipStream_t s, float* dst, const int64_t dnb[4], const View4& table, const View4& ids);
void launch_timestep_embedding(hipStream_t s, float* dst, const float* t, int n, int dim, int max_period, int64_t dst_row_stride);
void launch_geglu(hipStream_t s, float* dst, const float* x, int64_t tokens, int64_t inner, int64_t x_stride);

void launch_group_norm(hipStream_t s, float* dst, const float* x, int64_t hw, int64_t C, int64_t N, int groups, float eps,
                       const float* w, const float* b, bool silu);
void launch_layer_norm(hipStream_t s, float* dst, const float* x, int64_t ne0, int64_t nrows, int64_t x_stride, int64_t d_stride,
                       float eps, const float* w, const float* b, bool rms);
void launch_layer_norm_4d(hipStream_t s, float* dst, const float* x, const int64_t ne[4], const int64_t xnb[4], const int64_t dnb[4], float eps, const float* w,
                          const float* b, bool rms);
void launch_soft_max(hipStream_t s, float* dst, const float* x, int64_t ncols, int64_t nrows, float scale, const View4* mask,
                     int64_t rows_per_mat);
void launch_soft_max_rows_f16(hipStream_t s, void* dst16, const float* x, int64_t ncols, int64_t nrows);

void launch_mul_mat_generic(hipStream_t s, float* dst, const int64_t dne[4], const int64_t dnb[4], const View4& a, const View4& b);
void launch_im2col_f16(hipStream_t s, void* dst, int dst_type, const View4& x, int64_t KW, int64_t KH, int64_t OW, int64_t OH,
                       int s0, int s1, int p0, int p1, int d0, int d1);

size_t wswz_bytes(int64_t R, int64_t K);
void launch_wswz_linear(hipStream_t s, void* dst, const void* src, int src_type, int64_t K, int64_t R, int64_t src_row_bytes, int64_t geglu_inner = 0);
void launch_wswz_conv(hipStream_t s, void* dst, const void* src, int64_t KW, int64_t KH, int64_t IC, int64_t OC, int kblk = 0);

struct Epilogue {
    const float* bias     = nullptr;
    const float* residual = nullptr;
    const float* chan_add = nullptr;
    int64_t chan_ld       = 0;
    float scale           = 1.0f;
    int act               = -1;
    float* gn_scale       = nullptr;
    float* gn_shift       = nullptr;
    const float* gn_w     = nullptr;
    const float* gn_b     = nullptr;
    int gn_groups         = 0;
    float gn_eps          = 0.f;
    void* ln_dst16        = nullptr;
    const float* ln_w     = nullptr;
    const float* ln_b     = nullptr;
    float ln_eps          = 0.f;
    const float* gate     = nullptr;
    int gate_L            = 0;
    int gelu              = 0;
    int64_t split_col     = 0;
    void* split_dst16     = nullptr;
    int64_t split_ldd16   = 0;
    int qtype             = 0;
    int64_t qrow_bytes    = 0;
    int64_t a_run_L       = 0;
    int64_t a_run_S       = 0;
};
void gemm16_init();
bool gemm16_qinloop_supported(int wtype, int64_t rows, int64_t M, int64_t K, int mul, int split);
void gemm16_set_qinloop_min_rows(int v);
void gemm16_set_t192p(int v);
void gemm16_set_tap_major(int v);
int gemm16_tap_major();
void gemm16_set_splitk_target(int v);
void gemm16_set_splitk_mid(int v);
void gemm16_set_tile(int t);
#ifdef MI355X_EXPERIMENTS
void gemm16_set_abl(int v);
#endif
void gemm16_set_t320(int v);
void gemm16_set_t256p_pad(int v);
void gemm16_set_conv_wmajor(int v);
void gemm16_set_ln16_rows(int v);
void gemm16_set_tail_split(int v);
void gemm16_set_bn64(int v);
void gemm16_set_variant(int v);
void launch_gemm16_linear(hipStream_t s, float* dst, void* dst16, int64_t ldd16, const void* a16, int64_t lda, const void* wswz, int64_t rows,
                          int64_t K, int64_t M, int64_t ldd, const Epilogue& ep, int hm_d = 0, int hm_H = 0, int hm_L = 0, float* splitk_ws = nullptr, int* splitk_cnt = nullptr, int splitk_S = 0);
void launch_gemm16_linear_multi(hipStream_t s, int n, float* const* dst, void* const* dst16, const void* a16, int64_t lda, const void* const* wswz, int64_t rows,
                               int64_t K, int64_t M, const float* const* bias, float scale, int hm_d, int hm_H, int hm_L);
void launch_gemm16_linear_geglu(hipStream_t s, void* dst16, const void* a16, int64_t lda, const void* wswz_geglu, int64_t rows, int64_t K, int64_t M,
                                const float* bias, float* splitk_ws = nullptr, int* splitk_cnt = nullptr, int splitk_S = 0, int geglu_mode = 1);
int gemm16_geglu_mode(int64_t rows, int64_t M, int64_t K);
void gemm16_set_bn64_max(int v);
void gemm16_set_geglu16(int v);
int gemm16_split_k(int64_t rows, int64_t M, int64_t K, bool conv);
bool splitk_reduce_gn_supported(int64_t hw, int64_t C, int64_t N, int groups);
bool splitk_reduce_ln_supported(int64_t rows, int64_t M);
void gemm16_set_t320_linear_max_split(int v);
struct G16SplitPlan {
    int S;
    bool inkernel;
    size_t ws_bytes;
    int tiles;
};
G16SplitPlan gemm16_split_plan(int64_t rows, int64_t M, int64_t K, bool conv, bool plain_out, bool geglu = false);
void gemm16_set_splitk_inkernel(int v);
void gemm16_set_splitk_in_target(int v);
void launch_gemm16_conv(hipStream_t s, float* dst, const void* x16_nhwc, const void* wswz, int64_t W, int64_t H, int64_t IC, int64_t N, int64_t OC,
                        int ksize, int stride, int pad, bool upscale2x, const Epilogue& ep, float* splitk_ws = nullptr, int* splitk_cnt = nullptr, int splitk_S = 0);
int conv3w_plan(int64_t W, int64_t H, int64_t IC, int64_t N, int64_t OC, int ksize, int stride, bool upscale2x, int* bn_out = nullptr);
void launch_conv3w(hipStream_t s, float* dst, const void* x16_nhwc, const void* wswz32, int64_t W, int64_t H, int64_t IC, int64_t N, int64_t OC, const Epilogue& ep,
                   float* splitk_ws, int S);
void qgemm16_set_rb(int v);
void conv3w_set_prio(int v);
void conv3w_set(int v);
void conv3w_set_min_blocks(int v);
void conv3w_set_min_blocks_deep(int v);
void launch_pack_rows_f16(hipStream_t s, void* dst, const float* x, int64_t R, int64_t K, int64_t xs, int64_t L = 0, int64_t bs = 0);
void launch_pack_cols_f16(hipStream_t s, void* dst, int64_t ld, const float* x, int64_t R, int64_t K, int64_t xs, bool gelu);
void launch_layer_norm_f16(hipStream_t s, void* dst, const float* x, int64_t ne0, int64_t nrows, int64_t x_stride, float eps, const float* w,
                           const float* b, bool rms, int64_t mod_L = 0);
void launch_geglu_f16(hipStream_t s, void* dst, const float* x, int64_t tokens, int64_t inner, int64_t x_stride);
bool gn_two_source_supported(const float* x, const float* x2, int64_t hw, int64_t C, int64_t C1, int groups);
void launch_gn_stats(hipStream_t s, float* scale, float* shift, const float* x, int64_t hw, int64_t C, int64_t N, int groups, float eps,
                     const float* w, const float* b, const float* x2 = nullptr, int64_t C1 = 0, float* part = nullptr);
int gn_stats_split(int64_t hw, int64_t C, int64_t N, int groups);
void gemm16_set_gn_split_min(int v);
void launch_nchw_to_nhwc_f16(hipStream_t s, void* dst, const float* x, int64_t hw, int64_t C, int64_t N, const float* scale, const float* shift,
                             int act, const float* x2 = nullptr, int64_t C1 = 0, void* dst_raw = nullptr, float post_mul = 1.f, float* dst_f32 = nullptr);

bool qgemv_supported(int wtype, int64_t rows, int64_t K);
void qgemv_set_max_rows(int v);
size_t qgemv_workspace_bytes(int64_t rows, int64_t K);
void launch_qgemv_group(hipStream_t s, float* dst, int64_t Mtot, const float* x, int64_t xs, int64_t rows, const void* members_dev, int n_members, int wtype, int64_t K,
                        float pre_scale, bool pre_silu);
size_t qgemv_member_bytes();
void qgemv_fill_member(void* host_entry, const void* W, const float* bias, int start);
void launch_qgemv(hipStream_t s, float* dst, int64_t ldd, const float* x, int64_t xs, int64_t rows, const void* wraw, int wtype, int64_t K, int64_t M, void* ws,
                  const Epilogue& ep, float pre_scale, bool pre_silu = false);

bool fgemv_supported(int wtype, int64_t rows, int64_t K);
void fgemv_set_max_rows(int v);
void launch_fgemv(hipStream_t s, float* dst, int64_t ldd, const float* x, int64_t xs, int64_t rows, const void* w, int wtype, int64_t K, int64_t M, const Epilogue& ep,
                  bool pre_silu);
bool qgemm16_supported(int wtype, int64_t rows, int64_t K, int64_t M);
int qgemm16_split_k(int64_t rows, int64_t K, int64_t M);
bool wswz_q_supported(int wtype, int64_t K);
void launch_wswz_q(hipStream_t s, void* dst, const void* wraw, int wtype, int64_t K, int64_t R);
void qgemm16_set_max_rows(int v);
void launch_qgemm16(hipStream_t s, float* dst, void* dst16, int64_t ldd16, const void* a16, int64_t lda, int64_t rows, const void* wraw, int wtype, int64_t K,
                    int64_t M, const Epilogue& ep, float* splitk_ws = nullptr, int splitk_S = 1);
void splitk_reduce_rows(hipStream_t s, float* dst, const float* ws, int S, int64_t n, const float* bias, int64_t C, const float* residual);

bool flash_attn_supported(int64_t D, int64_t DV);
struct FlashOut {
    float* dst       = nullptr;
    int64_t nb_q = 0, nb_h = 0, nb_n = 0;
    int H            = 0;
    void* dst16      = nullptr;
    int64_t ld16     = 0;
};
void gemm16_set_t256p_min_nt_sk(int v);
void gemm16_set_t256p_min_tiles_sk(int v);
bool gemm16_split_col_supported(int64_t rows, int64_t M, int64_t K);
void gemm16_set_streamk(int v);
void launch_flash_attn(hipStream_t s, const FlashOut& out, const View4& q, const View4& k, const View4& v, float scale);
enum FlashVariant { FLASH_VAR_SHORT = 0, FLASH_VAR_QB2, FLASH_VAR_MSLOT, FLASH_VAR_GENERIC, FLASH_VAR_COUNT };
int64_t flash_attn_variant_launches(int variant);


struct CalibrationResult {
    float mfma_f16_tflops = 0.f, mfma_clock_mhz = 0.f, copy_tbs = 0.f, read_tbs = 0.f;
    int compute_units = 0;
};
bool calibrate_device(hipStream_t s, CalibrationResult* out);

}
```

Before: 376.2 it/s.

## Emit GroupNorm partial statistics from conv/linear epilogues and finalize without re-reading activations

Conv and NCHW-output linear GEMM epilogues now write per-256-position chunk mean/M2 records for each channel when their output feeds a GroupNorm. The later GroupNorm (and concat+GroupNorm) path then runs a small finalize kernel that merges these records in double precision instead of a stats kernel that re-reads the full fp32 activation. This removes one full activation read per GroupNorm, at the cost of extra epilogue work with cross-lane reductions, an LDS buffer, and a small record workspace. It only applies to non-split-K tiles of supported shapes, with aborts on contract violations.

```diff
diff --git a/include/ggml-mi355x.h b/include/ggml-mi355x.h
--- a/include/ggml-mi355x.h
+++ b/include/ggml-mi355x.h
@@ -70,6 +70,7 @@
     int64_t flash_qb2_launches;
     int64_t flash_mslot_launches;
     int64_t flash_generic_launches;
+    int64_t fused_gn_epilogue;
 };
 GGML_MI355X_API void ggml_backend_mi355x_get_stats(struct ggml_backend_mi355x_stats* out);
 GGML_MI355X_API int ggml_backend_mi355x_resolve_enums(const char* (*op_name)(int), const char* (*unary_op_name)(int), const char* (*type_name)(int));
diff --git a/stable-diffusion.cpp_amd/__init__.py b/stable-diffusion.cpp_amd/__init__.py
--- a/stable-diffusion.cpp_amd/__init__.py
+++ b/stable-diffusion.cpp_amd/__init__.py
@@ -308,7 +308,7 @@
 _BACKEND_STAT_FIELDS = ("graphs_computed plans_built nodes_seen kernels_planned kernels_launched fused_conv fused_conv_bounced fused_linear "
                         "fused_norm fused_geglu fused_attention generic_matmul swizzled_weight_bytes graph_replays fused_linear_geglu "
                         "split_k_gemms head_major_gemms fused_modulate fused_gate fused_gelu fused_rope fused_concat_heads qgemv_linears fused_chan_add fused_proj_tokens gemm_attention fused_q16 split_k_inlaunch qgemm16_linears fgemv_linears fused_presilu fused_sibling_linears hoisted_kv_linears window_convs hoisted_emb_linears fused_rows16 fused_joint_qkv jit_images fused_cat_rows16 fused_gn_stats fused_ln_reduce redirect_fallbacks fused_concat_gn fused_conv_scale view_graphs plans_evicted hoisted_mod_linears view_external_nodes qinloop_linears flash_out_alias flash_slice_images "
-                        "flash_short_launches flash_qb2_launches flash_mslot_launches flash_generic_launches").split()
+                        "flash_short_launches flash_qb2_launches flash_mslot_launches flash_generic_launches fused_gn_epilogue").split()
 
 
 class BackendStats(C.Structure):
diff --git a/stable-diffusion.cpp_amd/csrc/backend/planner.cpp b/stable-diffusion.cpp_amd/csrc/backend/planner.cpp
--- a/stable-diffusion.cpp_amd/csrc/backend/planner.cpp
+++ b/stable-diffusion.cpp_amd/csrc/backend/planner.cpp
@@ -132,7 +132,7 @@
 #define STAT(field) g_stat_counters[offsetof(ggml_backend_mi355x_stats, field) / sizeof(int64_t)]
 
 struct Options {
-    std::atomic<int> fusion{1}, mfma_gemm{1}, hip_graph{1}, flash_pattern{1}, fuse_modulate{1}, fuse_gate{1}, fuse_gelu{1}, fuse_rope{1}, fuse_concat_heads{1}, qgemv{1}, fuse_chan_add{1}, fuse_proj_tokens{1}, fuse_q16{1}, qgemm16{1}, fgemv{1}, fuse_siblings{1}, hoist_kv{1}, hoist_emb{1}, fuse_rows16{0}, fuse_cat_rows16{1}, fuse_joint_qkv{1}, jit_qimages{4096}, fuse_gn_stats{1}, fuse_ln_reduce{1}, relax_res_overlap{1}, fuse_split_gelu{1}, fuse_concat_gn{1}, fuse_gn_tokens{1}, fuse_linear_nchw{1}, fuse_conv_scale{1}, ignore_use_counts{0}, plan_cache_cap{512}, hoist_mod{1}, fuse_flash_slices{1}, fuse_act_pack{1};
+    std::atomic<int> fusion{1}, mfma_gemm{1}, hip_graph{1}, flash_pattern{1}, fuse_modulate{1}, fuse_gate{1}, fuse_gelu{1}, fuse_rope{1}, fuse_concat_heads{1}, qgemv{1}, fuse_chan_add{1}, fuse_proj_tokens{1}, fuse_q16{1}, qgemm16{1}, fgemv{1}, fuse_siblings{1}, hoist_kv{1}, hoist_emb{1}, fuse_rows16{0}, fuse_cat_rows16{1}, fuse_joint_qkv{1}, jit_qimages{4096}, fuse_gn_stats{1}, fuse_ln_reduce{1}, relax_res_overlap{1}, fuse_split_gelu{1}, fuse_concat_gn{1}, fuse_gn_tokens{1}, fuse_linear_nchw{1}, fuse_conv_scale{1}, ignore_use_counts{0}, plan_cache_cap{512}, hoist_mod{1}, fuse_flash_slices{1}, fuse_act_pack{1}, fuse_gn_epilogue{1};
 } g_opt;
 
 using Step = std::function<void(hipStream_t)>;
@@ -408,6 +408,19 @@
     float mul = 1.f;
     int64_t runL = 0, runS = 0;
 };
+
+static bool feeds_group_norm(const GInfo& gi, int j) {
+    const ggml_tensor* res = gi.node(j);
+    for (int k : gi.consumers[j]) {
+        const ggml_tensor* c = gi.node(k);
+        if (gi.done[k]) continue;
+        if (xop(c) == GGML_OP_GROUP_NORM && c->src[0] == res) return true;
+        if (xop(c) == GGML_OP_CONCAT && c->op_params[0] == 2 && (c->src[0] == res || c->src[1] == res))
+            for (int k2 : gi.consumers[k])
+                if (xop(gi.node(k2)) == GGML_OP_GROUP_NORM && gi.node(k2)->src[0] == c) return true;
+    }
+    return false;
+}
 
 struct Builder {
     Planner* P;
@@ -451,6 +464,7 @@
         float eps;
     };
     std::unordered_map<const ggml_tensor*, GnPre> gn_pre;
+    std::unordered_map<const ggml_tensor*, size_t> gn_rec;
     struct LnPre {
         size_t off;
         const float *w, *b;
@@ -1062,9 +1076,14 @@
         const int64_t HWt = nchw_HW, Nimg = nchw_N;
         const float* resp       = nchw_res;
         const Builder::Split sk = B.plan_split(tokens, M, rup64(K), true, true);
+        const bool rec_want = g_opt.fuse_gn_epilogue && feeds_group_norm(gi, nchw_add);
+        const bool rec_on  = sk.S <= 1 && rec_want && gemm16_conv_gn_rec_supported(HWt, Nimg, M, rup64(K), 1);
+        const size_t rec_o = rec_on ? B.alloc((size_t)Nimg * (HWt / GN_REC_CHUNK) * M * sizeof(GnRec)) : 0;
+        if (rec_on) B.gn_rec[gi.node(nchw_add)] = rec_o;
         B.emit_at(emit_node, i, [=](hipStream_t st) {
             Epilogue e2 = ep;
             e2.residual = resp;
+            if (rec_on) e2.gn_rec = (GnRec*)(P->arena + rec_o);
             launch_gemm16_conv(st, ndst, P->arena + off, swz, HWt, 1, K, Nimg, M, 1, 1, 0, false, e2, sk.ws(P), sk.cnt(P), sk.S);
         });
         STAT(fused_linear)++;
@@ -1770,6 +1789,7 @@
             gnp = Builder::GnPre{0, (const float*)gi.node(j1)->src[1]->data, (const float*)gi.node(j2)->src[1]->data, g->op_params[0], ggml_abi_op_param_f32(g, 1)};
         }
     }
+    const bool rec_want = g_opt.fuse_gn_epilogue && g_opt.fusion && token_major_out < 0 && feeds_group_norm(gi, last);
     auto gn_register = [&](int S) -> bool {
         if (S <= 1 || !gnp.groups) return false;
         if ((((uintptr_t)final_dst | (uintptr_t)ep.residual) & 15) != 0) return false;
@@ -1829,10 +1849,15 @@
         const size_t wsoff = w3S > 1 ? B.alloc((size_t)w3S * opos * OC * 4) : 0;
         if (w3S > 1) STAT(split_k_gemms)++;
         const bool gn_on = gn_register(w3S);
+        const int64_t ohw  = opos / N;
+        const bool rec_on  = w3S == 1 && rec_want && conv3w_gn_rec_supported(ohw, OC, N);
+        const size_t rec_o = rec_on ? B.alloc((size_t)N * (ohw / GN_REC_CHUNK) * OC * sizeof(GnRec)) : 0;
+        if (rec_on) B.gn_rec[gi.node(last)] = rec_o;
         B.emit_at(emit_node, i, [=](hipStream_t st) {
             Epilogue e2 = ep;
             if (emb_arena) e2.chan_add = (const float*)(P->arena + emb_off);
             if (gn_on) gn_fill(e2, gnp, P->arena, N * OC);
+            if (rec_on) e2.gn_rec = (GnRec*)(P->arena + rec_o);
             launch_conv3w(st, final_dst, P->arena + off, swz, SW, SH, IC, N, OC, e2, w3S > 1 ? (float*)(P->arena + wsoff) : nullptr, w3S);
         });
         STAT(fused_conv)++;
@@ -1841,10 +1866,15 @@
     }
     const Builder::Split sk = B.plan_split(opos, OC, rup64(IC) * ks * ks, true, true);
     const bool gn_on        = sk.inkernel ? false : gn_register(sk.S);
+    const int64_t ohw  = opos / N;
+    const bool rec_on  = sk.S <= 1 && rec_want && gemm16_conv_gn_rec_supported(ohw, N, OC, rup64(IC), ks);
+    const size_t rec_o = rec_on ? B.alloc((size_t)N * (ohw / GN_REC_CHUNK) * OC * sizeof(GnRec)) : 0;
+    if (rec_on) B.gn_rec[gi.node(last)] = rec_o;
     B.emit_at(emit_node, i, [=](hipStream_t st) {
         Epilogue e2 = ep;
         if (emb_arena) e2.chan_add = (const float*)(P->arena + emb_off);
         if (gn_on) gn_fill(e2, gnp, P->arena, N * OC);
+        if (rec_on) e2.gn_rec = (GnRec*)(P->arena + rec_o);
         launch_gemm16_conv(st, final_dst, P->arena + off, swz, SW, SH, IC, N, OC, ks, st_, pd, upscale, e2, sk.ws(P), sk.cnt(P), sk.S);
     });
     STAT(fused_conv)++;
@@ -1931,12 +1961,17 @@
         const bool have  = pre != B.gn_pre.end() && pre->second.w == w && pre->second.b == b && pre->second.groups == groups && pre->second.eps == eps;
         const size_t so  = have ? pre->second.off : B.alloc((size_t)N * C * 4 * 2);
         const size_t off = B.alloc((size_t)N * hw * rup64(C) * 2);
-        const int gsp    = have ? 0 : gn_stats_split(hw, C, N, groups);
+        const auto rec   = B.gn_rec.find(x);
+        const bool byrec = !have && g_opt.fuse_gn_epilogue && rec != B.gn_rec.end();
+        const size_t ro  = byrec ? rec->second : 0;
+        const int gsp    = (have || byrec) ? 0 : gn_stats_split(hw, C, N, groups);
         const size_t po  = gsp ? B.alloc((size_t)N * groups * gsp * 2 * 4) : 0;
+        if (byrec) STAT(fused_gn_epilogue)++;
         B.emit([=](hipStream_t st) {
             float* sc = (float*)(P->arena + so);
             float* sh = sc + N * C;
-            if (!have) launch_gn_stats(st, sc, sh, xp, hw, C, N, groups, eps, w, b, nullptr, 0, gsp ? (float*)(P->arena + po) : nullptr);
+            if (byrec) launch_gn_finalize(st, sc, sh, (const GnRec*)(P->arena + ro), nullptr, hw, C, C, N, groups, eps, w, b);
+            else if (!have) launch_gn_stats(st, sc, sh, xp, hw, C, N, groups, eps, w, b, nullptr, 0, gsp ? (float*)(P->arena + po) : nullptr);
             launch_nchw_to_nhwc_f16(st, P->arena + off, xp, hw, C, N, sc, sh, false);
         });
         chain.push_back(gi.sole(last));
@@ -1953,12 +1988,17 @@
         const bool have     = pre != B.gn_pre.end() && pre->second.w == w && pre->second.b == b && pre->second.groups == groups && pre->second.eps == eps;
         const size_t so     = have ? pre->second.off : B.alloc((size_t)N * C * 4 * 2);
         const size_t off    = B.alloc((size_t)N * hw * rup64(C) * 2);
-        const int gsp       = have ? 0 : gn_stats_split(hw, C, N, groups);
+        const auto rec      = B.gn_rec.find(x);
+        const bool byrec    = !have && g_opt.fuse_gn_epilogue && rec != B.gn_rec.end();
+        const size_t ro     = byrec ? rec->second : 0;
+        const int gsp       = (have || byrec) ? 0 : gn_stats_split(hw, C, N, groups);
         const size_t po     = gsp ? B.alloc((size_t)N * groups * gsp * 2 * 4) : 0;
+        if (byrec) STAT(fused_gn_epilogue)++;
         B.emit([=](hipStream_t st) {
             float* sc = (float*)(P->arena + so);
             float* sh = sc + N * C;
-            if (!have) launch_gn_stats(st, sc, sh, xp, hw, C, N, groups, eps, w, b, nullptr, 0, gsp ? (float*)(P->arena + po) : nullptr);
+            if (byrec) launch_gn_finalize(st, sc, sh, (const GnRec*)(P->arena + ro), nullptr, hw, C, C, N, groups, eps, w, b);
+            else if (!have) launch_gn_stats(st, sc, sh, xp, hw, C, N, groups, eps, w, b, nullptr, 0, gsp ? (float*)(P->arena + po) : nullptr);
             launch_nchw_to_nhwc_f16(st, P->arena + off, xp, hw, C, N, sc, sh, silu, nullptr, 0, nullptr, conv_mul);
         });
         STAT(kernels_planned)++;
@@ -2017,10 +2057,15 @@
     const size_t roff = jc >= 0 ? B.alloc((size_t)N * hw * rup64(C) * 2) : 0;
     const float *ap = (const float*)a->data, *bp = (const float*)b->data;
     const bool raw  = jc >= 0;
+    const auto ra = B.gn_rec.find(a), rb = B.gn_rec.find(b);
+    const bool byrec = g_opt.fuse_gn_epilogue && ra != B.gn_rec.end() && rb != B.gn_rec.end();
+    const size_t roa = byrec ? ra->second : 0, rob = byrec ? rb->second : 0;
+    if (byrec) STAT(fused_gn_epilogue)++;
     B.emit([=](hipStream_t st) {
         float* sc = (float*)(P->arena + so);
         float* sh = sc + N * C;
-        launch_gn_stats(st, sc, sh, ap, hw, C, N, groups, eps, w, bb, bp, C1);
+        if (byrec) launch_gn_finalize(st, sc, sh, (const GnRec*)(P->arena + roa), (const GnRec*)(P->arena + rob), hw, C, C1, N, groups, eps, w, bb);
+        else launch_gn_stats(st, sc, sh, ap, hw, C, N, groups, eps, w, bb, bp, C1);
         launch_nchw_to_nhwc_f16(st, P->arena + off, ap, hw, C, N, sc, sh, silu, bp, C1, raw ? (void*)(P->arena + roff) : nullptr);
     });
     B.packed[gi.node(last)] = Packed{off, rup64(C), true};
@@ -3722,6 +3767,7 @@
     OPT(fuse_rows16),
     OPT(fuse_cat_rows16),
     OPT(fuse_gn_stats),
+    OPT(fuse_gn_epilogue),
     OPT(fuse_joint_qkv),
     OPT(fuse_ln_reduce),
     OPT(jit_qimages),
diff --git a/stable-diffusion.cpp_amd/csrc/kernels/conv3w.hip b/stable-diffusion.cpp_amd/csrc/kernels/conv3w.hip
--- a/stable-diffusion.cpp_amd/csrc/kernels/conv3w.hip
+++ b/stable-diffusion.cpp_amd/csrc/kernels/conv3w.hip
@@ -256,6 +256,15 @@
         C3_MAIN(NPBMAX);
     }
 
+    if (g.ep.gn_rec) {
+        static_assert(4 * BN * (int)sizeof(GnRec) <= WBUF, "the tile's records fit one window buffer");
+        GnRec* lds = (GnRec*)(smem + (wb ^ 1) * WBUF);
+        if (g.ep.residual)
+            epi_conv_gn<true, BN, 4, 2, CB>(acc, g, row0, col0, wr, wc, lane, lds);
+        else
+            epi_conv_gn<false, BN, 4, 2, CB>(acc, g, row0, col0, wr, wc, lane, lds);
+        return;
+    }
     if (g.ep.residual)
         epi_conv<1>(acc, g, row0, col0, wr, wc, lane);
     else
@@ -293,6 +302,8 @@
     if (bn_out) *bn_out = bn;
     return S;
 }
+
+bool conv3w_gn_rec_supported(int64_t OHOW, int64_t OC, int64_t N) { return OHOW % GN_REC_CHUNK == 0 && OC % 32 == 0 && N > 0; }
 
 template <int TW, int BN>
 static void c3_launch(hipStream_t s, const G16Args& g, unsigned tiles, unsigned ny) {
@@ -340,6 +351,13 @@
     g.ep.chan_add = e.chan_add;
     g.ep.chan_ld  = (int)e.chan_ld;
     g.ncol_tiles  = (int)(OC / bn);
+    if (e.gn_rec) {
+        if ((S > 1 && splitk_ws) || !conv3w_gn_rec_supported(g.OHOW, OC, N)) {
+            fprintf(stderr, "ggml-mi355x: conv3w asked for a GroupNorm side band on a launch it does not serve (split %d, %lld positions per image)\n", S, (long long)g.OHOW);
+            abort();
+        }
+        g.ep.gn_rec = e.gn_rec;
+    }
     if (S > 1 && splitk_ws) {
         g.split_k  = S;
         g.nt_slice = (g.nt + S - 1) / S;
diff --git a/stable-diffusion.cpp_amd/csrc/kernels/g16_common.h b/stable-diffusion.cpp_amd/csrc/kernels/g16_common.h
--- a/stable-diffusion.cpp_amd/csrc/kernels/g16_common.h
+++ b/stable-diffusion.cpp_amd/csrc/kernels/g16_common.h
@@ -13,7 +13,56 @@
     int gelu          = 0;
     const float* chan_add = nullptr;
     int chan_ld           = 0;
+    GnRec* gn_rec         = nullptr;
 };
+
+__device__ __forceinline__ void gn_merge(float& m, float& q, float m2, float q2, float hn) {
+    const float d = m2 - m;
+    q             = (q + q2) + (d * d) * hn;
+    m             = 0.5f * (m + m2);
+}
+template <int CTRL>
+__device__ __forceinline__ float gn_dpp(float v) { return __int_as_float(__builtin_amdgcn_update_dpp(0, __float_as_int(v), CTRL, 0xf, 0xf, true)); }
+template <int NP, int CTRL>
+__device__ __forceinline__ void gn_bfly(float (&m)[8], float (&q)[8], bool sel, float hn) {
+#pragma unroll
+    for (int j = 0; j < NP; ++j) {
+        const float km = sel ? m[j + NP] : m[j], kq = sel ? q[j + NP] : q[j];
+        const float sm = sel ? m[j] : m[j + NP], sq = sel ? q[j] : q[j + NP];
+        m[j] = km;
+        q[j] = kq;
+        gn_merge(m[j], q[j], gn_dpp<CTRL>(sm), gn_dpp<CTRL>(sq), hn);
+    }
+}
+__device__ __forceinline__ int gn_lane_chan(int lane) {
+    const int j = (lane >> 1) & 7, r = (lane & 16) ? j : j + 8;
+    return (r & 3) + 8 * (r >> 2) + 4 * (lane >> 5);
+}
+template <int RB>
+__device__ __forceinline__ void gn_wave_stats(const float (&v)[RB][16], int lane, float& mo, float& qo) {
+    static_assert(RB == 1 || RB == 2, "one or two row blocks per wave");
+    constexpr float n0 = (float)RB;
+    float m[8], q[8];
+#pragma unroll
+    for (int j = 0; j < 8; ++j) {
+        float ma = v[0][j + 8], qa = 0.f, mb = v[0][j], qb = 0.f;
+        if constexpr (RB == 2) {
+            gn_merge(ma, qa, v[1][j + 8], 0.f, 0.5f);
+            gn_merge(mb, qb, v[1][j], 0.f, 0.5f);
+        }
+        const auto sm = __builtin_amdgcn_permlane16_swap(__float_as_uint(ma), __float_as_uint(mb), false, false);
+        const auto sq = __builtin_amdgcn_permlane16_swap(__float_as_uint(qa), __float_as_uint(qb), false, false);
+        m[j] = __uint_as_float(sm[0]);
+        q[j] = __uint_as_float(sq[0]);
+        gn_merge(m[j], q[j], __uint_as_float(sm[1]), __uint_as_float(sq[1]), 0.5f * n0);
+    }
+    gn_bfly<4, 0x140>(m, q, (lane & 8) != 0, n0);
+    gn_bfly<2, 0x141>(m, q, (lane & 4) != 0, 2.f * n0);
+    gn_bfly<1, 0x1B>(m, q, (lane & 2) != 0, 4.f * n0);
+    gn_merge(m[0], q[0], gn_dpp<0xB1>(m[0]), gn_dpp<0xB1>(q[0]), 8.f * n0);
+    mo = m[0];
+    qo = q[0];
+}
 
 struct G16Args {
     const _Float16* A;
@@ -353,4 +402,61 @@
     }
 }
 
-}
+template <bool RES, int BN, int WR, int RB, int CB>
+__device__ __forceinline__ void epi_conv_gn(const float16_t (&acc)[RB][CB], const G16Args& g, int64_t row0, int col0, int wr, int wc, int lane, GnRec* lds) {
+    static_assert(WR * RB == 8 && (RB == 1 || RB == 2), "a 256-position tile");
+    const int hi = lane >> 5, lc = lane & 31;
+    const uint32_t ohow = (uint32_t)g.OHOW;
+    const uint32_t img0 = (uint32_t)(row0 / g.OHOW), p0 = (uint32_t)(row0 - (int64_t)img0 * g.OHOW);
+    const uint32_t le   = (uint32_t)(wr * (RB * 32) + lc) + 4u * hi * ohow;
+    const uint32_t cld  = g.ep.chan_ld ? (uint32_t)g.ep.chan_ld : (uint32_t)g.C;
+    const int chl = gn_lane_chan(lane);
+#pragma unroll
+    for (int cb = 0; cb < CB; ++cb) {
+        const int cblk   = col0 + (wc * CB + cb) * 32;
+        const int64_t ub = ((int64_t)img0 * g.C + cblk) * g.OHOW + p0;
+        const float* pb  = g.ep.bias ? g.ep.bias + cblk : nullptr;
+        const float* pc  = g.ep.chan_add ? g.ep.chan_add + (int64_t)img0 * cld + cblk : nullptr;
+        float v[RB][16];
+#pragma unroll
+        for (int r0 = 0; r0 < 16; r0 += 8) {
+            float bv[8], rv[RB][8];
+#pragma unroll
+            for (int r = r0; r < r0 + 8; ++r) {
+                const int ro = (r & 3) + 8 * (r >> 2);
+                bv[r - r0]   = pb ? ld_u(pb + ro, 16u * hi) : 0.f;
+                if (pc) bv[r - r0] += ld_u(pc + ro, 16u * hi);
+#pragma unroll
+                for (int rb = 0; rb < RB; ++rb) rv[rb][r - r0] = RES ? ld_u(g.ep.residual + ub + (int64_t)ro * g.OHOW + rb * 32, le * 4u) : 0.f;
+            }
+#pragma unroll
+            for (int r = r0; r < r0 + 8; ++r) {
+                const int ro = (r & 3) + 8 * (r >> 2);
+#pragma unroll
+                for (int rb = 0; rb < RB; ++rb) {
+                    v[rb][r] = acc[rb][cb][r] * g.ep.scale + bv[r - r0] + rv[rb][r - r0];
+                    st_u(g.dst + ub + (int64_t)ro * g.OHOW + rb * 32, le * 4u, v[rb][r]);
+                }
+            }
+        }
+        float m, q;
+        gn_wave_stats<RB>(v, lane, m, q);
+        if (!(lane & 1)) lds[wr * BN + (wc * CB + cb) * 32 + chl] = GnRec{m, q};
+    }
+    __syncthreads();
+    const int c = (wc * WR + wr) * 64 + lane;
+    if (c < BN) {
+        GnRec a[WR];
+#pragma unroll
+        for (int i = 0; i < WR; ++i) a[i] = lds[i * BN + c];
+        float hn = 16.f * RB;
+#pragma unroll
+        for (int st = 1; st < WR; st *= 2, hn *= 2.f)
+#pragma unroll
+            for (int i = 0; i < WR; i += 2 * st) gn_merge(a[i].mean, a[i].m2, a[i + st].mean, a[i + st].m2, hn);
+        const uint32_t chunks = ohow / (uint32_t)GN_REC_CHUNK, t = p0 / (uint32_t)GN_REC_CHUNK;
+        g.ep.gn_rec[((int64_t)img0 * chunks + t) * g.C + col0 + c] = a[0];
+    }
+}
+
+}
diff --git a/stable-diffusion.cpp_amd/csrc/kernels/gemm16.hip b/stable-diffusion.cpp_amd/csrc/kernels/gemm16.hip
--- a/stable-diffusion.cpp_amd/csrc/kernels/gemm16.hip
+++ b/stable-diffusion.cpp_amd/csrc/kernels/gemm16.hip
@@ -46,6 +46,8 @@
     constexpr int SMEMB = QT ? QR0 + QNRAW * QRAWB : NST * (ABYTES + BBYTES);
     static_assert(SMEMB <= 160 * 1024, "LDS budget");
     __shared__ __attribute__((aligned(1024))) char smem[SMEMB];
+    constexpr bool G16_GN_REC_TILE = CONV && BM == 256 && BN != 128 && ((WR == 4 && RB == 2) || (WR == 8 && RB == 1));
+    static_assert(!G16_GN_REC_TILE || WR * BN * (int)sizeof(GnRec) <= SMEMB, "the tile's records fit the staging ring");
 
     const int lane0 = threadIdx.x & 63;
     const int wave = __builtin_amdgcn_readfirstlane(threadIdx.x >> 6);
@@ -868,6 +870,14 @@
             epi_dispatch_linear<BM>(acc, gs, row0, col0, wr, wc, lane);
         } else
         epi_dispatch_linear<BM>(acc, g, row0, col0, wr, wc, lane);
+    } else if (G16_GN_REC_TILE && g.ep.gn_rec) {
+        if constexpr (G16_GN_REC_TILE) {
+            __syncthreads();
+            if (g.ep.residual)
+                epi_conv_gn<true, BN, WR, RB, CB>(acc, g, row0, col0, wr, wc, lane, (GnRec*)smem);
+            else
+                epi_conv_gn<false, BN, WR, RB, CB>(acc, g, row0, col0, wr, wc, lane, (GnRec*)smem);
+        }
     } else {
         const bool fullc = col0 + BN <= g.C;
         if (fullc) {
@@ -1047,6 +1057,14 @@
     return wts >= 2.0 * act ? nrow : 0;
 }
 static bool g16_trace();
+static bool g16_gn_rec_tile_ok(int tile, int64_t C, int64_t ohow, int ny) {
+    const int bn = (tile == G16_T160 || tile == G16_T160N) ? 160 : (tile == G16_T320 ? 320 : (tile == G16_T256P ? 256 : 0));
+    return bn > 0 && ny == 1 && C % bn == 0 && ohow % GN_REC_CHUNK == 0;
+}
+[[noreturn]] static void g16_gn_rec_contract_violation() {
+    fprintf(stderr, "ggml-mi355x: conv launch asked for a GroupNorm side band on a shape / tile it does not serve\n");
+    abort();
+}
 template <int BN_, bool CONV_>
 static void g16_launch(hipStream_t s, G16Args& g, int64_t rows, double flops, double bytes) {
     const unsigned ny = g.split_k > 1 ? (unsigned)g.split_k : 1u;
@@ -1090,6 +1108,9 @@
                 g16_launch<BN_, CONV_>(s, t, rows - (int64_t)rtm * 256, flops * (1.0 - fm), bytes * (1.0 - fm));
                 return;
             }
+        }
+        if constexpr (CONV_) {
+            if (g.ep.gn_rec && !g16_gn_rec_tile_ok(tile, g.C, g.OHOW, (int)ny)) g16_gn_rec_contract_violation();
         }
         if (tile != G16_T128) {
             const int64_t rt256 = (rows + 255) / 256;
@@ -1174,6 +1195,7 @@
             return;
         }
     }
+    if (CONV_ && g.ep.gn_rec) g16_gn_rec_contract_violation();
     const dim3 grid((unsigned)(((rows + 127) / 128) * g.ncol_tiles * mul), ny);
     KScope ks_(s, CONV_ ? KF_CONV_T128 : KF_LINEAR, flops, bytes);
     if (g_g16_variant == 0)
@@ -1735,6 +1757,11 @@
     g16_launch<128, false>(s, g, rows, 2.0 * rows * K * M, (double)rows * rup64(K, 64) * 2.0 + (double)rup64(K, 64) * rup64(M, 128) * 2.0 + (double)rows * (M / 2) * 2.0);
 }
 
+bool gemm16_conv_gn_rec_supported(int64_t OHOW, int64_t N, int64_t OC, int64_t ICp, int ksize) {
+    if (OC <= 64 || g_g16_variant != 3) return false;
+    const int64_t nt = (int64_t)ksize * ksize * (ICp / 64) * (g16_bk32() ? 2 : 1);
+    return g16_gn_rec_tile_ok(g16_pick_tile(OHOW * N, OC, 0, true, 0, nt, 1), OC, OHOW, 1);
+}
 void launch_gemm16_conv(hipStream_t s, float* dst, const void* x16_nhwc, const void* wswz, int64_t W, int64_t H, int64_t IC, int64_t N, int64_t OC, int ksize,
                         int stride, int pad, bool upscale2x, const Epilogue& e, float* splitk_ws, int* splitk_cnt, int splitk_S) {
     G16Args g{};
@@ -1765,6 +1792,8 @@
     g.ep.chan_ld  = (int)e.chan_ld;
     const bool inker = splitk_ws && splitk_cnt != nullptr && splitk_S > 1;
     const int S      = inker ? splitk_S : (splitk_ws ? gemm16_split_k(g.R, OC, (int64_t)g.ICp * ksize * ksize, true) : 1);
+    if (e.gn_rec && (S > 1 || OC <= 64)) g16_gn_rec_contract_violation();
+    g.ep.gn_rec = e.gn_rec;
     if (S > 1) {
         g.split_k  = S;
         g.nt_slice = (g.nt + S - 1) / S;
@@ -2229,6 +2258,50 @@
         shift[(int64_t)n * C + c] = (b ? b[c] : 0.f) - mean * sc;
     }
 }
+__device__ __forceinline__ double gn_wave_sum_f64(double v) {
+#pragma unroll
+    for (int o = 32; o > 0; o >>= 1) v += __shfl_xor(v, o, 64);
+    return v;
+}
+__global__ __launch_bounds__(64) void k_gn_finalize(float* __restrict__ scale, float* __restrict__ shift, const GnRec* __restrict__ r1, const GnRec* __restrict__ r2, int chunks,
+                                                    int C, int C1, int groups, int cpg, float eps, const float* __restrict__ w, const float* __restrict__ b) {
+    const int gidx = blockIdx.x % groups, n = blockIdx.x / groups;
+    const int c0 = gidx * cpg, c1 = min(c0 + cpg, C);
+    if (c0 >= c1) return;
+    const int nc = c1 - c0, nrec = nc * chunks;
+    auto rec = [&](int i) -> GnRec {
+        const int t = i / nc, c = c0 + (i - t * nc);
+        return c < C1 ? r1[((int64_t)n * chunks + t) * C1 + c] : r2[((int64_t)n * chunks + t) * (C - C1) + (c - C1)];
+    };
+    double s = 0.0;
+    for (int i = threadIdx.x; i < nrec; i += 64) s += (double)rec(i).mean;
+    const double mean = gn_wave_sum_f64(s) / (double)nrec;
+    double q = 0.0;
+    for (int i = threadIdx.x; i < nrec; i += 64) {
+        const GnRec r  = rec(i);
+        const double d = (double)r.mean - mean;
+        q += (double)r.m2 + (double)GN_REC_CHUNK * d * d;
+    }
+    const double var = gn_wave_sum_f64(q) / ((double)nrec * (double)GN_REC_CHUNK);
+    const float rstd = (float)(1.0 / sqrt(var + (double)eps));
+    for (int c = c0 + threadIdx.x; c < c1; c += 64) {
+        const float sc            = (w ? w[c] : 1.f) * rstd;
+        scale[(int64_t)n * C + c] = sc;
+        shift[(int64_t)n * C + c] = (b ? b[c] : 0.f) - (float)mean * sc;
+    }
+}
+void launch_gn_finalize(hipStream_t s, float* scale, float* shift, const GnRec* r1, const GnRec* r2, int64_t hw, int64_t C, int64_t C1, int64_t N, int groups, float eps,
+                        const float* w, const float* b) {
+    if (hw % GN_REC_CHUNK != 0 || !r1 || (r2 != nullptr) != (C1 < C) || C1 <= 0 || C1 > C) {
+        fprintf(stderr, "ggml-mi355x: GroupNorm finalize asked for a shape the side band does not describe\n");
+        abort();
+    }
+    const int chunks = (int)(hw / GN_REC_CHUNK), cpg = (int)((C + groups - 1) / groups);
+    KScope ks_(s, KF_GN_STATS, 0.0, (double)N * chunks * C * 8.0 + (double)N * C * 8.0);
+    if (g16_trace()) fprintf(stderr, "GN finalize hw=%lld C=%lld N=%lld groups=%d C1=%lld\n", (long long)hw, (long long)C, (long long)N, groups, (long long)C1);
+    k_gn_finalize<<<(unsigned)(N * groups), 64, 0, s>>>(scale, shift, r1, r2, chunks, (int)C, (int)C1, groups, cpg, eps, w, b);
+}
+
 static int64_t g_gn_split_min = 1 << 16;
 void gemm16_set_gn_split_min(int v) { g_gn_split_min = v <= 0 ? (1ll << 62) : (int64_t)v; }
 int gn_stats_split(int64_t hw, int64_t C, int64_t N, int groups) {
@@ -2247,6 +2320,7 @@
 void launch_gn_stats(hipStream_t s, float* scale, float* shift, const float* x, int64_t hw, int64_t C, int64_t N, int groups, float eps, const float* w,
                      const float* b, const float* x2, int64_t C1, float* part) {
     KScope ks_(s, KF_GN_STATS, 0.0, (double)hw * C * N * 4.0);
+    if (g16_trace()) fprintf(stderr, "GN stats hw=%lld C=%lld N=%lld groups=%d C1=%lld\n", (long long)hw, (long long)C, (long long)N, groups, (long long)(x2 ? C1 : C));
     const int cpg       = (int)((C + groups - 1) / groups);
     const int64_t cnt   = (int64_t)cpg * hw;
     const bool v4       = hw % 4 == 0 && ((((uintptr_t)x) | ((uintptr_t)x2)) & 15) == 0;
diff --git a/stable-diffusion.cpp_amd/csrc/kernels/kernels.h b/stable-diffusion.cpp_amd/csrc/kernels/kernels.h
--- a/stable-diffusion.cpp_amd/csrc/kernels/kernels.h
+++ b/stable-diffusion.cpp_amd/csrc/kernels/kernels.h
@@ -50,6 +50,11 @@
 void launch_wswz_linear(hipStream_t s, void* dst, const void* src, int src_type, int64_t K, int64_t R, int64_t src_row_bytes, int64_t geglu_inner = 0);
 void launch_wswz_conv(hipStream_t s, void* dst, const void* src, int64_t KW, int64_t KH, int64_t IC, int64_t OC, int kblk = 0);
 
+struct GnRec {
+    float mean, m2;
+};
+constexpr int GN_REC_CHUNK = 256;
+
 struct Epilogue {
     const float* bias     = nullptr;
     const float* residual = nullptr;
@@ -63,6 +68,7 @@
     const float* gn_b     = nullptr;
     int gn_groups         = 0;
     float gn_eps          = 0.f;
+    GnRec* gn_rec         = nullptr;
     void* ln_dst16        = nullptr;
     const float* ln_w     = nullptr;
     const float* ln_b     = nullptr;
@@ -121,9 +127,11 @@
 void gemm16_set_splitk_in_target(int v);
 void launch_gemm16_conv(hipStream_t s, float* dst, const void* x16_nhwc, const void* wswz, int64_t W, int64_t H, int64_t IC, int64_t N, int64_t OC,
                         int ksize, int stride, int pad, bool upscale2x, const Epilogue& ep, float* splitk_ws = nullptr, int* splitk_cnt = nullptr, int splitk_S = 0);
+bool gemm16_conv_gn_rec_supported(int64_t OHOW, int64_t N, int64_t OC, int64_t ICp, int ksize);
 int conv3w_plan(int64_t W, int64_t H, int64_t IC, int64_t N, int64_t OC, int ksize, int stride, bool upscale2x, int* bn_out = nullptr);
 void launch_conv3w(hipStream_t s, float* dst, const void* x16_nhwc, const void* wswz32, int64_t W, int64_t H, int64_t IC, int64_t N, int64_t OC, const Epilogue& ep,
                    float* splitk_ws, int S);
+bool conv3w_gn_rec_supported(int64_t OHOW, int64_t OC, int64_t N);
 void qgemm16_set_rb(int v);
 void conv3w_set_prio(int v);
 void conv3w_set(int v);
@@ -138,6 +146,8 @@
 void launch_gn_stats(hipStream_t s, float* scale, float* shift, const float* x, int64_t hw, int64_t C, int64_t N, int groups, float eps,
                      const float* w, const float* b, const float* x2 = nullptr, int64_t C1 = 0, float* part = nullptr);
 int gn_stats_split(int64_t hw, int64_t C, int64_t N, int groups);
+void launch_gn_finalize(hipStream_t s, float* scale, float* shift, const GnRec* r1, const GnRec* r2, int64_t hw, int64_t C, int64_t C1, int64_t N, int groups, float eps,
+                        const float* w, const float* b);
 void gemm16_set_gn_split_min(int v);
 void launch_nchw_to_nhwc_f16(hipStream_t s, void* dst, const float* x, int64_t hw, int64_t C, int64_t N, const float* scale, const float* shift,
                              int act, const float* x2 = nullptr, int64_t C1 = 0, void* dst_raw = nullptr, float post_mul = 1.f, float* dst_f32 = nullptr);
```

Result: faster. 384.1 it/s (median of 6 runs) (+2.1%).
